# NVIDIA/vid2vid

Hardware: NVIDIA H100
Metric: frames/sec at 2048x1024 inference (higher is better)
Workload: dtype bf16x3 (split-bf16 hi/lo operands, 3 wgmma per K block, fp32 accumulate: fp32-class)

## Files before the change

### include/v2v_b200.h

```cpp
#ifndef V2V_B200_H
#define V2V_B200_H
#include <stdint.h>

#ifdef __cplusplus
extern "C" {
#endif

typedef struct CUstream_st* v2v_stream_t;
typedef struct v2v_plan v2v_plan;

#define V2V_ERR_INVALID 10001
#define V2V_ERR_STATE 10002
#define V2V_ERR_UNSUPPORTED 10003

enum { V2V_PAD_NONE = 0, V2V_PAD_ZERO = 1, V2V_PAD_REFLECT = 2 };
enum { V2V_ACT_NONE = 0, V2V_ACT_RELU = 1, V2V_ACT_LRELU = 2, V2V_ACT_TANH = 3, V2V_ACT_SIGMOID = 4 };
enum { V2V_NORM_NONE = 0, V2V_NORM_BATCH = 1, V2V_NORM_INSTANCE = 2 };
enum { V2V_IMPL_UMMA = 0, V2V_IMPL_SIMT = 1 };
enum { V2V_PREC_BF16 = 0, V2V_PREC_BF16X3 = 1 };

int v2v_version(void);
const char* v2v_last_error(void);


int v2v_correlation_out_shape(int H, int W, int pad_size, int kernel_size, int max_displacement, int stride1,
                              int stride2, int* outC, int* outH, int* outW);
int v2v_correlation_forward(const float* in1, const float* in2, float* out, int N, int C, int H, int W, int pad_size,
                            int kernel_size, int max_displacement, int stride1, int stride2, int corr_type_multiply,
                            v2v_stream_t stream);

int v2v_resample2d_forward(const float* in1, const float* flow, float* out, int N, int C, int H, int W, int inH,
                           int inW, int kernel_size, v2v_stream_t stream);

int v2v_channelnorm_forward(const float* in, float* out, int N, int C, int H, int W, int norm_deg,
                            v2v_stream_t stream);

int v2v_resample_forward(const float* image, const float* flow, float* out, int N, int C, int H, int W,
                         int align_corners, v2v_stream_t stream);

int v2v_onehot_edges(const float* labels, const float* inst, float* out, int F, int label_nc, int use_instance, int H,
                     int W, v2v_stream_t stream);

int v2v_avgpool3s2(const float* in, float* out, int P, int H, int W, v2v_stream_t stream);

int v2v_fg_mask(const float* real_A, float* mask, int B, int T, int C, int H, int W, int t, const int* fg_labels,
                int n_labels, v2v_stream_t stream);

int v2v_ids_window_push(float* window, const void* frame, int dtype, int B, int T, int H, int W, v2v_stream_t stream);
#define V2V_MAX_SLOTS 64
enum { V2V_SLOT_KEEP = 0, V2V_SLOT_PUSH = 1, V2V_SLOT_RESTART = 2, V2V_SLOT_CLEAR = 3 };
int v2v_slots_window_push(float* window, const void* frames, int dtype, int B, int T, int C, int H, int W, const int* ops,
                          v2v_stream_t stream);
int v2v_tensor2im_u8(const float* image, uint8_t* out, int B, int C, int H, int W, v2v_stream_t stream);

int v2v_l1_loss_forward(const float* a, const float* b, const float* mask, int N, int C, int H, int W, double* sum_ws, float* out,
                        v2v_stream_t stream);
int v2v_l1_loss_backward(const float* a, const float* b, const float* mask, int N, int C, int H, int W, const float* grad_out,
                         float* grad_a, float* grad_b, v2v_stream_t stream);
int v2v_mse_const_forward(const float* x, int64_t numel, float target, double* sum_ws, float* out, v2v_stream_t stream);
int v2v_mse_const_backward(const float* x, int64_t numel, float target, const float* grad_out, float* grad_x, v2v_stream_t stream);
int v2v_avgpool3s2_backward(const float* grad_out, float* grad_in, int P, int H, int W, v2v_stream_t stream);
int v2v_resample_backward(const float* image, const float* flow, const float* grad_out, float* grad_image, float* grad_flow, int N,
                          int C, int H, int W, int align_corners, v2v_stream_t stream);
int v2v_avgpool2(const float* in, float* out, int P, int H, int W, v2v_stream_t stream);
int v2v_avgpool2_backward(const float* grad_out, float* grad_in, int P, int H, int W, v2v_stream_t stream);
int v2v_face_region(const float* real_A, int N, int C, int H, int W, int openpose_only, int* box, v2v_stream_t stream);

#define V2V_MAX_INSTANCE_IDS 256
#define V2V_FACE_MAX_LABELS 32
#define V2V_FACE_MAX_FEAT 64
int v2v_instance_mean(const float* x, const float* inst, float* out, int N, int C, int H, int W, int n_ids, v2v_stream_t stream);
int v2v_face_features(const float* pooled, const float* inst, const float* table, const int* rows, int n_labels, int max_rows,
                      int num_images, int feat_num, int table_stride, float* out, int* chosen, int N, int H, int W,
                      v2v_stream_t stream);

int v2v_flownet_prep(const float* frame0, const float* frame1, int64_t batch_stride, int64_t channel_stride, float* x, float* x1,
                     float* mean_ws, int B, int H, int W, float rgb_max, v2v_stream_t stream);
int v2v_resize(const float* in, float* out, float* out_div, int planes, int h, int w, int H, int W, int mode, int use_scale_factor,
               float mul, float pre_div, float div, v2v_stream_t stream);
int v2v_sub_channels(const float* a, const float* b, float* out, int N, int Ca, int c_off, int C, int H, int W, v2v_stream_t stream);
int v2v_flow_conf(const float* im1, const float* warped, float* conf, int N, int C, int H, int W, float threshold,
                  v2v_stream_t stream);


typedef struct v2v_conv_desc {
  int Cin, Cout, kh, kw;
  int stride;
  int pad;
  int pad_mode;
  int transposed;
  int output_padding;
  const float* weight;
  const float* bias;
  int Cout2;
  const float* weight2;
  const float* bias2;
} v2v_conv_desc;

typedef struct v2v_norm_desc {
  int kind;
  const float* gamma;
  const float* beta;
  float* running_mean;
  float* running_var;
  int64_t* num_batches_tracked;
  float momentum, eps;
} v2v_norm_desc;

typedef struct v2v_head_channel {
  int slot;
  int channel;
  int dst_C;
  int act;
  float scale;
} v2v_head_channel;

int v2v_plan_create(int device, int conv_impl , v2v_plan** out);
int v2v_plan_destroy(v2v_plan* plan);
int v2v_plan_set_precision(v2v_plan* plan, int precision);

int v2v_g_input(v2v_plan* plan, int slot, int N, int C_src, int c_off, int C, int H, int W, int* value_out);
#define V2V_INPUT_EXACT_BF16 1
int v2v_g_input_ex(v2v_plan* plan, int slot, int N, int C_src, int c_off, int C, int H, int W, int flags, int* value_out);
int v2v_g_conv(v2v_plan* plan, int value_in, const v2v_conv_desc* conv, int* raw_out);
int v2v_g_norm_act(v2v_plan* plan, int raw_in, const v2v_norm_desc* norm, int act, float slope, int add0, int add1,
                   int* value_out);
int v2v_g_norm_act_slice(v2v_plan* plan, int raw_in, int c_off, int C, const v2v_norm_desc* norm, int act, float slope,
                         int add0, int add1, int* value_out);
int v2v_g_conv_act(v2v_plan* plan, int value_in, const v2v_conv_desc* conv, int act, float slope, int* value_out);
int v2v_g_head(v2v_plan* plan, int value_in, const v2v_conv_desc* conv, const v2v_head_channel* channels);
int v2v_g_concat(v2v_plan* plan, const int* values, int n, int* value_out);
int v2v_g_correlation(v2v_plan* plan, int value_a, int value_b, int pad_size, int kernel_size, int max_displacement, int stride1,
                      int stride2, int act, float slope, int* value_out);
int v2v_g_maxpool2(v2v_plan* plan, int value_in, int* value_out);
int v2v_g_feature_l1(v2v_plan* plan, int value_x, int value_y, int slot, int index);
int v2v_g_export(v2v_plan* plan, int value, int slot);
int v2v_g_composite(v2v_plan* plan, int s_raw, int s_flow, int s_weight, int s_prev, int prev_C, int s_fg, int s_mask,
                    int s_final, int N, int H, int W, int use_warp, int align_corners);

int v2v_g_composite_ex(v2v_plan* plan, int s_raw, int s_flow, int s_weight, int s_prev, int prev_C, int s_fg, int s_mask,
                       int s_final, int s_raw_out, int N, int H, int W, int use_warp, int align_corners);

int v2v_plan_set_training(v2v_plan* plan, int on);
int v2v_plan_set_sample_stats(v2v_plan* plan, int on);
#define V2V_IMAGE_ACTIVE 1
#define V2V_IMAGE_RAW_ONLY 2
int v2v_plan_set_image_flags(v2v_plan* plan, int slot);
int v2v_plan_backward(v2v_plan* plan, void* const* io_ptrs, void* const* grad_io_ptrs, int n_io, const void* const* params,
                      void* const* param_grads, int n_params, v2v_stream_t stream);

int v2v_plan_finalize(v2v_plan* plan, v2v_stream_t stream);
int v2v_plan_finalize_ws(v2v_plan* plan, void* workspace, int64_t workspace_bytes, v2v_stream_t stream);
int v2v_plan_repack(v2v_plan* plan, v2v_stream_t stream);
int v2v_plan_run(v2v_plan* plan, void* const* io_ptrs, int n_io, int use_graph, v2v_stream_t stream);

int v2v_plan_profile(v2v_plan* plan, void* const* io_ptrs, int n_io, v2v_stream_t stream, int max_ops, int* kinds,
                     float* ms, double* macs, int* n_ops);

int v2v_plan_num_kernels(const v2v_plan* plan);
double v2v_plan_conv_macs(const v2v_plan* plan);
int64_t v2v_plan_workspace_bytes(const v2v_plan* plan);
int64_t v2v_plan_describe(const v2v_plan* plan, char* buf, int64_t cap);

int v2v_conv_tap_table(const v2v_conv_desc* conv, int H, int W, int allow_reuse, int* n_groups, int* R, int* plane,
                       int* dy, int* dx, int* tap0, int* n_phases, int* phase_begin, int* oy_add, int* ox_add,
                       int* pads, int* parity, int* grid_hw, int* out_hw, int* mul);

#ifdef __cplusplus
}
#endif
#endif
```

### vid2vid_b200/_lib.py

```python
import ctypes as C
import os

_HERE = os.path.dirname(os.path.abspath(__file__))
LIB_PATH = os.environ.get('V2V_LIB') or os.path.join(_HERE, 'libv2v_b200.so')

PAD_NONE, PAD_ZERO, PAD_REFLECT = 0, 1, 2
ACT_NONE, ACT_RELU, ACT_LRELU, ACT_TANH, ACT_SIGMOID = 0, 1, 2, 3, 4
NORM_NONE, NORM_BATCH, NORM_INSTANCE = 0, 1, 2
IMPL_UMMA, IMPL_SIMT = 0, 1
PREC_BF16, PREC_BF16X3 = 0, 1
IMAGE_ACTIVE, IMAGE_RAW_ONLY = 1, 2
SLOT_KEEP, SLOT_PUSH, SLOT_RESTART, SLOT_CLEAR = 0, 1, 2, 3
MAX_SLOTS = 64


class ConvDesc(C.Structure):
    _fields_ = [('Cin', C.c_int), ('Cout', C.c_int), ('kh', C.c_int), ('kw', C.c_int), ('stride', C.c_int),
                ('pad', C.c_int), ('pad_mode', C.c_int), ('transposed', C.c_int), ('output_padding', C.c_int),
                ('weight', C.c_void_p), ('bias', C.c_void_p), ('Cout2', C.c_int), ('weight2', C.c_void_p),
                ('bias2', C.c_void_p)]


class NormDesc(C.Structure):
    _fields_ = [('kind', C.c_int), ('gamma', C.c_void_p), ('beta', C.c_void_p), ('running_mean', C.c_void_p),
                ('running_var', C.c_void_p), ('num_batches_tracked', C.c_void_p), ('momentum', C.c_float),
                ('eps', C.c_float)]


class HeadChannel(C.Structure):
    _fields_ = [('slot', C.c_int), ('channel', C.c_int), ('dst_C', C.c_int), ('act', C.c_int), ('scale', C.c_float)]


_lib = None
LAUNCHES = [0]

SYMBOLS = [
    'v2v_version', 'v2v_last_error',
    'v2v_correlation_out_shape', 'v2v_correlation_forward', 'v2v_resample2d_forward', 'v2v_channelnorm_forward',
    'v2v_resample_forward', 'v2v_onehot_edges', 'v2v_avgpool3s2', 'v2v_fg_mask',
    'v2v_l1_loss_forward', 'v2v_l1_loss_backward', 'v2v_mse_const_forward', 'v2v_mse_const_backward', 'v2v_avgpool3s2_backward',
    'v2v_resample_backward', 'v2v_avgpool2', 'v2v_avgpool2_backward', 'v2v_face_region', 'v2v_instance_mean', 'v2v_face_features', 'v2v_ids_window_push', 'v2v_slots_window_push', 'v2v_tensor2im_u8', 'v2v_flownet_prep', 'v2v_resize', 'v2v_sub_channels', 'v2v_flow_conf',
    'v2v_plan_create', 'v2v_plan_destroy', 'v2v_plan_set_precision', 'v2v_g_input', 'v2v_g_input_ex', 'v2v_g_conv', 'v2v_g_norm_act', 'v2v_g_norm_act_slice', 'v2v_g_conv_act',
    'v2v_g_head', 'v2v_g_concat', 'v2v_g_correlation', 'v2v_g_maxpool2', 'v2v_g_feature_l1', 'v2v_g_export', 'v2v_g_composite', 'v2v_g_composite_ex', 'v2v_plan_set_training', 'v2v_plan_set_sample_stats', 'v2v_plan_set_image_flags', 'v2v_plan_backward', 'v2v_plan_finalize', 'v2v_plan_finalize_ws', 'v2v_plan_repack', 'v2v_plan_run',
    'v2v_plan_profile', 'v2v_plan_num_kernels', 'v2v_plan_conv_macs', 'v2v_plan_workspace_bytes', 'v2v_plan_describe',
    'v2v_conv_tap_table',
]


def lib():
    global _lib
    if _lib is not None:
        return _lib
    if not os.path.exists(LIB_PATH):
        raise RuntimeError('libv2v_b200.so is not built (%s). Run `python -c "import __graft_entry__ as g; g.build()"` '
                           'or `python vid2vid_b200/build.py`. There is no fallback path.' % LIB_PATH)
    l = C.CDLL(LIB_PATH)
    l.v2v_last_error.restype = C.c_char_p
    l.v2v_plan_conv_macs.restype = C.c_double
    l.v2v_plan_workspace_bytes.restype = C.c_int64
    l.v2v_plan_describe.restype = C.c_int64
    l.v2v_plan_describe.argtypes = [C.c_void_p, C.c_char_p, C.c_int64]
    l.v2v_plan_create.argtypes = [C.c_int, C.c_int, C.POINTER(C.c_void_p)]
    l.v2v_plan_destroy.argtypes = [C.c_void_p]
    l.v2v_plan_set_precision.argtypes = [C.c_void_p, C.c_int]
    l.v2v_g_input.argtypes = [C.c_void_p] + [C.c_int] * 7 + [C.POINTER(C.c_int)]
    l.v2v_g_input_ex.argtypes = [C.c_void_p] + [C.c_int] * 8 + [C.POINTER(C.c_int)]
    l.v2v_g_conv.argtypes = [C.c_void_p, C.c_int, C.POINTER(ConvDesc), C.POINTER(C.c_int)]
    l.v2v_g_norm_act.argtypes = [C.c_void_p, C.c_int, C.POINTER(NormDesc), C.c_int, C.c_float, C.c_int, C.c_int,
                                 C.POINTER(C.c_int)]
    l.v2v_g_norm_act_slice.argtypes = [C.c_void_p, C.c_int, C.c_int, C.c_int, C.POINTER(NormDesc), C.c_int, C.c_float, C.c_int,
                                       C.c_int, C.POINTER(C.c_int)]
    l.v2v_g_conv_act.argtypes = [C.c_void_p, C.c_int, C.POINTER(ConvDesc), C.c_int, C.c_float, C.POINTER(C.c_int)]
    l.v2v_g_head.argtypes = [C.c_void_p, C.c_int, C.POINTER(ConvDesc), C.POINTER(HeadChannel)]
    l.v2v_g_export.argtypes = [C.c_void_p, C.c_int, C.c_int]
    l.v2v_g_maxpool2.argtypes = [C.c_void_p, C.c_int, C.POINTER(C.c_int)]
    l.v2v_g_feature_l1.argtypes = [C.c_void_p] + [C.c_int] * 4
    l.v2v_g_concat.argtypes = [C.c_void_p, C.POINTER(C.c_int), C.c_int, C.POINTER(C.c_int)]
    l.v2v_g_correlation.argtypes = [C.c_void_p] + [C.c_int] * 8 + [C.c_float, C.POINTER(C.c_int)]
    l.v2v_g_composite.argtypes = [C.c_void_p] + [C.c_int] * 13
    l.v2v_plan_finalize.argtypes = [C.c_void_p, C.c_void_p]
    l.v2v_plan_finalize_ws.argtypes = [C.c_void_p, C.c_void_p, C.c_int64, C.c_void_p]
    l.v2v_g_composite_ex.argtypes = [C.c_void_p] + [C.c_int] * 14
    l.v2v_plan_set_training.argtypes = [C.c_void_p, C.c_int]
    l.v2v_plan_set_sample_stats.argtypes = [C.c_void_p, C.c_int]
    l.v2v_plan_set_image_flags.argtypes = [C.c_void_p, C.c_int]
    l.v2v_plan_backward.argtypes = [C.c_void_p, C.POINTER(C.c_void_p), C.POINTER(C.c_void_p), C.c_int, C.POINTER(C.c_void_p),
                                    C.POINTER(C.c_void_p), C.c_int, C.c_void_p]
    l.v2v_plan_repack.argtypes = [C.c_void_p, C.c_void_p]
    l.v2v_plan_run.argtypes = [C.c_void_p, C.POINTER(C.c_void_p), C.c_int, C.c_int, C.c_void_p]
    l.v2v_plan_profile.argtypes = [C.c_void_p, C.POINTER(C.c_void_p), C.c_int, C.c_void_p, C.c_int, C.POINTER(C.c_int),
                                   C.POINTER(C.c_float), C.POINTER(C.c_double), C.POINTER(C.c_int)]
    l.v2v_plan_num_kernels.argtypes = [C.c_void_p]
    l.v2v_plan_conv_macs.argtypes = [C.c_void_p]
    l.v2v_plan_workspace_bytes.argtypes = [C.c_void_p]
    fp, ip, vp = C.c_void_p, C.POINTER(C.c_int), C.c_void_p
    l.v2v_correlation_out_shape.argtypes = [C.c_int] * 7 + [ip, ip, ip]
    l.v2v_correlation_forward.argtypes = [fp, fp, fp] + [C.c_int] * 10 + [vp]
    l.v2v_resample2d_forward.argtypes = [fp, fp, fp] + [C.c_int] * 7 + [vp]
    l.v2v_channelnorm_forward.argtypes = [fp, fp] + [C.c_int] * 5 + [vp]
    l.v2v_resample_forward.argtypes = [fp, fp, fp] + [C.c_int] * 5 + [vp]
    l.v2v_onehot_edges.argtypes = [fp, fp, fp] + [C.c_int] * 5 + [vp]
    l.v2v_avgpool3s2.argtypes = [fp, fp] + [C.c_int] * 3 + [vp]
    l.v2v_fg_mask.argtypes = [fp, fp] + [C.c_int] * 6 + [ip, C.c_int, vp]
    l.v2v_l1_loss_forward.argtypes = [fp, fp, fp] + [C.c_int] * 4 + [vp, fp, vp]
    l.v2v_l1_loss_backward.argtypes = [fp, fp, fp] + [C.c_int] * 4 + [fp, fp, fp, vp]
    l.v2v_mse_const_forward.argtypes = [fp, C.c_int64, C.c_float, vp, fp, vp]
    l.v2v_mse_const_backward.argtypes = [fp, C.c_int64, C.c_float, fp, fp, vp]
    l.v2v_avgpool3s2_backward.argtypes = [fp, fp, C.c_int, C.c_int, C.c_int, vp]
    l.v2v_avgpool2.argtypes = [fp, fp] + [C.c_int] * 3 + [vp]
    l.v2v_avgpool2_backward.argtypes = [fp, fp] + [C.c_int] * 3 + [vp]
    l.v2v_face_region.argtypes = [fp] + [C.c_int] * 5 + [vp, vp]
    l.v2v_instance_mean.argtypes = [fp, fp, fp] + [C.c_int] * 5 + [vp]
    l.v2v_face_features.argtypes = [fp, fp, fp, ip] + [C.c_int] * 5 + [fp, vp] + [C.c_int] * 3 + [vp]
    l.v2v_resample_backward.argtypes = [fp, fp, fp, fp, fp] + [C.c_int] * 5 + [vp]
    l.v2v_ids_window_push.argtypes = [fp, vp] + [C.c_int] * 5 + [vp]
    l.v2v_slots_window_push.argtypes = [fp, vp] + [C.c_int] * 6 + [ip, vp]
    l.v2v_tensor2im_u8.argtypes = [fp, vp] + [C.c_int] * 4 + [vp]
    l.v2v_flownet_prep.argtypes = [fp, fp, C.c_int64, C.c_int64, fp, fp, fp, C.c_int, C.c_int, C.c_int, C.c_float, vp]
    l.v2v_resize.argtypes = [fp, fp, fp] + [C.c_int] * 7 + [C.c_float, C.c_float, C.c_float, vp]
    l.v2v_sub_channels.argtypes = [fp, fp, fp] + [C.c_int] * 6 + [vp]
    l.v2v_flow_conf.argtypes = [fp, fp, fp] + [C.c_int] * 4 + [C.c_float, vp]
    l.v2v_conv_tap_table.argtypes = [C.POINTER(ConvDesc), C.c_int, C.c_int, C.c_int] + [ip] * 15
    _lib = l
    return l


def check(rc):
    if rc != 0:
        msg = lib().v2v_last_error()
        raise RuntimeError('libv2v_b200: error %d: %s' % (rc, msg.decode() if msg else '?'))


def current_stream_ptr():
    import torch
    return C.c_void_p(torch.cuda.current_stream().cuda_stream)
```

### vid2vid_b200/csrc/plan.cu

```cuda
#include <algorithm>
#include <cmath>
#include <cstdarg>
#include <cstdio>
#include <cstring>
#include <string>
#include <vector>

#include "plan_internal.h"

namespace v2v {

thread_local std::string g_last_error;
void set_error(const char* fmt, ...) {
  char buf[1024];
  va_list ap;
  va_start(ap, fmt);
  vsnprintf(buf, sizeof(buf), fmt, ap);
  va_end(ap);
  g_last_error = buf;
}

struct DeviceGuard {
  int prev = -1; bool changed = false;
  explicit DeviceGuard(int dev) {
    if (cudaGetDevice(&prev) == cudaSuccess && prev != dev) changed = (cudaSetDevice(dev) == cudaSuccess);
  }
  ~DeviceGuard() { if (changed) cudaSetDevice(prev); }
};

static ActDesc make_act(const Value& v, const Req& r, int split) {
  ActDesc a{};
  a.split = split;
  a.base = nullptr;
  a.N = v.N; a.H = v.H; a.W = v.W; a.Cvalid = v.C; a.C = v.Cp;
  a.pad_t = r.pads[0]; a.pad_l = r.pads[1]; a.pad_b = r.pads[2]; a.pad_r = r.pads[3];
  a.parity = r.parity;
  const int Hpad = v.H + a.pad_t + a.pad_b, Wpad = v.W + a.pad_l + a.pad_r;
  if (a.parity) { a.P = 4; a.Hp = (Hpad + 1) / 2; a.Wp = (Wpad + 1) / 2; }
  else { a.P = 1; a.Hp = Hpad; a.Wp = Wpad; }
  return a;
}

static bool same_req(const Req& a, const Req& b) {
  return a.mode == b.mode && a.parity == b.parity && !memcmp(a.pads, b.pads, sizeof(a.pads));
}

static int add_req(Value& v, const Req& r) {
  for (size_t i = 0; i < v.reqs.size(); ++i)
    if (same_req(v.reqs[i], r)) return (int)i;
  v.reqs.push_back(r);
  return (int)v.reqs.size() - 1;
}

static Req conv_req(const v2v_conv_desc& c, const ConvGeom& g) {
  Req r{};
  r.mode = c.transposed ? PAD_ZERO : (c.pad == 0 ? PAD_ZERO : c.pad_mode);
  memcpy(r.pads, g.pads, sizeof(r.pads));
  r.parity = g.parity;
  return r;
}

static void mark_backward_liveness(v2v_plan* P) {
  const size_t nv = P->values.size(), nr = P->raws.size();
  std::vector<int> uses(nv, 0), raw_uses(nr, 0);
  std::vector<char> live(nv, 0), raw_live(nr, 0);
  auto dead = [&](int v) { return uses[v] > 0 && !live[v]; };
  auto use = [&](int v, bool l) { if (v < 0) return; ++uses[v]; if (l) live[v] = 1; };
  P->op_live.assign(P->gops.size(), 1);
  for (int i = (int)P->gops.size() - 1; i >= 0; --i) {
    const GOp& op = P->gops[i];
    bool ol = true;
    switch (op.kind) {
      case G_INPUT: case G_RAWIN: case G_NORM_ACT: case G_CONV_ACT: case G_CONCAT: case G_CORR: case G_MAXPOOL:
        ol = !dead(op.value_out); break;
      case G_CONV: ol = !(raw_uses[op.raw] > 0 && !raw_live[op.raw]); break;
      default: break;
    }
    P->op_live[i] = ol;
    switch (op.kind) {
      case G_CONV: case G_CONV_ACT: case G_HEAD: case G_EXPORT: case G_MAXPOOL: use(op.value_in, ol); break;
      case G_NORM_ACT: ++raw_uses[op.raw]; if (ol) raw_live[op.raw] = 1; use(op.add[0], ol); use(op.add[1], ol); break;
      case G_CONCAT: for (int v : op.cat_in) use(v, ol); break;
      case G_CORR: use(op.value_in, ol); use(op.value_in2, ol); break;
      case G_FEATL1: use(op.value_in, true); use(op.value_in2, false); break;
      default: break;
    }
  }
  for (size_t v = 0; v < nv; ++v) P->values[v].detached = dead((int)v);
}

static int lower(v2v_plan* P) {
  if (P->lowered) return 0;
  for (auto& op : P->gops) {
    if (op.kind == G_CONV || op.kind == G_CONV_ACT || op.kind == G_HEAD) {
      Value& vin = P->values[op.value_in];
      int rc = conv_geometry(op.conv, vin.Cp, op.kind == G_HEAD ? (P->impl == V2V_IMPL_UMMA ? 2 : 1) : 0, P->tiling_n(vin.N), vin.H,
                             vin.W, true, P->sp(), &op.geom);
      if (rc) return rc;
      op.req_index = add_req(vin, conv_req(op.conv, op.geom));
      const v2v_conv_desc& c = op.conv;
      const double px = op.conv.transposed ? (double)vin.N * vin.H * vin.W : (double)vin.N * op.geom.out_h * op.geom.out_w;
      op.macs = px * c.Cin * c.Cout * c.kh * c.kw;
      P->conv_macs += op.macs;
    }
  }
  mark_backward_liveness(P);
  for (auto& v : P->values) {
    if (v.reqs.empty()) { Req r{}; r.mode = PAD_NONE; v.reqs.push_back(r); }
    v.bufs.clear();
    for (auto& r : v.reqs) {
      P->acts.push_back(make_act(v, r, P->precise));
      P->act_pad_mode.push_back(r.mode);
      v.bufs.push_back((int)P->acts.size() - 1);
    }
  }
  P->lowered = true;
  return 0;
}

int new_value(v2v_plan* p, int N, int H, int W, int C) {
  Value v; v.N = N; v.H = H; v.W = W; v.C = C; v.Cp = std::max(pad_channels(C), p->pad_min);
  p->values.push_back(v);
  return (int)p->values.size() - 1;
}

int size_arena(v2v_plan* P) {
  if (P->sized) return 0;
  int rc = lower(P); if (rc) return rc;
  size_t off = 0;
  auto take = [&](size_t bytes) { size_t o = off; off = round_up_sz(off + bytes, 1024); return o; };
  P->act_off.assign(P->acts.size(), 0);
  for (size_t i = 0; i < P->acts.size(); ++i) P->act_off[i] = take(P->acts[i].elems() * sizeof(bf16));
  P->raw_off.assign(P->raws.size(), v2v_plan::RawOff{});
  P->w_off.assign(P->gops.size(), 0);
  for (size_t i = 0; i < P->gops.size(); ++i) {
    GOp& op = P->gops[i];
    if (op.kind == G_CONV || op.kind == G_CONV_ACT || op.kind == G_HEAD) {
      fill_conv_params(P, op);
      P->w_off[i] = take((size_t)P->sp() * (op.geom.headkx ? op.geom.headkx * op.conv.Cout : op.conv.Cout) * op.Ktotal * sizeof(bf16));
      if (op.kind == G_CONV) {
        Raw& r = P->raws[op.raw];
        r.desc.N = r.N; r.desc.H = r.H; r.desc.W = r.W; r.desc.Cvalid = r.C; r.desc.C = round_up(r.C, 8);
        r.desc.f32 = P->precise;
        P->raw_off[op.raw].raw = take(r.desc.elems() * r.desc.elem_bytes());
        P->raw_off[op.raw].scale = take((size_t)r.N * r.C * sizeof(float));
        P->raw_off[op.raw].shift = take((size_t)r.N * r.C * sizeof(float));
      }
    }
  }
  P->corr_off.assign(P->gops.size(), 0);
  for (size_t i = 0; i < P->gops.size(); ++i)
    if (P->gops[i].kind == G_CORR) {
      const Value& a = P->values[P->gops[i].value_in], &o = P->values[P->gops[i].value_out];
      P->corr_off[i] = take((2 * (size_t)a.N * a.C * a.H * a.W + (size_t)o.N * o.C * o.H * o.W) * sizeof(float));
    }
  P->l1_off.assign(P->gops.size(), 0);
  for (size_t i = 0; i < P->gops.size(); ++i)
    if (P->gops[i].kind == G_FEATL1) {
      const Value& x = P->values[P->gops[i].value_in];
      P->l1_off[i] = take((size_t)feature_l1_blocks(make_act(x, x.reqs[0], P->precise)) * sizeof(double));
    }
  P->stats_begin = off;
  for (size_t i = 0; i < P->raws.size(); ++i)
    if (P->raws[i].conv_op >= 0 && !P->raws[i].no_stats) P->raw_off[i].stats = take((size_t)P->raws[i].N * 2 * P->raws[i].C * sizeof(stat_t) + 64);
  P->stats_end = off;
  P->arena_bytes = off;
  P->sized = true;
  return 0;
}

int run_xop(v2v_plan* P, const XOp& x, cudaStream_t s) {
  switch (x.kind) {
    case X_IMPORT: V2V_CUDA(launch_import_nchw(x.imp, s)); break;
    case X_EXPORT: V2V_CUDA(launch_export_nchw(x.exp, s)); break;
    case X_FINALIZE: V2V_CUDA(launch_stats_finalize(x.fin, s)); break;
    case X_APPLY: V2V_CUDA(launch_norm_apply(x.app, s)); break;
    case X_COMPOSITE: V2V_CUDA(launch_composite(x.comp, s)); break;
    case X_RAWSTATS: V2V_CUDA(launch_raw_stats(x.rawd, x.stats, x.stats_C, s)); break;
    case X_MEMSET: V2V_CUDA(cudaMemsetAsync(x.ms_ptr, 0, x.ms_bytes, s)); break;
    case X_COPY: V2V_CUDA(launch_act_copy(x.copy, s)); break;
    case X_CORR:
      V2V_CUDA(launch_correlation(x.corr.in1, x.corr.in2, x.corr.out, x.corr.N, x.corr.C, x.corr.H, x.corr.W, x.corr.pad, x.corr.k,
                                  x.corr.max_disp, x.corr.s1, x.corr.s2, s));
      break;
    case X_MAXPOOL: V2V_CUDA(launch_maxpool2(x.pool, s)); break;
    case X_FEATL1: V2V_CUDA(launch_feature_l1(x.fl1, s)); break;
    case X_CONV: {
      const GOp& op = P->gops[x.gop];
      if (P->impl == V2V_IMPL_UMMA) V2V_CUDA(launch_conv_umma(op.tmA, op.tmB, op.kp, s));
      else V2V_CUDA(launch_conv_simt(P->acts[P->values[op.value_in].bufs[op.req_index]], op.wpacked, op.Ktotal, op.kp, s));
      break;
    }
  }
  return 0;
}

FeatL1Params featl1_params(const v2v_plan* P, const GOp& op) {
  FeatL1Params f{};
  f.x = P->acts[P->values[op.value_in].bufs[0]]; f.y = P->acts[P->values[op.value_in2].bufs[0]];
  f.Cvalid = P->values[op.value_in].C;
  f.io = P->io_dev; f.slot = op.slot; f.index = op.l1_index;
  f.blocks = feature_l1_blocks(f.x);
  return f;
}

}

extern "C" {

int v2v_version(void) { return 100; }
const char* v2v_last_error(void) { return g_last_error.c_str(); }

int v2v_plan_create(int device, int conv_impl, v2v_plan** out) {
  V2V_REQUIRE(out, V2V_ERR_INVALID, "null out");
  v2v_plan* p = new v2v_plan();
  p->device = device;
  p->impl = conv_impl;
  *out = p;
  return 0;
}

int v2v_plan_set_precision(v2v_plan* p, int precision) {
  V2V_REQUIRE(p && !p->lowered && p->gops.empty(), V2V_ERR_STATE, "set the precision before describing the plan");
  V2V_REQUIRE(precision == V2V_PREC_BF16 || precision == V2V_PREC_BF16X3, V2V_ERR_INVALID, "unknown precision %d", precision);
  p->precise = (precision == V2V_PREC_BF16X3);
  return 0;
}

int v2v_plan_set_training(v2v_plan* p, int on) {
  V2V_REQUIRE(p && !p->finalized, V2V_ERR_STATE, "set the training flag before finalize");
  V2V_REQUIRE(!(on && p->sample_stats), V2V_ERR_STATE,
              "a per-sample-statistics plan cannot train: training normalises with the statistics of the whole batch");
  p->train = on != 0;
  return 0;
}

int v2v_plan_set_sample_stats(v2v_plan* p, int on) {
  V2V_REQUIRE(p && !p->lowered, V2V_ERR_STATE, "set per-sample statistics before the plan is lowered");
  V2V_REQUIRE(on || p->flags_slot < 0, V2V_ERR_STATE, "a plan with per-image flags keeps per-sample statistics");
  V2V_REQUIRE(!(on && p->train), V2V_ERR_STATE,
              "per-sample statistics are for inference plans: a training plan normalises with the statistics of the whole batch");
  p->sample_stats = on != 0;
  return 0;
}

int v2v_plan_set_image_flags(v2v_plan* p, int slot) {
  V2V_REQUIRE(p && !p->finalized, V2V_ERR_STATE, "set the image flags before finalize");
  V2V_REQUIRE(!p->train, V2V_ERR_STATE, "per-image flags are for inference plans: a training plan cannot skip images");
  V2V_REQUIRE(p->sample_stats, V2V_ERR_STATE,
              "per-image flags need a per-sample-statistics plan: batch statistics mix the images, so none can be skipped");
  V2V_REQUIRE(slot >= 0, V2V_ERR_INVALID, "bad flags slot %d", slot);
  p->flags_slot = slot;
  p->n_slots = std::max(p->n_slots, slot + 1);
  return 0;
}

int v2v_plan_backward(v2v_plan* P, void* const* io_ptrs, void* const* grad_io_ptrs, int n_io, const void* const* params,
                      void* const* param_grads, int n_params, v2v_stream_t stream_) {
  V2V_REQUIRE(P && P->finalized && P->train, V2V_ERR_STATE, "plan not finalized in training mode");
  V2V_REQUIRE(n_io >= P->n_slots && io_ptrs && grad_io_ptrs, V2V_ERR_INVALID, "need %d io / gradient pointers", P->n_slots);
  DeviceGuard guard(P->device);
  std::unordered_map<const void*, void*> pg;
  for (int i = 0; i < n_params; ++i) if (params[i] && param_grads[i]) pg[params[i]] = param_grads[i];
  return run_backward(P, io_ptrs, grad_io_ptrs, pg, reinterpret_cast<cudaStream_t>(stream_));
}

int v2v_plan_destroy(v2v_plan* p) {
  if (!p) return 0;
  if (p->graph_exec) cudaGraphExecDestroy(p->graph_exec);
  if (p->graph_stream) cudaStreamDestroy(p->graph_stream);
  if (p->arena && p->arena_owned) cudaFree(p->arena);
  if (p->garena) cudaFree(p->garena);
  if (p->train_stats) cudaFree(p->train_stats);
  if (p->io_dev) cudaFree(p->io_dev);
  if (p->wg_stage) cudaFree(p->wg_stage);
  for (auto& u : p->bwd) if (u.child) v2v_plan_destroy(u.child);
  delete p;
  return 0;
}

int v2v_g_input_ex(v2v_plan* p, int slot, int N, int C_src, int c_off, int C, int H, int W, int flags, int* value_out) {
  int rc = v2v_g_input(p, slot, N, C_src, c_off, C, H, W, value_out);
  if (rc) return rc;
  p->values[*value_out].exact_bf16 = (flags & V2V_INPUT_EXACT_BF16) != 0;
  return 0;
}

int v2v_g_input(v2v_plan* p, int slot, int N, int C_src, int c_off, int C, int H, int W, int* value_out) {
  V2V_REQUIRE(p && !p->lowered && value_out, V2V_ERR_STATE, "plan already lowered or null");
  V2V_REQUIRE(slot >= 0 && N > 0 && C > 0 && c_off >= 0 && c_off + C <= C_src && H > 0 && W > 0, V2V_ERR_INVALID,
              "bad input description");
  GOp op; op.kind = G_INPUT; op.slot = slot; op.C_src = C_src; op.c_off = c_off;
  op.value_out = new_value(p, N, H, W, C);
  p->values[op.value_out].input_slot = slot;
  p->n_slots = std::max(p->n_slots, slot + 1);
  p->gops.push_back(op);
  *value_out = op.value_out;
  return 0;
}

static int check_conv(v2v_plan* p, int value_in, const v2v_conv_desc* c) {
  V2V_REQUIRE(p && !p->lowered && c, V2V_ERR_STATE, "plan already lowered or null");
  V2V_REQUIRE(value_in >= 0 && value_in < (int)p->values.size(), V2V_ERR_INVALID, "bad value id %d", value_in);
  V2V_REQUIRE(c->Cin == p->values[value_in].C, V2V_ERR_INVALID, "conv Cin %d != value channels %d", c->Cin,
              p->values[value_in].C);
  V2V_REQUIRE(c->Cout > 0, V2V_ERR_INVALID, "bad Cout");
  return 0;
}

int v2v_g_conv(v2v_plan* p, int value_in, const v2v_conv_desc* c, int* raw_out) {
  int rc = check_conv(p, value_in, c); if (rc) return rc;
  V2V_REQUIRE(raw_out, V2V_ERR_INVALID, "null raw_out");
  ConvGeom g; rc = conv_geometry(*c, p->values[value_in].Cp, 0, p->values[value_in].N, p->values[value_in].H, p->values[value_in].W, true, p->sp(), &g); if (rc) return rc;
  GOp op; op.kind = G_CONV; op.value_in = value_in; op.conv = *c;
  Raw r{}; r.N = p->values[value_in].N; r.H = g.out_h; r.W = g.out_w; r.C = c->Cout; r.conv_op = (int)p->gops.size();
  p->raws.push_back(r);
  op.raw = (int)p->raws.size() - 1;
  p->gops.push_back(op);
  *raw_out = op.raw;
  return 0;
}

int v2v_g_norm_act_slice(v2v_plan* p, int raw_in, int c_off, int C, const v2v_norm_desc* norm, int act, float slope,
                         int add0, int add1, int* value_out) {
  V2V_REQUIRE(p && !p->lowered && norm && value_out, V2V_ERR_STATE, "plan already lowered or null");
  V2V_REQUIRE(raw_in >= 0 && raw_in < (int)p->raws.size(), V2V_ERR_INVALID, "bad raw id");
  const Raw& r = p->raws[raw_in];
  V2V_REQUIRE(c_off >= 0 && C > 0 && c_off + C <= r.C && (c_off % 8) == 0, V2V_ERR_INVALID,
              "bad channel slice [%d, %d) of %d", c_off, c_off + C, r.C);
  GOp op; op.kind = G_NORM_ACT; op.raw = raw_in; op.norm = *norm; op.act = act; op.slope = slope;
  op.add[0] = add0; op.add[1] = add1; op.n_off = c_off; op.cC = C;
  for (int k = 0; k < 2; ++k)
    if (op.add[k] >= 0) {
      V2V_REQUIRE(op.add[k] < (int)p->values.size(), V2V_ERR_INVALID, "bad addend id");
      const Value& a = p->values[op.add[k]];
      V2V_REQUIRE(a.N == r.N && a.H == r.H && a.W == r.W && a.C == C, V2V_ERR_INVALID,
                  "addend shape (%d,%d,%d,%d) != raw shape (%d,%d,%d,%d)", a.N, a.C, a.H, a.W, r.N, C, r.H, r.W);
    }
  op.value_out = new_value(p, r.N, r.H, r.W, C);
  p->gops.push_back(op);
  *value_out = op.value_out;
  return 0;
}

int v2v_g_norm_act(v2v_plan* p, int raw_in, const v2v_norm_desc* norm, int act, float slope, int add0, int add1,
                   int* value_out) {
  V2V_REQUIRE(p && raw_in >= 0 && raw_in < (int)p->raws.size(), V2V_ERR_INVALID, "bad raw id");
  return v2v_g_norm_act_slice(p, raw_in, 0, p->raws[raw_in].C, norm, act, slope, add0, add1, value_out);
}

int v2v_g_conv_act(v2v_plan* p, int value_in, const v2v_conv_desc* c, int act, float slope, int* value_out) {
  int rc = check_conv(p, value_in, c); if (rc) return rc;
  V2V_REQUIRE(value_out, V2V_ERR_INVALID, "null value_out");
  ConvGeom g; rc = conv_geometry(*c, p->values[value_in].Cp, 0, p->values[value_in].N, p->values[value_in].H, p->values[value_in].W, true, p->sp(), &g); if (rc) return rc;
  GOp op; op.kind = G_CONV_ACT; op.value_in = value_in; op.conv = *c; op.act = act; op.slope = slope;
  op.value_out = new_value(p, p->values[value_in].N, g.out_h, g.out_w, c->Cout);
  p->gops.push_back(op);
  *value_out = op.value_out;
  return 0;
}

int v2v_g_head(v2v_plan* p, int value_in, const v2v_conv_desc* c, const v2v_head_channel* ch) {
  int rc = check_conv(p, value_in, c); if (rc) return rc;
  V2V_REQUIRE(ch && c->Cout <= V2V_MAX_HEAD && !c->transposed && c->stride == 1, V2V_ERR_UNSUPPORTED,
              "head conv must be stride-1 with Cout <= %d", V2V_MAX_HEAD);
  GOp op; op.kind = G_HEAD; op.value_in = value_in; op.conv = *c;
  for (int j = 0; j < c->Cout; ++j) { op.head[j] = ch[j]; p->n_slots = std::max(p->n_slots, ch[j].slot + 1); }
  p->gops.push_back(op);
  return 0;
}

int v2v_g_concat(v2v_plan* p, const int* values, int n, int* value_out) {
  V2V_REQUIRE(p && !p->lowered && values && n >= 1 && value_out, V2V_ERR_STATE, "plan already lowered or null");
  GOp op; op.kind = G_CONCAT;
  int C = 0;
  for (int i = 0; i < n; ++i) {
    V2V_REQUIRE(values[i] >= 0 && values[i] < (int)p->values.size(), V2V_ERR_INVALID, "bad value id %d", values[i]);
    const Value& a = p->values[values[i]], &a0 = p->values[values[0]];
    V2V_REQUIRE(a.N == a0.N && a.H == a0.H && a.W == a0.W, V2V_ERR_INVALID, "concat operands differ in extent");
    C += a.C;
    op.cat_in.push_back(values[i]);
  }
  const int N0 = p->values[values[0]].N, H0 = p->values[values[0]].H, W0 = p->values[values[0]].W;
  op.value_out = new_value(p, N0, H0, W0, C);
  p->gops.push_back(op);
  *value_out = op.value_out;
  return 0;
}

int v2v_g_correlation(v2v_plan* p, int value_a, int value_b, int pad_size, int kernel_size, int max_displacement, int stride1,
                      int stride2, int act, float slope, int* value_out) {
  V2V_REQUIRE(p && !p->lowered && value_out, V2V_ERR_STATE, "plan already lowered or null");
  V2V_REQUIRE(value_a >= 0 && value_a < (int)p->values.size() && value_b >= 0 && value_b < (int)p->values.size(), V2V_ERR_INVALID,
              "bad value id");
  const Value a = p->values[value_a], b = p->values[value_b];
  V2V_REQUIRE(a.N == b.N && a.C == b.C && a.H == b.H && a.W == b.W, V2V_ERR_INVALID, "correlation operands differ in shape");
  V2V_REQUIRE(kernel_size == 1 && stride1 == 1 && pad_size == max_displacement, V2V_ERR_UNSUPPORTED,
              "correlation: only kernel 1, stride1 1, pad == max displacement (FlowNetC.py:31)");
  V2V_REQUIRE(act == V2V_ACT_NONE || act == V2V_ACT_LRELU, V2V_ERR_UNSUPPORTED, "correlation: activation must be none / LeakyReLU");
  int oc, oh, ow;
  int rc = v2v_correlation_out_shape(a.H, a.W, pad_size, kernel_size, max_displacement, stride1, stride2, &oc, &oh, &ow);
  if (rc) return rc;
  GOp op; op.kind = G_CORR; op.value_in = value_a; op.value_in2 = value_b; op.act = act; op.slope = slope;
  op.corr[0] = pad_size; op.corr[1] = kernel_size; op.corr[2] = max_displacement; op.corr[3] = stride1; op.corr[4] = stride2;
  op.value_out = new_value(p, a.N, oh, ow, oc);
  p->gops.push_back(op);
  *value_out = op.value_out;
  return 0;
}

int v2v_g_maxpool2(v2v_plan* p, int value_in, int* value_out) {
  V2V_REQUIRE(p && !p->lowered && value_out, V2V_ERR_STATE, "plan already lowered or null");
  V2V_REQUIRE(value_in >= 0 && value_in < (int)p->values.size(), V2V_ERR_INVALID, "bad value id %d", value_in);
  const Value a = p->values[value_in];
  V2V_REQUIRE(a.H >= 2 && a.W >= 2, V2V_ERR_INVALID, "max-pool input %dx%d is smaller than its window", a.H, a.W);
  GOp op; op.kind = G_MAXPOOL; op.value_in = value_in;
  op.value_out = new_value(p, a.N, a.H / 2, a.W / 2, a.C);
  p->gops.push_back(op);
  *value_out = op.value_out;
  return 0;
}

int v2v_g_feature_l1(v2v_plan* p, int value_x, int value_y, int slot, int index) {
  V2V_REQUIRE(p && !p->lowered, V2V_ERR_STATE, "plan already lowered or null");
  V2V_REQUIRE(value_x >= 0 && value_x < (int)p->values.size() && value_y >= 0 && value_y < (int)p->values.size() && value_x != value_y,
              V2V_ERR_INVALID, "bad value ids %d, %d", value_x, value_y);
  V2V_REQUIRE(slot >= 0 && index >= 0, V2V_ERR_INVALID, "bad output slot %d / index %d", slot, index);
  const Value a = p->values[value_x], b = p->values[value_y];
  V2V_REQUIRE(a.N == b.N && a.C == b.C && a.H == b.H && a.W == b.W, V2V_ERR_INVALID, "feature L1 operands differ in shape");
  GOp op; op.kind = G_FEATL1; op.value_in = value_x; op.value_in2 = value_y; op.slot = slot; op.l1_index = index;
  p->n_slots = std::max(p->n_slots, slot + 1);
  p->gops.push_back(op);
  return 0;
}

int v2v_g_export(v2v_plan* p, int value, int slot) {
  V2V_REQUIRE(p && !p->lowered, V2V_ERR_STATE, "plan already lowered or null");
  V2V_REQUIRE(value >= 0 && value < (int)p->values.size() && slot >= 0, V2V_ERR_INVALID, "bad export");
  GOp op; op.kind = G_EXPORT; op.value_in = value; op.slot = slot;
  p->n_slots = std::max(p->n_slots, slot + 1);
  p->gops.push_back(op);
  return 0;
}

int v2v_g_composite(v2v_plan* p, int s_raw, int s_flow, int s_weight, int s_prev, int prev_C, int s_fg, int s_mask,
                    int s_final, int N, int H, int W, int use_warp, int align_corners) {
  return v2v_g_composite_ex(p, s_raw, s_flow, s_weight, s_prev, prev_C, s_fg, s_mask, s_final, -1, N, H, W, use_warp, align_corners);
}

int v2v_g_composite_ex(v2v_plan* p, int s_raw, int s_flow, int s_weight, int s_prev, int prev_C, int s_fg, int s_mask,
                       int s_final, int s_raw_out, int N, int H, int W, int use_warp, int align_corners) {
  V2V_REQUIRE(p && !p->lowered, V2V_ERR_STATE, "plan already lowered or null");
  V2V_REQUIRE(s_raw >= 0 && s_final >= 0, V2V_ERR_INVALID, "composite needs raw and final slots");
  V2V_REQUIRE(!use_warp || (s_flow >= 0 && s_weight >= 0 && s_prev >= 0 && prev_C >= 3), V2V_ERR_INVALID,
              "warp needs flow, weight and prev");
  V2V_REQUIRE((s_fg >= 0) == (s_mask >= 0), V2V_ERR_INVALID, "fg and mask go together");
  GOp op; op.kind = G_COMPOSITE;
  CompositeParams& c = op.comp;
  c.s_raw = s_raw; c.s_flow = s_flow; c.s_weight = s_weight; c.s_prev = s_prev; c.s_fg = s_fg; c.s_mask = s_mask;
  c.s_raw_out = s_raw_out;
  p->n_slots = std::max(p->n_slots, s_raw_out + 1);
  c.s_final = s_final; c.prev_C = prev_C; c.N = N; c.H = H; c.W = W; c.align_corners = align_corners; c.use_warp = use_warp;
  int m = std::max({s_raw, s_flow, s_weight, s_prev, s_fg, s_mask, s_final});
  p->n_slots = std::max(p->n_slots, m + 1);
  p->gops.push_back(op);
  return 0;
}

static int finalize_impl(v2v_plan* P, void* workspace, size_t workspace_bytes, cudaStream_t stream) {
  V2V_REQUIRE(P && !P->finalized, V2V_ERR_STATE, "plan null or already finalized");
  int rc = size_arena(P); if (rc) return rc;
  DeviceGuard guard(P->device);
  const std::vector<size_t>& act_off = P->act_off;
  const std::vector<v2v_plan::RawOff>& raw_off = P->raw_off;
  const std::vector<size_t>& w_off = P->w_off;
  const std::vector<size_t>& corr_off = P->corr_off;
  const size_t stats_begin = P->stats_begin, stats_end = P->stats_end;
  if (workspace) {
    V2V_REQUIRE(workspace_bytes >= P->arena_bytes && (reinterpret_cast<uintptr_t>(workspace) & 1023) == 0, V2V_ERR_INVALID,
                "workspace of %zu bytes (1024-byte aligned) needed, got %zu at %p", P->arena_bytes, workspace_bytes, workspace);
    P->arena = workspace; P->arena_owned = false;
  } else {
    V2V_CUDA(cudaMalloc(&P->arena, P->arena_bytes));
  }
  V2V_CUDA(cudaMemsetAsync(P->arena, 0, P->arena_bytes, stream));
  V2V_CUDA(cudaMalloc(reinterpret_cast<void**>(&P->io_dev), sizeof(void*) * std::max(1, P->n_slots)));
  uint8_t* base = reinterpret_cast<uint8_t*>(P->arena);
  for (size_t i = 0; i < P->acts.size(); ++i) P->acts[i].base = reinterpret_cast<bf16*>(base + act_off[i]);
  for (size_t i = 0; i < P->raws.size(); ++i) {
    Raw& r = P->raws[i];
    r.desc.base = base + raw_off[i].raw;
    r.stats = reinterpret_cast<stat_t*>(base + raw_off[i].stats);
    r.scale = reinterpret_cast<float*>(base + raw_off[i].scale);
    r.shift = reinterpret_cast<float*>(base + raw_off[i].shift);
  }

  if (P->train) {
    size_t tot = 0;
    for (auto& r : P->raws) tot += 2 * (size_t)r.N * r.C;
    float* st = nullptr;
    V2V_CUDA(cudaMalloc(reinterpret_cast<void**>(&st), std::max<size_t>(tot, 1) * sizeof(float)));
    V2V_CUDA(cudaMemsetAsync(st, 0, std::max<size_t>(tot, 1) * sizeof(float), stream));
    P->train_stats = st;
    for (auto& r : P->raws) { r.mean = st; st += (size_t)r.N * r.C; r.rstd = st; st += (size_t)r.N * r.C; }
  }
  if (stats_end > stats_begin) {
    XOp m; m.kind = X_MEMSET; m.ms_ptr = base + stats_begin; m.ms_bytes = stats_end - stats_begin;
    P->xops.push_back(m);
  }
  for (size_t i = 0; i < P->gops.size(); ++i) {
    GOp& op = P->gops[i];
    switch (op.kind) {
      case G_INPUT: {
        const Value& v = P->values[op.value_out];
        for (size_t m = 0; m < v.bufs.size(); ++m) {
          XOp x; x.kind = X_IMPORT; x.gop = (int)i;
          x.imp.io = reinterpret_cast<const void* const*>(P->io_dev); x.imp.slot = op.slot;
          x.imp.c_off = op.c_off; x.imp.C_src = op.C_src;
          x.imp.out = P->acts[v.bufs[m]]; x.imp.pad_mode = P->act_pad_mode[v.bufs[m]];
          x.imp.skip_lo = v.exact_bf16 ? 1 : 0;
          P->xops.push_back(x);
        }
        break;
      }
      case G_CONV: case G_CONV_ACT: case G_HEAD: {
        const Value& vin = P->values[op.value_in];
        const ActDesc& ain = P->acts[vin.bufs[op.req_index]];
        op.wpacked = reinterpret_cast<bf16*>(base + w_off[i]);
        ConvKernelParams& kp = op.kp;
        V2V_REQUIRE(kp.Cp == ain.C, V2V_ERR_STATE, "internal: conv of op %zu reads %d padded channels from a %d-channel buffer", i,
                    kp.Cp, ain.C);
        kp.io = P->io_dev;
        if (op.kind == G_CONV) {
          Raw& r = P->raws[op.raw];
          kp.epi = EPI_RAW_STATS; kp.out = r.desc.base; kp.out_C = r.desc.C; kp.out_f32 = r.desc.f32;
          kp.stats = r.no_stats ? nullptr : r.stats; kp.stats_C = r.C; kp.bias = nullptr;
        } else if (op.kind == G_CONV_ACT) {
          const Value& vo = P->values[op.value_out];
          V2V_REQUIRE(vo.bufs.size() == 1 && P->act_pad_mode[vo.bufs[0]] != PAD_REFLECT, V2V_ERR_UNSUPPORTED,
                      "conv_act output needs a single zero/none-padded consumer layout");
          kp.epi = EPI_ACT_BF16; kp.out_act = P->acts[vo.bufs[0]]; kp.out_C = kp.out_act.C;
        } else {
          kp.epi = EPI_HEAD_F32;
          kp.bias2 = op.conv.Cout2 > 0 ? op.conv.bias2 : nullptr; kp.Cout1 = op.conv.Cout - op.conv.Cout2;
          for (int j = 0; j < op.conv.Cout; ++j) {
            kp.head_slot[j] = op.head[j].slot;
            kp.head_off[j] = (long long)op.head[j].channel * op.geom.out_h * op.geom.out_w;
            kp.head_bstride[j] = (long long)op.head[j].dst_C * op.geom.out_h * op.geom.out_w;
            kp.head_act[j] = op.head[j].act; kp.head_scale[j] = op.head[j].scale;
          }
        }
        if (P->impl == V2V_IMPL_UMMA) {
          rc = make_tmap_act(&op.tmA, ain, kp.PW, kp.PH, kp.kc); if (rc) return rc;
          rc = make_tmap_w(&op.tmB, op.wpacked, P->sp() * op.Ktotal, op.geom.headkx ? op.geom.headkx * op.conv.Cout : op.conv.Cout, kp.BN,
                           kp.kc); if (rc) return rc;
        }
        rc = pack_one(op, stream); if (rc) return rc;
        XOp x; x.kind = X_CONV; x.gop = (int)i;
        P->xops.push_back(x);
        if (op.kind == G_CONV && P->impl == V2V_IMPL_SIMT) {
          XOp s; s.kind = X_RAWSTATS; s.rawd = P->raws[op.raw].desc; s.stats = P->raws[op.raw].stats; s.stats_C = P->raws[op.raw].C;
          P->xops.push_back(s);
        }
        break;
      }
      case G_NORM_ACT: {
        Raw& r = P->raws[op.raw];
        const GOp& cop = P->gops[r.conv_op];
        FinalizeParams fp{};
        const bool has_norm = op.norm.kind != V2V_NORM_NONE;
        if (has_norm) {
          fp.stats = r.stats; fp.Cs = r.C; fp.C = op.cC; fp.c_off = op.n_off; fp.scale_stride = r.C;
          fp.N = r.N;
          fp.count = (double)r.H * r.W; fp.instance = (op.norm.kind == V2V_NORM_INSTANCE) || P->sample_stats;
          fp.sample_running = P->sample_stats;
          fp.io = P->io_dev; fp.flags_slot = P->flags_slot;
          const int cout1 = cop.conv.Cout - cop.conv.Cout2;
          V2V_REQUIRE(op.n_off == 0 || (cop.conv.Cout2 > 0 && op.n_off == cout1), V2V_ERR_UNSUPPORTED,
                      "a raw slice must start at channel 0 or at the second weight set");
          fp.gamma = op.norm.gamma; fp.beta = op.norm.beta; fp.conv_bias = op.n_off == 0 ? cop.conv.bias : cop.conv.bias2;
          fp.momentum = op.norm.momentum; fp.eps = op.norm.eps;
        } else if (cop.conv.bias != nullptr) {
          V2V_REQUIRE(op.n_off == 0 && cop.conv.Cout2 == 0, V2V_ERR_UNSUPPORTED, "biased norm-less conv cannot be sliced");
          v2v_plan::BiasAffine ba{r.scale, r.shift, cop.conv.bias, r.N, r.C, r.C};
          P->bias_affines.push_back(ba);
          V2V_CUDA(launch_bias_affine(ba.scale, ba.shift, ba.bias, ba.N, ba.C, ba.stride, stream));
        }
        const Value& vo = P->values[op.value_out];
        for (size_t m = 0; m < vo.bufs.size(); ++m) {
          XOp a; a.kind = X_APPLY;
          ApplyParams& ap = a.app;
          ap.raw = r.desc;
          ap.raw.base = reinterpret_cast<uint8_t*>(r.desc.base) + (size_t)op.n_off * r.desc.elem_bytes();
          ap.raw.Cvalid = op.cC;
          ap.scale = (has_norm || cop.conv.bias != nullptr) ? r.scale + op.n_off : nullptr;
          ap.shift = r.shift + op.n_off;
          ap.scale_stride = r.C;
          ap.act = op.act; ap.slope = op.slope;
          ap.n_add = 0;
          for (int k = 0; k < 2; ++k) if (op.add[k] >= 0) ap.add[ap.n_add++] = P->acts[P->values[op.add[k]].bufs[0]];
          ap.out = P->acts[vo.bufs[m]]; ap.pad_mode = P->act_pad_mode[vo.bufs[m]];
          if (has_norm) {
            const bool first = std::find(r.running_done.begin(), r.running_done.end(), op.n_off) == r.running_done.end();
            FinalizeParams side = fp;
            side.running_mean = op.norm.running_mean; side.running_var = op.norm.running_var;
            side.num_batches_tracked = reinterpret_cast<long long*>(op.norm.num_batches_tracked);
            side.scale = r.scale; side.shift = r.shift; side.mean_out = r.mean; side.rstd_out = r.rstd;
            if (first) {
              GOp& prod = P->gops[r.conv_op];
              if (P->impl == V2V_IMPL_UMMA && prod.kp.n_fin < 2) {
                prod.kp.fin[prod.kp.n_fin++] = side;
                prod.kp.fin_counter = reinterpret_cast<unsigned int*>(reinterpret_cast<uint8_t*>(r.stats) + (size_t)r.N * 2 * r.C * sizeof(stat_t));
              } else {
                XOp f; f.kind = X_FINALIZE; f.fin = side; P->xops.push_back(f);
              }
              r.running_done.push_back(op.n_off);
            }
          }
          P->xops.push_back(a);
        }
        break;
      }
      case G_RAWIN: {
        const Value& vo = P->values[op.value_out];
        for (size_t m = 0; m < vo.bufs.size(); ++m) {
          XOp a; a.kind = X_APPLY;
          ApplyParams& ap = a.app;
          ap.raw.base = const_cast<float*>(op.ext_raw); ap.raw.N = vo.N; ap.raw.H = vo.H; ap.raw.W = vo.W; ap.raw.C = op.ext_C;
          ap.raw.Cvalid = vo.C; ap.raw.f32 = 1;
          ap.scale = nullptr; ap.shift = nullptr; ap.scale_stride = 0; ap.act = ACT_NONE; ap.slope = 0.f; ap.n_add = 0;
          ap.out = P->acts[vo.bufs[m]]; ap.pad_mode = P->act_pad_mode[vo.bufs[m]];
          P->xops.push_back(a);
        }
        break;
      }
      case G_EXPORT: {
        XOp x; x.kind = X_EXPORT; x.exp.io = P->io_dev; x.exp.slot = op.slot; x.exp.in = P->acts[P->values[op.value_in].bufs[0]];
        P->xops.push_back(x);
        break;
      }
      case G_COMPOSITE: {
        XOp x; x.kind = X_COMPOSITE; x.comp = op.comp; x.comp.io = P->io_dev; x.comp.s_flags = P->flags_slot;
        P->xops.push_back(x);
        break;
      }
      case G_CONCAT: {
        const Value& vo = P->values[op.value_out];
        for (size_t m = 0; m < vo.bufs.size(); ++m) {
          int c_off = 0;
          for (int src : op.cat_in) {
            XOp x; x.kind = X_COPY;
            x.copy.in = P->acts[P->values[src].bufs[0]];
            x.copy.out = P->acts[vo.bufs[m]];
            x.copy.c_off = c_off; x.copy.pad_mode = P->act_pad_mode[vo.bufs[m]];
            c_off += P->values[src].C;
            P->xops.push_back(x);
          }
        }
        break;
      }
      case G_MAXPOOL: {
        const Value& vo = P->values[op.value_out];
        for (size_t m = 0; m < vo.bufs.size(); ++m) {
          V2V_REQUIRE(P->act_pad_mode[vo.bufs[m]] != PAD_REFLECT, V2V_ERR_UNSUPPORTED, "max-pool output needs a zero / no halo");
          XOp x; x.kind = X_MAXPOOL; x.gop = (int)i;
          x.pool.in = P->acts[P->values[op.value_in].bufs[0]]; x.pool.out = P->acts[vo.bufs[m]];
          P->xops.push_back(x);
        }
        break;
      }
      case G_FEATL1: {
        XOp x; x.kind = X_FEATL1; x.gop = (int)i;
        x.fl1 = featl1_params(P, op);
        x.fl1.partials = reinterpret_cast<double*>(base + P->l1_off[i]);
        P->xops.push_back(x);
        break;
      }
      case G_CORR: {
        const Value& va = P->values[op.value_in], &vb = P->values[op.value_in2], &vo = P->values[op.value_out];
        float* sa = reinterpret_cast<float*>(base + corr_off[i]);
        float* sb = sa + (size_t)va.N * va.C * va.H * va.W;
        float* so = sb + (size_t)va.N * va.C * va.H * va.W;
        XOp ea; ea.kind = X_EXPORT; ea.exp.io = P->io_dev; ea.exp.slot = 0; ea.exp.direct = sa; ea.exp.in = P->acts[va.bufs[0]];
        XOp eb = ea; eb.exp.direct = sb; eb.exp.in = P->acts[vb.bufs[0]];
        P->xops.push_back(ea); P->xops.push_back(eb);
        XOp c; c.kind = X_CORR;
        c.corr = CorrParams{sa, sb, so, va.N, va.C, va.H, va.W, op.corr[0], op.corr[1], op.corr[2], op.corr[3], op.corr[4]};
        P->xops.push_back(c);
        for (size_t m = 0; m < vo.bufs.size(); ++m) {
          XOp x; x.kind = X_IMPORT; x.gop = (int)i;
          x.imp.io = reinterpret_cast<const void* const*>(P->io_dev); x.imp.slot = 0; x.imp.direct = so;
          x.imp.c_off = 0; x.imp.C_src = vo.C; x.imp.act = op.act; x.imp.slope = op.slope;
          x.imp.out = P->acts[vo.bufs[m]]; x.imp.pad_mode = P->act_pad_mode[vo.bufs[m]];
          P->xops.push_back(x);
        }
        break;
      }
    }
  }
  if (P->train) {
    rc = alloc_training(P, stream); if (rc) return rc;
    rc = build_backward_units(P, stream); if (rc) return rc;
  }
  V2V_CUDA(cudaStreamSynchronize(stream));
  P->finalized = true;
  return 0;
}

int v2v_plan_finalize(v2v_plan* P, v2v_stream_t stream_) {
  return finalize_impl(P, nullptr, 0, reinterpret_cast<cudaStream_t>(stream_));
}

int v2v_plan_finalize_ws(v2v_plan* P, void* workspace, int64_t workspace_bytes, v2v_stream_t stream_) {
  V2V_REQUIRE(workspace && workspace_bytes > 0, V2V_ERR_INVALID, "null workspace");
  return finalize_impl(P, workspace, (size_t)workspace_bytes, reinterpret_cast<cudaStream_t>(stream_));
}

int v2v_plan_repack(v2v_plan* P, v2v_stream_t stream_) {
  V2V_REQUIRE(P && P->finalized, V2V_ERR_STATE, "plan not finalized");
  DeviceGuard guard(P->device);
  cudaStream_t stream = reinterpret_cast<cudaStream_t>(stream_);
  for (auto& op : P->gops)
    if (op.kind == G_CONV || op.kind == G_CONV_ACT || op.kind == G_HEAD) { int rc = pack_one(op, stream); if (rc) return rc; }
  for (const auto& ba : P->bias_affines) V2V_CUDA(launch_bias_affine(ba.scale, ba.shift, ba.bias, ba.N, ba.C, ba.stride, stream));
  for (auto& u : P->bwd) if (u.child) { int rc = v2v_plan_repack(u.child, stream_); if (rc) return rc; }
  return 0;
}

static int check_composite_alignment(const v2v_plan* P, void* const* io_ptrs) {
  for (const XOp& x : P->xops)
    if (x.kind == X_COMPOSITE && composite_vec4(x.comp))
      V2V_REQUIRE(composite_slots_aligned(x.comp, io_ptrs), V2V_ERR_INVALID,
                  "composite (W %% 4 == 0) needs 16-byte aligned raw / final / flow / weight / fg / mask tensors");
  return 0;
}

int v2v_plan_run(v2v_plan* P, void* const* io_ptrs, int n_io, int use_graph, v2v_stream_t stream_) {
  V2V_REQUIRE(P && P->finalized, V2V_ERR_STATE, "plan not finalized");
  V2V_REQUIRE(n_io >= P->n_slots && io_ptrs, V2V_ERR_INVALID, "need %d io pointers, got %d", P->n_slots, n_io);
  if (int rc = check_composite_alignment(P, io_ptrs)) return rc;
  DeviceGuard guard(P->device);
  cudaStream_t stream = reinterpret_cast<cudaStream_t>(stream_);
  V2V_CUDA(cudaMemcpyAsync(P->io_dev, io_ptrs, sizeof(void*) * P->n_slots, cudaMemcpyHostToDevice, stream));
  if (use_graph & 2) {
    for (const XOp& x : P->xops) {
      if (x.kind == X_FINALIZE) {
        XOp y = x; y.fin.running_mean = nullptr; y.fin.running_var = nullptr; y.fin.num_batches_tracked = nullptr;
        int rc = run_xop(P, y, stream); if (rc) return rc;
      } else if (x.kind == X_CONV && P->impl == V2V_IMPL_UMMA && P->gops[x.gop].kp.n_fin > 0) {
        const GOp& op = P->gops[x.gop];
        ConvKernelParams kp = op.kp;
        for (int q = 0; q < kp.n_fin; ++q) { kp.fin[q].running_mean = nullptr; kp.fin[q].running_var = nullptr; kp.fin[q].num_batches_tracked = nullptr; }
        V2V_CUDA(launch_conv_umma(op.tmA, op.tmB, kp, stream));
      } else { int rc = run_xop(P, x, stream); if (rc) return rc; }
    }
    return 0;
  }
  if (!use_graph) {
    for (const XOp& x : P->xops) { int rc = run_xop(P, x, stream); if (rc) return rc; }
    return 0;
  }
  if (!P->graph_exec) {
    cudaGraph_t graph;
    if (!P->graph_stream) V2V_CUDA(cudaStreamCreateWithFlags(&P->graph_stream, cudaStreamNonBlocking));
    V2V_CUDA(cudaStreamBeginCapture(P->graph_stream, cudaStreamCaptureModeThreadLocal));
    int rc = 0;
    for (const XOp& x : P->xops) { rc = run_xop(P, x, P->graph_stream); if (rc) break; }
    cudaError_t e = cudaStreamEndCapture(P->graph_stream, &graph);
    if (rc) return rc;
    V2V_CUDA(e);
    V2V_CUDA(cudaGraphInstantiate(&P->graph_exec, graph, 0));
    V2V_CUDA(cudaGraphDestroy(graph));
  }
  V2V_CUDA(cudaGraphLaunch(P->graph_exec, stream));
  return 0;
}

int v2v_plan_profile(v2v_plan* P, void* const* io_ptrs, int n_io, v2v_stream_t stream_, int max_ops, int* kinds,
                     float* ms, double* macs, int* n_ops) {
  V2V_REQUIRE(P && P->finalized, V2V_ERR_STATE, "plan not finalized");
  V2V_REQUIRE(n_io >= P->n_slots && io_ptrs && kinds && ms && macs && n_ops, V2V_ERR_INVALID, "bad profile arguments");
  if (int rc = check_composite_alignment(P, io_ptrs)) return rc;
  DeviceGuard guard(P->device);
  cudaStream_t stream = reinterpret_cast<cudaStream_t>(stream_);
  V2V_CUDA(cudaMemcpyAsync(P->io_dev, io_ptrs, sizeof(void*) * P->n_slots, cudaMemcpyHostToDevice, stream));
  const int n = std::min<int>(max_ops, (int)P->xops.size());
  std::vector<cudaEvent_t> ev(n + 1);
  for (auto& e : ev) V2V_CUDA(cudaEventCreate(&e));
  V2V_CUDA(cudaEventRecord(ev[0], stream));
  for (int i = 0; i < (int)P->xops.size(); ++i) {
    int rc = run_xop(P, P->xops[i], stream);
    if (rc) return rc;
    if (i < n) V2V_CUDA(cudaEventRecord(ev[i + 1], stream));
  }
  V2V_CUDA(cudaStreamSynchronize(stream));
  for (int i = 0; i < n; ++i) {
    V2V_CUDA(cudaEventElapsedTime(&ms[i], ev[i], ev[i + 1]));
    kinds[i] = (int)P->xops[i].kind;
    macs[i] = (P->xops[i].kind == X_CONV) ? P->gops[P->xops[i].gop].macs : 0.0;
  }
  for (auto& e : ev) cudaEventDestroy(e);
  *n_ops = n;
  return 0;
}

int v2v_plan_num_kernels(const v2v_plan* P) { return P ? (int)P->xops.size() : 0; }
double v2v_plan_conv_macs(const v2v_plan* P) {
  if (!P) return 0.0;
  if (!P->lowered) lower(const_cast<v2v_plan*>(P));
  return P->conv_macs;
}
int64_t v2v_plan_workspace_bytes(const v2v_plan* P_) {
  v2v_plan* P = const_cast<v2v_plan*>(P_);
  if (!P) return 0;
  if (!P->sized && size_arena(P)) return -1;
  return (int64_t)P->arena_bytes;
}

}

extern "C" {

int64_t v2v_plan_describe(const v2v_plan* P_, char* buf, int64_t cap) {
// ... 78 lines not shown
```

### vid2vid_b200/csrc/plan_internal.h

```cpp
#pragma once
#include <string>
#include <unordered_map>
#include <vector>

#include "../../include/v2v_b200.h"
#include "v2v_internal.h"
#include "backward.h"

namespace v2v {

void set_error(const char* fmt, ...);

#define V2V_CUDA(expr)                                                                          \
  do {                                                                                          \
    cudaError_t e__ = (expr);                                                                   \
    if (e__ != cudaSuccess) {                                                                   \
      set_error("%s failed: %s (%s:%d)", #expr, cudaGetErrorString(e__), __FILE__, __LINE__);   \
      return (int)e__;                                                                          \
    }                                                                                           \
  } while (0)
#define V2V_REQUIRE(cond, code, ...) \
  do {                               \
    if (!(cond)) {                   \
      set_error(__VA_ARGS__);        \
      return code;                   \
    }                                \
  } while (0)

static inline int round_up(int a, int b) { return (a + b - 1) / b * b; }
static inline size_t round_up_sz(size_t a, size_t b) { return (a + b - 1) / b * b; }
static inline int pad_channels(int c) { return c <= 16 ? 16 : (c <= 32 ? 32 : round_up(c, 64)); }

struct ConvGeom {
  int pads[4];
  int parity;
  int grid_h, grid_w;
  int out_h, out_w;
  int mul;
  int TH, TW, R;
  int RW;
  int patch2d_kc;
  int patch2d_bn;
  int headkx;
  int n_groups, n_phases;
  ConvGroup groups[V2V_MAX_TAPS];
  ConvPhase phases[V2V_MAX_PHASES];
};

struct Req { int mode, pads[4], parity; };

struct Value {
  int N, H, W, C;
  int Cp;
  std::vector<Req> reqs;
  std::vector<int> bufs;
  float* gval = nullptr;
  int input_slot = -1;
  bool exact_bf16 = false;
  bool detached = false;
};
struct Raw {
  int N, H, W, C;
  int conv_op = -1;
  RawDesc desc{};
  stat_t* stats = nullptr;
  float* scale = nullptr; float* shift = nullptr;
  std::vector<int> running_done;
  float* mean = nullptr; float* rstd = nullptr;
  float* graw = nullptr;
  bool no_stats = false;
};

enum GKind { G_INPUT, G_CONV, G_NORM_ACT, G_CONV_ACT, G_HEAD, G_EXPORT, G_COMPOSITE, G_CONCAT, G_CORR, G_RAWIN, G_MAXPOOL, G_FEATL1 };
struct GOp {
  GKind kind;
  int slot = -1, C_src = 0, c_off = 0;
  int value_in = -1, value_out = -1, raw = -1;
  v2v_conv_desc conv{};
  ConvGeom geom{};
  int req_index = -1;
  v2v_norm_desc norm{};
  int act = 0; float slope = 0.f;
  int add[2] = {-1, -1};
  int n_off = 0, cC = 0;
  v2v_head_channel head[V2V_MAX_HEAD];
  CompositeParams comp{};
  std::vector<int> cat_in;
  int value_in2 = -1;
  int l1_index = 0;
  int corr[5] = {0, 0, 0, 0, 0};
  const float* ext_raw = nullptr; int ext_C = 0;
  int pack_dgrad = 0; const float* dg_w2 = nullptr; int dg_Cout1 = 0;
  bf16* wpacked = nullptr; int Ktotal = 0, Cp = 0;
  float* gdz = nullptr;
  double macs = 0.0;
  CUtensorMap tmA{}, tmB{};
  ConvKernelParams kp{};
};

enum XKind { X_IMPORT, X_CONV, X_RAWSTATS, X_FINALIZE, X_APPLY, X_EXPORT, X_COMPOSITE, X_MEMSET, X_COPY, X_CORR, X_MAXPOOL, X_FEATL1 };
struct XOp {
  XKind kind;
  int gop = -1;
  ImportParams imp{};
  ExportParams exp{};
  FinalizeParams fin{};
  ApplyParams app{};
  CompositeParams comp{};
  CopyParams copy{};
  CorrParams corr{};
  PoolParams pool{};
  FeatL1Params fl1{};
  RawDesc rawd{}; stat_t* stats = nullptr; int stats_C = 0;
  void* ms_ptr = nullptr; size_t ms_bytes = 0;
};

}

using namespace v2v;

struct BwdUnit {
  int gop = -1, mode = 0;
  v2v_plan* child = nullptr;
  int child_raw = -1;
  bool wgrad = false;
  std::string simt, wg_simt;
  CUtensorMap tmOut{}, tmIn{};
  WgradParams wg{};
  int M = 0, M1 = 0, Nv = 0;
};

struct v2v_plan {
  std::vector<BwdUnit> bwd;
  std::vector<int> bwd_of;
  float* wg_stage = nullptr;
  int pad_min = 0;

  int device = 0;
  int impl = V2V_IMPL_UMMA;
  int precise = 0;
  int sp() const { return precise ? 2 : 1; }
  bool lowered = false, finalized = false;
  bool train = false;
  bool sample_stats = false;
  int tiling_n(int N) const { return sample_stats ? 1 : N; }
  int flags_slot = -1;
  void* garena = nullptr; size_t garena_bytes = 0;
  std::vector<float*> gslot;
  float* gsums = nullptr;
  float* train_stats = nullptr;
  std::vector<Value> values;
  std::vector<Raw> raws;
  std::vector<GOp> gops;
  std::vector<ActDesc> acts;
  std::vector<int> act_pad_mode;
  std::vector<char> op_live;
  std::vector<XOp> xops;
  int n_slots = 0;
  double conv_macs = 0.0;
  struct BiasAffine { float* scale; float* shift; const float* bias; int N, C, stride; };
  std::vector<BiasAffine> bias_affines;
  struct RawOff { size_t raw = 0, stats = 0, scale = 0, shift = 0; };
  bool sized = false, arena_owned = true;
  std::vector<size_t> act_off, w_off, corr_off, l1_off;
  std::vector<RawOff> raw_off;
  size_t stats_begin = 0, stats_end = 0;
  void* arena = nullptr; size_t arena_bytes = 0;
  void** io_dev = nullptr;
  cudaGraphExec_t graph_exec = nullptr;
  cudaStream_t graph_stream = nullptr;
};

namespace v2v {

extern const int kSmemBudget;
int conv_geometry(const v2v_conv_desc& c, int Cp, int head, int N, int H, int W, bool allow_reuse, int sp, ConvGeom* g);
void fill_conv_params(v2v_plan* P, GOp& op);
int make_tmap_act(CUtensorMap* tm, const ActDesc& a, int box_w, int box_h, int kc);
int make_tmap_w(CUtensorMap* tm, bf16* w, int Ktotal, int Cout, int BN, int kc);
int pack_one(const GOp& op, cudaStream_t stream);
void describe_conv(v2v_plan* P, const GOp& op, std::string& s);

int new_value(v2v_plan* p, int N, int H, int W, int C);
int size_arena(v2v_plan* P);
int run_xop(v2v_plan* P, const XOp& x, cudaStream_t s);
FeatL1Params featl1_params(const v2v_plan* P, const GOp& op);

int alloc_training(v2v_plan* P, cudaStream_t stream);
int choose_backward_unit(v2v_plan* P, int i, BwdUnit& u);
int build_backward_units(v2v_plan* P, cudaStream_t stream);
int run_backward(v2v_plan* P, void* const* io, void* const* gio, const std::unordered_map<const void*, void*>& pg,
                 cudaStream_t s);
void describe_backward_unit(const BwdUnit& u, std::string& s);
void describe_epilogue_backward(const v2v_plan* P, std::string& s);

}
```

### vid2vid_b200/csrc/pyramid.cu

```cuda
#include "../../include/v2v_b200.h"
#include "ptx.cuh"
#include "v2v_internal.h"

namespace v2v {

__global__ void onehot_edges_kernel(const float* __restrict__ labels, const float* __restrict__ inst,
                                    float* __restrict__ out, int F, int label_nc, int use_inst, int H, int W) {
  const size_t HW = (size_t)H * W;
  const int Cout = label_nc + (use_inst ? 1 : 0);
  const int x = blockIdx.x * blockDim.x + threadIdx.x, y = blockIdx.y, f = blockIdx.z;
  if (x < W) {
    const size_t pix = (size_t)y * W + x;
    const size_t idx = (size_t)f * HW + pix;
    const int lab = (int)labels[idx];
    float* o = out + (size_t)f * Cout * HW + pix;
    for (int c = 0; c < label_nc; ++c) o[(size_t)c * HW] = (c == lab) ? 1.f : 0.f;
    if (use_inst) {
      const float* ip = inst + (size_t)f * HW;
      const float v = ip[pix];
      bool e = false;
      if (x > 0) e |= (ip[pix - 1] != v);
      if (x < W - 1) e |= (ip[pix + 1] != v);
      if (y > 0) e |= (ip[pix - W] != v);
      if (y < H - 1) e |= (ip[pix + W] != v);
      o[(size_t)label_nc * HW] = e ? 1.f : 0.f;
    }
  }
}

__global__ void __launch_bounds__(256) avgpool3s2_kernel(const float* __restrict__ in, float* __restrict__ out, int P, int H, int W,
                                                         int Ho, int Wo) {
  const int xo = blockIdx.x * blockDim.x + threadIdx.x;
  if (xo >= Wo) return;
  const int yo = blockIdx.y;
  for (int pl = blockIdx.z; pl < P; pl += gridDim.z) {
    const float* ip = in + (size_t)pl * H * W;
    float s = 0.f;
    int cnt = 0;
#pragma unroll
    for (int dy = -1; dy <= 1; ++dy) {
      const int y = 2 * yo + dy;
      if (y < 0 || y >= H) continue;
#pragma unroll
      for (int dx = -1; dx <= 1; ++dx) {
        const int x = 2 * xo + dx;
        if (x < 0 || x >= W) continue;
        s += __ldg(ip + (size_t)y * W + x);
        ++cnt;
      }
    }
    out[((size_t)pl * Ho + yo) * Wo + xo] = s / (float)cnt;
  }
}

__global__ void __launch_bounds__(128) avgpool3s2_vec_kernel(const float* __restrict__ in, float* __restrict__ out, int P, int H, int W,
                                                             int Ho, int Wo) {
  const int k = blockIdx.x * blockDim.x + threadIdx.x;
  if (4 * k >= W) return;
  const int yo = blockIdx.y;
  for (int pl = blockIdx.z; pl < P; pl += gridDim.z) {
    const float* ip = in + (size_t)pl * H * W;
    float s0 = 0.f, s1 = 0.f;
    int rows = 0;
#pragma unroll
    for (int dy = -1; dy <= 1; ++dy) {
      const int y = 2 * yo + dy;
      if (y < 0 || y >= H) continue;
      ++rows;
      const float* rp = ip + (size_t)y * W + 4 * k;
      const float4 v = *reinterpret_cast<const float4*>(rp);
      if (k > 0) s0 += __ldg(rp - 1);
      s0 += v.x; s0 += v.y;
      s1 += v.y; s1 += v.z; s1 += v.w;
    }
    const int c0 = (k > 0 ? 3 : 2), c1 = 3;
    *reinterpret_cast<float2*>(out + ((size_t)pl * Ho + yo) * Wo + 2 * k) = make_float2(s0 / (float)(rows * c0), s1 / (float)(rows * c1));
  }
}

struct FgLabels { int v[16]; };
__global__ void fg_mask_kernel(const float* __restrict__ real_A, float* __restrict__ mask, int B, int T, int C, int H,
                               int W, int t, FgLabels labels, int n_labels) {
  const size_t HW = (size_t)H * W, total = (size_t)B * HW;
  for (size_t idx = blockIdx.x * (size_t)blockDim.x + threadIdx.x; idx < total;
       idx += (size_t)gridDim.x * blockDim.x) {
    const int b = (int)(idx / HW);
    const size_t pix = idx - (size_t)b * HW;
    float s = 0.f;
    for (int i = 0; i < n_labels; ++i) s += real_A[(((size_t)b * T + t) * C + labels.v[i]) * HW + pix];
    mask[idx] = fminf(fmaxf(s, 0.f), 1.f);
  }
}

__global__ void ids_window_push_kernel(float* __restrict__ window, const void* __restrict__ frame, int dtype, int T, size_t HW,
                                       size_t total) {
  for (size_t idx = blockIdx.x * (size_t)blockDim.x + threadIdx.x; idx < total; idx += (size_t)gridDim.x * blockDim.x) {
    const size_t b = idx / HW, pix = idx - b * HW;
    float* win = window + b * T * HW;
    for (int t = 0; t + 1 < T; ++t) win[(size_t)t * HW + pix] = win[(size_t)(t + 1) * HW + pix];
    float v;
    if (dtype == 0) v = (float)reinterpret_cast<const uint8_t*>(frame)[idx];
    else if (dtype == 1) v = (float)reinterpret_cast<const int*>(frame)[idx];
    else v = reinterpret_cast<const float*>(frame)[idx];
    win[(size_t)(T - 1) * HW + pix] = v;
  }
}

struct SlotOps { int v[V2V_MAX_SLOTS]; };
__global__ void slots_window_push_kernel(float* __restrict__ window, const void* __restrict__ frames, int dtype, int T, size_t E,
                                         size_t total, SlotOps ops) {
  for (size_t idx = blockIdx.x * (size_t)blockDim.x + threadIdx.x; idx < total; idx += (size_t)gridDim.x * blockDim.x) {
    const size_t b = idx / E, e = idx - b * E;
    const int op = ops.v[b];
    if (op == V2V_SLOT_KEEP) continue;
    float* win = window + b * T * E;
    if (op == V2V_SLOT_PUSH)
      for (int t = 0; t + 1 < T; ++t) win[(size_t)t * E + e] = win[(size_t)(t + 1) * E + e];
    else
      for (int t = 0; t + 1 < T; ++t) win[(size_t)t * E + e] = 0.f;
    float v = 0.f;
    if (op != V2V_SLOT_CLEAR) {
      if (dtype == 0) v = (float)reinterpret_cast<const uint8_t*>(frames)[idx];
      else if (dtype == 1) v = (float)reinterpret_cast<const int*>(frames)[idx];
      else v = reinterpret_cast<const float*>(frames)[idx];
    }
    win[(size_t)(T - 1) * E + e] = v;
  }
}

__global__ void tensor2im_u8_kernel(const float* __restrict__ img, uint8_t* __restrict__ out, int C, size_t HW, size_t total) {
  for (size_t pix = blockIdx.x * (size_t)blockDim.x + threadIdx.x; pix < total; pix += (size_t)gridDim.x * blockDim.x) {
    const size_t b = pix / HW, p = pix - b * HW;
    for (int c = 0; c < C; ++c) {
      float v = __fmul_rn(__fdiv_rn(__fadd_rn(img[(b * C + c) * HW + p], 1.f), 2.0f), 255.0f);
      v = fminf(fmaxf(v, 0.f), 255.f);
      out[pix * C + c] = (uint8_t)v;
    }
  }
}

static inline int grid1d(size_t total) {
  size_t b = (total + 255) / 256;
  const size_t cap = 132 * 16;
  return (int)(b < cap ? (b ? b : 1) : cap);
}

cudaError_t launch_onehot_edges(const float* labels, const float* inst, float* out, int F, int label_nc, int use_inst,
                                int H, int W, cudaStream_t s) {
  dim3 grid((W + 255) / 256, H, F);
  onehot_edges_kernel<<<grid, 256, 0, s>>>(labels, inst, out, F, label_nc, use_inst, H, W);
  return cudaGetLastError();
}
cudaError_t launch_avgpool3s2(const float* in, float* out, int P, int H, int W, cudaStream_t s) {
  const int Ho = (H - 1) / 2 + 1, Wo = (W - 1) / 2 + 1;
  const bool aligned = (reinterpret_cast<uintptr_t>(in) & 15) == 0 && (reinterpret_cast<uintptr_t>(out) & 7) == 0;
  if (W % 4 == 0 && W >= 4 && aligned) {
    dim3 grid((W / 4 + 127) / 128, Ho, P < 64 ? P : 64);
    avgpool3s2_vec_kernel<<<grid, 128, 0, s>>>(in, out, P, H, W, Ho, Wo);
    return cudaGetLastError();
  }
  dim3 grid((Wo + 255) / 256, Ho, P < 64 ? P : 64);
  avgpool3s2_kernel<<<grid, 256, 0, s>>>(in, out, P, H, W, Ho, Wo);
  return cudaGetLastError();
}
cudaError_t launch_ids_window_push(float* window, const void* frame, int dtype, int B, int T, int H, int W, cudaStream_t s) {
  ids_window_push_kernel<<<grid1d((size_t)B * H * W), 256, 0, s>>>(window, frame, dtype, T, (size_t)H * W, (size_t)B * H * W);
  return cudaGetLastError();
}
cudaError_t launch_slots_window_push(float* window, const void* frames, int dtype, int B, int T, int C, int H, int W, const int* ops,
                                    cudaStream_t s) {
  SlotOps o{};
  for (int b = 0; b < B; ++b) o.v[b] = ops[b];
  const size_t E = (size_t)C * H * W;
  slots_window_push_kernel<<<grid1d((size_t)B * E), 256, 0, s>>>(window, frames, dtype, T, E, (size_t)B * E, o);
  return cudaGetLastError();
}
cudaError_t launch_tensor2im_u8(const float* img, uint8_t* out, int B, int C, int H, int W, cudaStream_t s) {
  tensor2im_u8_kernel<<<grid1d((size_t)B * H * W), 256, 0, s>>>(img, out, C, (size_t)H * W, (size_t)B * H * W);
  return cudaGetLastError();
}
cudaError_t launch_fg_mask(const float* real_A, float* mask, int B, int T, int C, int H, int W, int t,
                           FgLabels labels, int n_labels, cudaStream_t s) {
  fg_mask_kernel<<<grid1d((size_t)B * H * W), 256, 0, s>>>(real_A, mask, B, T, C, H, W, t, labels, n_labels);
  return cudaGetLastError();
}

}
```

### vid2vid_b200/csrc/v2v_internal.h

```cpp
#pragma once
#include <cuda.h>
#include <cuda_runtime.h>
#include <cuda_bf16.h>
#include <stdint.h>

namespace v2v {

typedef __nv_bfloat16 bf16;

struct ActDesc {
  bf16* base;
  int N, H, W;
  int C;
  int Cvalid;
  int pad_t, pad_l, pad_b, pad_r;
  int parity;
  int P, Hp, Wp;
  int split;
  __host__ __device__ int Cs() const { return C << split; }
  __host__ __device__ size_t elems() const { return (size_t)N * P * Hp * Wp * Cs(); }
  __host__ __device__ size_t offset(int n, int y, int x) const {
    int yp = y + pad_t, xp = x + pad_l;
    if (parity) {
      int pl = ((yp & 1) << 1) | (xp & 1);
      return ((((size_t)n * 4 + pl) * Hp + (yp >> 1)) * Wp + (xp >> 1)) * Cs();
    }
    return (((size_t)n * Hp + yp) * Wp + xp) * Cs();
  }
};

struct RawDesc {
  void* base;
  int N, H, W, C, Cvalid;
  int f32;
  __host__ __device__ size_t elems() const { return (size_t)N * H * W * C; }
  __host__ __device__ size_t elem_bytes() const { return f32 ? 4 : 2; }
};

enum PadMode { PAD_NONE = 0, PAD_ZERO = 1, PAD_REFLECT = 2 };
enum ActKind { ACT_NONE = 0, ACT_RELU = 1, ACT_LRELU = 2, ACT_TANH = 3, ACT_SIGMOID = 4 };
enum EpiMode { EPI_RAW_STATS = 0, EPI_HEAD_F32 = 1, EPI_ACT_BF16 = 2 };

#define V2V_MAX_TAPS 64
#define V2V_MAX_PHASES 4
#define V2V_MAX_HEAD 16
#define V2V_MAX_ACC_COLS 128

struct ConvGroup {
  int8_t plane, dy, dx, pad_;
  int16_t tap0, pad2_;
};

struct ConvPhase {
  int group_begin, group_end;
  int oy_add, ox_add;
};

typedef unsigned long long stat_t;
#define V2V_STAT_SUM_SCALE 1048576.0f
#define V2V_STAT_SQ_SCALE 65536.0f

struct FinalizeParams {
  const stat_t* stats;
  int Cs, C;
  int N;
  double count;
  int instance;
  int sample_running;
  const float* gamma;
  const float* beta;
  const float* conv_bias;
  float* running_mean;
  float* running_var;
  long long* num_batches_tracked;
  float momentum, eps;
  float* scale;
  float* shift;
  float* mean_out;
  float* rstd_out;
  int c_off, scale_stride;
  void* const* io;
  int flags_slot = -1;
};

struct ConvKernelParams {
  int N, tiles_x, tiles_y, TH, TW;
  int grid_h, grid_w;
  int Cout, BN;
  int Cp, cblocks;
  int kc, row_bytes, kmma;
  int kmma_last;
  int BNt;
  int layout_type, sbo_bytes;
  int R, RW;
  int PW, PH;
  int sbo_a_bytes;
  int a_slot_bytes, b_slot_bytes, SB;
  int b_resident;
  int n_tiles, m_total;
  int CG, SG;
  int MG, total_units;
  int num_phases;
  int split;
  int a_half_bytes, b_half_bytes;
  int Khalf;
  int out_f32;
  int ring2, TB, SBr;
  int tile_dx;
  int headkx;
  int n_fin;
  FinalizeParams fin[2];
  unsigned int* fin_counter;
  int a_exact;

  ConvPhase phases[V2V_MAX_PHASES];
  ConvGroup groups[V2V_MAX_TAPS];
  int epi;
  int oy_mul, ox_mul;
  int out_H, out_W, out_C;
  void* out;
  ActDesc out_act;
  stat_t* stats;
  int stats_C;
  const float* bias;
  const float* bias2; int Cout1;
  int grid;
  void* const* io;
  int head_slot[V2V_MAX_HEAD];
  long long head_off[V2V_MAX_HEAD];
  long long head_bstride[V2V_MAX_HEAD];
  int head_act[V2V_MAX_HEAD];
  float head_scale[V2V_MAX_HEAD];
  float lrelu_slope;
  int act;
};

cudaError_t launch_conv_umma(const CUtensorMap& tmA, const CUtensorMap& tmB, const ConvKernelParams& p,
                             cudaStream_t stream);
cudaError_t launch_conv_simt(const ActDesc& in, const bf16* wpacked, int Ktotal, const ConvKernelParams& p,
                             cudaStream_t stream);
size_t conv_umma_smem_bytes(const ConvKernelParams& p);
int conv_umma_tail_width(const ConvKernelParams& p);
int conv_umma_async_epilogue(const ConvKernelParams& p);



struct ApplyParams {
  RawDesc raw;
  const float* scale;
  const float* shift;
  int scale_stride;
  int act; float slope;
  int n_add;
  ActDesc add[2];
  ActDesc out;
  int pad_mode;
};

struct ImportParams {
  const void* const* io;
  int slot;
  const float* direct;
  int act; float slope;
  int c_off, C_src;
  ActDesc out;
  int pad_mode;
  int skip_lo;
};
struct ExportParams {
  void* const* io;
  int slot;
  float* direct;
  ActDesc in;
};

struct CopyParams {
  ActDesc in, out;
  int c_off;
  int pad_mode;
};

struct CorrParams {
  const float* in1; const float* in2; float* out;
  int N, C, H, W, pad, k, max_disp, s1, s2;
};

struct PackParams {
  const float* w;
  const float* w2; int Cout1;
  int transposed;
  int Cout, Cin, kh, kw;
  int Cp, ntaps;
  int8_t tap_ky[V2V_MAX_TAPS], tap_kx[V2V_MAX_TAPS];
  int split;
  int headkx;
  int dgrad;
  bf16* out;
};

struct CompositeParams {
  void* const* io;
  int s_raw, s_flow, s_weight, s_prev, s_fg, s_mask, s_final;
  int s_raw_out;
  int prev_C;
  int N, H, W;
  int align_corners;
  int use_warp;
  int s_flags = -1;
};

struct PoolParams {
  ActDesc in, out;
};
struct FeatL1Params {
  ActDesc x, y;
  int Cvalid;
  void* const* io;
  int slot, index;
  double* partials;
  int blocks;
};

cudaError_t launch_raw_stats(const RawDesc& raw, stat_t* stats, int stats_C, cudaStream_t stream);

__device__ __forceinline__ void split_bf16(float x, bf16& hi, bf16& lo) {
  hi = __float2bfloat16_rn(x);
  lo = __float2bfloat16_rn(x - __bfloat162float(hi));
}
cudaError_t launch_stats_finalize(const FinalizeParams& p, cudaStream_t stream);
cudaError_t launch_norm_apply(const ApplyParams& p, cudaStream_t stream);
bool norm_apply_uses_rows(const ApplyParams& p);
cudaError_t launch_import_nchw(const ImportParams& p, cudaStream_t stream);
cudaError_t launch_export_nchw(const ExportParams& p, cudaStream_t stream);
cudaError_t launch_pack_weights(const PackParams& p, cudaStream_t stream);
cudaError_t launch_act_copy(const CopyParams& p, cudaStream_t stream);
cudaError_t launch_bias_affine(float* scale, float* shift, const float* bias, int N, int C, int stride, cudaStream_t stream);
cudaError_t launch_correlation(const float*, const float*, float*, int, int, int, int, int, int, int, int, int, cudaStream_t);
cudaError_t launch_composite(const CompositeParams& p, cudaStream_t stream);
bool composite_vec4(const CompositeParams& p);
bool composite_slots_aligned(const CompositeParams& p, void* const* io);
cudaError_t launch_maxpool2(const PoolParams& p, cudaStream_t stream);
cudaError_t launch_maxpool2_bwd(const PoolParams& p, const float* gout, float* gin, cudaStream_t stream);
cudaError_t launch_feature_l1(const FeatL1Params& p, cudaStream_t stream);
cudaError_t launch_feature_l1_bwd(const FeatL1Params& p, const float* g, float* gx, cudaStream_t stream);
int feature_l1_blocks(const ActDesc& x);
int device_sm_count();

}
```

### vid2vid_b200/model_g.py

```python
import collections
import contextlib
import os

import torch
import torch.nn as nn

from .base_model import HostScheduleMixin
from . import networks, ops


def _adam(params, **kw):
    params = list(params)
    if params and all(p.is_cuda for p in params):
        try:
            return torch.optim.Adam(params, fused=True, **kw)
        except (TypeError, RuntimeError):
            pass
    return torch.optim.Adam(params, **kw)


class Vid2VidModelG(HostScheduleMixin, nn.Module):
    def name(self):
        return 'Vid2VidModelG'

    def initialize(self, opt):
        self.opt = opt
        self.gpu_ids = opt.gpu_ids
        self.isTrain = opt.isTrain
        self.n_scales = opt.n_scales_spatial
        self.use_single_G = opt.use_single_G
        if getattr(opt, 'openpose_only', False):
            opt.no_flow = True
        dev = torch.device('cuda', self.gpu_ids[0] if len(self.gpu_ids) else torch.cuda.current_device())
        self.device_ = dev
        for s in range(self.n_scales):
            setattr(self, 'netG' + str(s), networks.build_netG(opt, s).to(dev))
        getattr(self, 'netG' + str(self.n_scales - 1)).input_exact_bf16 = bool(opt.label_nc != 0)
        if (not self.isTrain or getattr(opt, 'continue_train', False) or getattr(opt, 'load_pretrain', '')) and \
                not getattr(opt, 'synthetic_weights', False):
            for s in range(self.n_scales):
                self.load_network(getattr(self, 'netG' + str(s)), 'G' + str(s), opt.which_epoch, getattr(opt, 'load_pretrain', ''))
        self.netG_i = self.load_single_G() if self.use_single_G else None
        self.fake_B_prev = None
        if self.isTrain:
            self.init_train()
        return self

    def load_network(self, network, network_label, epoch_label, save_dir=''):
        save_filename = '%s_net_%s.pth' % (epoch_label, network_label)
        save_dir = save_dir or os.path.join(self.opt.checkpoints_dir, self.opt.name)
        save_path = os.path.join(save_dir, save_filename)
        if not os.path.isfile(save_path):
            print('%s not exists yet!' % save_path)
            if 'G0' in network_label:
                raise FileNotFoundError('Generator must exist! (%s)' % save_path)
            return
        sd = torch.load(save_path, map_location=self.device_)
        try:
            network.load_state_dict(sd)
        except Exception:
            own = network.state_dict()
            kept = {k: v for k, v in sd.items() if k in own and v.size() == own[k].size()}
            missing = sorted({k.split('.')[0] for k in own if k not in kept})
            print('Pretrained network %s: loaded %d of %d tensors; not initialised from the file: %s' % (
                network_label, len(kept), len(own), missing))
            own.update(kept)
            network.load_state_dict(own)

    def load_single_G(self):
        opt = self.opt
        if 'City' in opt.dataroot:
            single_path = 'checkpoints/label2city_single/'
            if opt.loadSize == 512:
                load_path, netG = single_path + 'latest_net_G_512.pth', networks.define_G(35, 3, 0, 64, 'global', 3, 'instance', 0, [], opt)
            elif opt.loadSize == 1024:
                load_path, netG = single_path + 'latest_net_G_1024.pth', networks.define_G(35, 3, 0, 64, 'global', 4, 'instance', 0, [], opt)
            elif opt.loadSize == 2048:
                load_path, netG = single_path + 'latest_net_G_2048.pth', networks.define_G(35, 3, 0, 32, 'local', 4, 'instance', 0, [], opt)
            else:
                raise ValueError('Single image generator does not exist')
        elif 'face' in opt.dataroot:
            single_path = 'checkpoints/edge2face_single/'
            load_path = single_path + 'latest_net_G.pth'
            opt.feat_num = 16
            netG = networks.define_G(15, 3, 0, 64, 'global_with_features', 3, 'instance', 0, [], opt)
            self.netE = self._load(networks.define_G(3, 16, 0, 16, 'encoder', 4, 'instance', 0, []), single_path + 'latest_net_E.pth')
            self.load_face_features(single_path + 'features.npy')
        else:
            raise ValueError('Single image generator does not exist')
        return self._load(netG, load_path)

    def _load(self, net, path):
        if not (getattr(self.opt, 'synthetic_weights', False) and not os.path.exists(path)):
            if not os.path.exists(path):
                raise FileNotFoundError('first-frame generator weights not found: %s' % path)
            net.load_state_dict(torch.load(path, map_location=self.device_))
        return net.to(self.device_)

    def load_face_features(self, path='checkpoints/edge2face_single/features.npy', features=None):
        if features is None:
            if os.path.exists(path):
                import numpy as np
                features = np.load(path, encoding='latin1', allow_pickle=True).item()
            elif getattr(self.opt, 'synthetic_weights', False):
                features = networks.synthetic_face_features(16, self.opt.feat_num, seed=0)
            else:
                raise FileNotFoundError('face features table not found: %s' % path)
        table, self.face_rows, self.face_num_images = networks.pack_face_features(features, self.opt.feat_num)
        self.face_table = table.to(self.device_)
        return features

    def encode_input(self, input_map, real_image, inst_map=None):
        size = input_map.size()
        self.bs, tG, self.height, self.width = size[0], size[1], size[3], size[4]
        input_map = input_map.to(self.device_, torch.float32)
        if self.opt.label_nc != 0:
            inst = inst_map.to(self.device_, torch.float32) if self.opt.use_instance else None
            input_map = ops.onehot_edges(input_map, inst, self.opt.label_nc, self.opt.use_instance)
        elif self.opt.use_instance:
            raise NotImplementedError('use_instance without label_nc')
        pool_map = None
        if self.opt.dataset_mode == 'face':
            pool_map = inst_map.to(self.device_, torch.float32)
        if real_image is not None:
            real_image = real_image.to(self.device_, torch.float32)
        return input_map, real_image, pool_map

    def build_pyr(self, tensor):
        if tensor is None:
            return [None] * self.n_scales
        pyr = [tensor]
        for _ in range(1, self.n_scales):
            pyr.append(ops.avgpool3s2(pyr[-1]))
        return pyr

    def compute_mask(self, real_As, ts, te=None):
        assert te is None or te == ts + 1
        return ops.fg_mask(real_As, ts, list(self.opt.fg_labels))

    def inference(self, input_A, input_B, inst_A):
        with torch.no_grad():
            real_A, real_B, pool_map = self.encode_input(input_A, input_B, inst_A)
            with self._per_clip_statistics(self.bs > 1):
                return self._inference(real_A, real_B, pool_map)

    @contextlib.contextmanager
    def _per_clip_statistics(self, on):
        nets = [getattr(self, 'netG' + str(s)) for s in range(self.n_scales)] + ([self.netG_i] if self.netG_i is not None else [])
        prev = [getattr(net, 'sample_stats', False) for net in nets]
        for net in nets:
            net.sample_stats = on
        try:
            yield
        finally:
            for net, p in zip(nets, prev):
                net.sample_stats = p

    def _inference(self, real_A, real_B, pool_map):
        self.is_first_frame = self.fake_B_prev is None
        if self.is_first_frame:
            self.fake_B_prev = self.generate_first_frame(real_A, real_B, pool_map)
        elif self.bs != self._clips():
            raise ValueError('this sequence was started with %d clip(s) and is fed %d: clips of one sequence start and advance '
                             'together (reset_stream() starts a new one)' % (self._clips(), self.bs))
        real_A = self.build_pyr(real_A)
        self.fake_B_feat = self.flow_feat = self.fake_B_fg_feat = None
        for s in range(self.n_scales):
            fake_B = self.generate_frame_infer(real_A[self.n_scales - 1 - s], s)
        return fake_B, (real_A[0][0, -1] if self.bs == 1 else real_A[0][:, -1])

    def _clips(self):
        return self.fake_B_prev[0].shape[0] if self.fake_B_prev[0].dim() == 5 else 1

    def reset_stream(self, clips=None):
        n = self._clips() if self.fake_B_prev is not None else 0
        if clips is not None and n > 1 and sorted(set(clips)) != list(range(n)):
            raise NotImplementedError('restarting clip(s) %s of a running batch of %d clips is not supported: the clips of a batch '
                                      'start and advance together; call reset_stream() to restart the whole batch, or use '
                                      'stream_slots(B), whose slots start and stop independently' % (list(clips), n))
        self.fake_B_prev = None
        self._win_A = self._win_I = None

    _DT = {torch.uint8: 0, torch.int32: 1, torch.float32: 2}

    def inference_stream(self, label_frame, inst_frame=None, out_u8=None):
        import ctypes as C
        from . import _lib as L
        if self.opt.dataset_mode == 'face' and self.use_single_G:
            raise ValueError('inference_stream does not take the real frames that the face first-frame generator needs '
                             '(use_single_G with dataset_mode face): use inference()')
        tG = self.opt.n_frames_G
        H, W = label_frame.shape[-2:]
        B = label_frame.shape[0] if label_frame.dim() == 3 else 1
        if inst_frame is not None and tuple(inst_frame.shape) != tuple(label_frame.shape):
            raise ValueError('inst_frame %s does not match label_frame %s' % (tuple(inst_frame.shape), tuple(label_frame.shape)))
        dev = self.device_
        if getattr(self, '_win_A', None) is not None and self._win_A.shape[0] != B:
            raise ValueError('this stream was started with %d clip(s) and is fed %d: clips of one stream start and advance '
                             'together (reset_stream() starts a new one)' % (self._win_A.shape[0], B))
        if getattr(self, '_win_A', None) is None or self._win_A.shape[-2:] != (H, W):
            self._win_A = torch.zeros(B, tG, 1, H, W, device=dev)
            self._win_I = torch.zeros(B, tG, 1, H, W, device=dev) if self.opt.use_instance else None
            self._win_n = 0
        for win, fr in ((self._win_A, label_frame), (self._win_I, inst_frame if inst_frame is not None else label_frame)):
            if win is None:
                continue
            fr = fr.to(dev, non_blocking=True).contiguous()
            if fr.dtype not in self._DT:
                raise TypeError('id maps must be uint8, int32 or float32')
            L.check(L.lib().v2v_ids_window_push(C.c_void_p(win.data_ptr()), C.c_void_p(fr.data_ptr()), self._DT[fr.dtype], B, tG, H,
                                                W, L.current_stream_ptr()))
            L.LAUNCHES[0] += 1
        self._win_n += 1
        if self._win_n < tG:
            return None
        fake_B, _ = self.inference(self._win_A, None, self._win_I)
        if out_u8 is None:
            return fake_B
        shape = (H, W, fake_B.shape[1]) if label_frame.dim() == 2 else (B, H, W, fake_B.shape[1])
        if getattr(self, '_u8_dev', None) is None or tuple(self._u8_dev.shape) != shape:
            self._u8_dev = torch.empty(shape, dtype=torch.uint8, device=dev)
        L.check(L.lib().v2v_tensor2im_u8(C.c_void_p(fake_B.data_ptr()), C.c_void_p(self._u8_dev.data_ptr()), B, fake_B.shape[1], H,
                                         W, L.current_stream_ptr()))
        L.LAUNCHES[0] += 1
        if out_u8.is_cuda:
            out_u8.copy_(self._u8_dev)
        else:
            out_u8.copy_(self._u8_dev, non_blocking=True)
        return out_u8

    def stream_slots(self, B):
        return SlotStream(self, B)

    def generate_frame_infer(self, real_A, s):
        tG = self.opt.n_frames_G
        b, _, _, h, w = real_A.size()
        si = self.n_scales - 1 - s
        netG_s = getattr(self, 'netG' + str(s))
        real_As_reshaped = real_A[:, :tG].reshape(b, -1, h, w)
        fake_B_prevs_reshaped = self.fake_B_prev[si].reshape(b, -1, h, w)
        mask_F = None
        if self.opt.fg:
            mask_F = self.compute_mask(real_A, tG - 1)
            mask_F = mask_F[0] if b == 1 else mask_F
        use_raw_only = self.opt.no_first_img and self.is_first_frame
        fake_B, flow, weight, fake_B_raw, self.fake_B_feat, self.flow_feat, self.fake_B_fg_feat = netG_s.forward(
            real_As_reshaped, fake_B_prevs_reshaped, mask_F, self.fake_B_feat, self.flow_feat, self.fake_B_fg_feat,
            use_raw_only)
        if b == 1:
            self.fake_B_prev[si] = torch.cat([self.fake_B_prev[si][1:, ...], fake_B])
        else:
            self.fake_B_prev[si] = torch.cat([self.fake_B_prev[si][:, 1:], fake_B.unsqueeze(1)], dim=1)
        return fake_B

    def generate_first_frame(self, real_A, real_B, pool_map=None):
        tG = self.opt.n_frames_G
        if self.opt.no_first_img:
            fake_B_prev = torch.zeros(self.bs, tG - 1, self.opt.output_nc, self.height, self.width, device=self.device_)
        elif self.opt.isTrain or self.opt.use_real_img:
            fake_B_prev = real_B[:, :(tG - 1), ...]
        elif self.opt.use_single_G:
            if self.opt.use_instance:
                real_A = real_A[:, :, :self.opt.label_nc, :, :]
            frames = []
            if self.opt.dataset_mode == 'face':
                self.netG_i.sample_stats = False
                for i in range(tG - 1):
                    frames.append(torch.cat([self.netG_i.forward(real_A[c:c + 1, i].contiguous(), self.get_face_features(
                        real_B[c:c + 1, i], pool_map[c:c + 1, i])) for c in range(self.bs)]).unsqueeze(1))
            else:
                for i in range(tG - 1):
                    frames.append(self.netG_i.forward(real_A[:, i].contiguous(), None).unsqueeze(1))
            fake_B_prev = torch.cat(frames, dim=1)
        else:
            raise ValueError('Please specify the method for generating the first frame')
        fake_B_prev = self.build_pyr(fake_B_prev)
        if not self.opt.isTrain and self.bs == 1:
            fake_B_prev = [B[0] for B in fake_B_prev]
        return fake_B_prev

    def get_face_features(self, real_image, inst):
        feat = self.netE.forward(real_image.contiguous(), inst.contiguous())
        feat_map, self.face_chosen = ops.face_features(feat, inst.contiguous(), self.face_table, self.face_rows, self.face_num_images)
        return feat_map

    def init_train(self):
        opt = self.opt
        self.n_gpus = 1
        self.n_frames_per_gpu = min(getattr(opt, 'max_frames_per_gpu', 1), opt.n_frames_total - opt.n_frames_G + 1)
        self.n_frames_load = self.n_gpus * self.n_frames_per_gpu
        self.n_frames_bp = 1
        self.finetune_all = getattr(opt, 'niter_fix_global', 0) == 0
        scales = range(self.n_scales) if self.finetune_all else [self.n_scales - 1]
        params = [p for s in scales for p in getattr(self, 'netG' + str(s)).parameters()]
        beta1, beta2, lr = (0.0, 0.9, opt.lr / 2) if opt.TTUR else (opt.beta1, 0.999, opt.lr)
        self.old_lr = opt.lr
        self.optimizer_G = _adam(params, lr=lr, betas=(beta1, beta2))
        return self

    def forward(self, input_A, input_B, inst_A, fake_B_prev, dummy_bs=0):
        tG = self.opt.n_frames_G
        real_A_all, real_B_all, _ = self.encode_input(input_A, input_B, inst_A)
        is_first_frame = fake_B_prev is None
        if is_first_frame:
            fake_B_prev = self.generate_first_frame(real_A_all, real_B_all)
        fake_B, fake_B_raw, flow, weight = self.generate_frame_train(real_A_all, fake_B_prev, is_first_frame)
        fake_B_prev = [B[:, -tG + 1:].detach() for B in fake_B]
        fake_B = [B[:, tG - 1:] for B in fake_B]
        return fake_B[0], fake_B_raw, flow, weight, real_A_all[:, tG - 1:], real_B_all[:, tG - 2:], fake_B_prev

    def generate_frame_train(self, real_A_all, fake_B_pyr, is_first_frame):
        tG, n_scales = self.opt.n_frames_G, self.n_scales
        if not hasattr(self, 'n_frames_load'):
            self.init_train()
        bs = real_A_all.shape[0]
        real_A_pyr = self.build_pyr(real_A_all)
        fake_B_pyr = list(fake_B_pyr)
        fake_Bs_raw, flows, weights = None, None, None
        cat = lambda a, b: b if a is None else torch.cat([a, b], dim=1)
        for t in range(self.n_frames_load):
            fake_B_feat = flow_feat = fake_B_fg_feat = None
            for s in range(n_scales):
                si = n_scales - 1 - s
                real_As = real_A_pyr[si]
                h, w = real_As.shape[-2:]
                real_As_reshaped = real_As[:, t:t + tG].reshape(bs, -1, h, w)
                fake_B_prevs = fake_B_pyr[si][:, t:t + tG - 1]
                if (t % self.n_frames_bp) == 0:
                    fake_B_prevs = fake_B_prevs.detach()
                fake_B_prevs_reshaped = fake_B_prevs.reshape(bs, -1, h, w)
                mask_F = self.compute_mask(real_As, t + tG - 1) if self.opt.fg else None
                use_raw_only = self.opt.no_first_img and is_first_frame
                frozen = s != n_scales - 1 and not self.finetune_all
                with torch.no_grad() if frozen else contextlib.nullcontext():
                    fake_B, flow, weight, fake_B_raw, fake_B_feat, flow_feat, fake_B_fg_feat = getattr(self, 'netG' + str(s)).forward(
                        real_As_reshaped, fake_B_prevs_reshaped, mask_F, fake_B_feat, flow_feat, fake_B_fg_feat, use_raw_only)
                fake_B_pyr[si] = cat(fake_B_pyr[si], fake_B.unsqueeze(1))
                if s == n_scales - 1:
                    fake_Bs_raw = cat(fake_Bs_raw, fake_B_raw.unsqueeze(1))
                    if flow is not None:
                        flows, weights = cat(flows, flow.unsqueeze(1)), cat(weights, weight.unsqueeze(1))
        return fake_B_pyr, fake_Bs_raw, flows, weights

    def save(self, label):
        for s in range(self.n_scales):
            self.save_network(getattr(self, 'netG' + str(s)), 'G' + str(s), label, self.gpu_ids)

    def compute_fake_B_prev(self, real_B_prev, fake_B_last, fake_B):
        fake_B_prev = real_B_prev[:, 0:1] if fake_B_last is None else fake_B_last[0][:, -1:]
        if fake_B.size()[1] > 1:
            fake_B_prev = torch.cat([fake_B_prev, fake_B[:, :-1].detach()], dim=1)
        return fake_B_prev


class SlotStep(collections.namedtuple('SlotStep', 'ops ready join raw_only')):

    def flags(self):
        from . import _lib as L
        return [(L.IMAGE_ACTIVE if r else 0) | (L.IMAGE_RAW_ONLY if o else 0) for r, o in zip(self.ready, self.raw_only)]


class SlotSchedule:

    def __init__(self, B, tG, no_first_img=False):
        from . import _lib as L
        if not 1 <= B <= L.MAX_SLOTS:
            raise ValueError('a slot stream has 1 to %d slots, not %d' % (L.MAX_SLOTS, B))
        self.B, self.tG, self.no_first_img = B, tG, bool(no_first_img)
        self.frames = [0] * B
        self._next = [None] * B

    def _slot(self, k):
        if isinstance(k, bool) or not isinstance(k, int) or not 0 <= k < self.B:
            raise IndexError('slot %r is out of range for a stream of %d slots' % (k, self.B))
        return k

    def start(self, k):
        self._next[self._slot(k)] = 'start'

    def stop(self, k):
        self._next[self._slot(k)] = 'stop'

    def step(self):
        from . import _lib as L
        ops = []
        for k in range(self.B):
            nxt, self._next[k] = self._next[k], None
            if nxt == 'start':
                self.frames[k] = 1
                ops.append(L.SLOT_RESTART)
            elif nxt == 'stop':
                self.frames[k] = 0
                ops.append(L.SLOT_CLEAR)
            elif self.frames[k]:
                self.frames[k] += 1
                ops.append(L.SLOT_PUSH)
            else:
                ops.append(L.SLOT_KEEP)
        ready = [n >= self.tG for n in self.frames]
        join = [n == self.tG for n in self.frames]
        return SlotStep(ops, ready, join, [j and self.no_first_img for j in join])


class SlotStream:

    def __init__(self, model, B):
        opt = model.opt
        if opt.dataset_mode == 'face' and model.use_single_G:
            raise ValueError('a slot stream does not take the real frames that the face first-frame generator needs '
                             '(use_single_G with dataset_mode face): use inference()')
        if not (opt.no_first_img or (model.use_single_G and not opt.use_real_img)):
            raise ValueError('a slot stream seeds the first frames of a joining clip with --no_first_img or --use_single_G '
                             '(it takes no real frames)')
        self.model, self.B, self.tG = model, B, opt.n_frames_G
        self.schedule = SlotSchedule(B, self.tG, opt.no_first_img)
        self.C = 1 if opt.label_nc != 0 else opt.input_nc
        self._win_A = self._win_I = self.fake_B_prev = self._flags = self._u8_dev = None

    def start(self, k):
        self.schedule.start(k)

    def stop(self, k):
        self.schedule.stop(k)

    def _check(self, frames, inst):
        B, opt = self.B, self.model.opt
        if opt.label_nc != 0:
            if frames.dim() != 3 or frames.shape[0] != B:
                raise ValueError('frames must be (%d, H, W) id maps, got %s' % (B, tuple(frames.shape)))
            if frames.dtype not in Vid2VidModelG._DT:
                raise TypeError('id maps must be uint8, int32 or float32')
        elif frames.dim() != 4 or tuple(frames.shape[:2]) != (B, self.C) or frames.dtype != torch.float32:
            raise ValueError('frames must be (%d, %d, H, W) float32, got %s %s' % (B, self.C, tuple(frames.shape), frames.dtype))
        if inst is not None and (tuple(inst.shape) != tuple(frames.shape) or inst.dtype not in Vid2VidModelG._DT):
            raise ValueError('inst %s does not match frames %s' % (tuple(inst.shape), tuple(frames.shape)))
        H, W = frames.shape[-2:]
        if self._win_A is not None and tuple(self._win_A.shape[-2:]) != (H, W):
            raise ValueError('this slot stream runs %dx%d frames, got %dx%d' % (self._win_A.shape[-2], self._win_A.shape[-1], H, W))
        return H, W

    def step(self, frames, inst=None, out_u8=None):
        import ctypes as C
        from . import _lib as L
        m, opt, B, tG = self.model, self.model.opt, self.B, self.tG
        H, W = self._check(frames, inst)
        dev = m.device_
        if self._win_A is None:
            self._win_A = torch.zeros(B, tG, self.C, H, W, device=dev)
            self._win_I = torch.zeros(B, tG, 1, H, W, device=dev) if opt.use_instance else None
            self.fake_B_prev, h, w = [], H, W
            for _ in range(m.n_scales):
                self.fake_B_prev.append(torch.zeros(B, tG - 1, opt.output_nc, h, w, device=dev))
                h, w = (h - 1) // 2 + 1, (w - 1) // 2 + 1
            self._flags = torch.zeros(B, dtype=torch.int32, device=dev)
        st = self.schedule.step()
        ops = (C.c_int * B)(*st.ops)
        for win, fr in ((self._win_A, frames), (self._win_I, inst if inst is not None else frames)):
            if win is None:
                continue
            fr = fr.to(dev, non_blocking=True).contiguous()
            L.check(L.lib().v2v_slots_window_push(C.c_void_p(win.data_ptr()), C.c_void_p(fr.data_ptr()), Vid2VidModelG._DT[fr.dtype],
                                                  B, tG, win.shape[2], H, W, ops, L.current_stream_ptr()))
            L.LAUNCHES[0] += 1
        self._flags.copy_(torch.tensor(st.flags(), dtype=torch.int32).pin_memory(), non_blocking=True)
        with torch.no_grad():
            real_A, _, _ = m.encode_input(self._win_A, None, self._win_I)
            for k in range(B):
                if st.join[k]:
                    self._seed_first_frames(real_A, k)
            real_A = m.build_pyr(real_A)
            feats = (None, None, None)
            with m._per_clip_statistics(True):
                for s in range(m.n_scales):
                    si = m.n_scales - 1 - s
                    ra = real_A[si]
                    h, w = ra.shape[-2:]
                    mask = m.compute_mask(ra, tG - 1) if opt.fg else None
                    fake_B, _, _, _, *feats = getattr(m, 'netG' + str(s)).forward(
                        ra[:, :tG].reshape(B, -1, h, w), self.fake_B_prev[si].reshape(B, -1, h, w), mask, *feats, False,
                        image_flags=self._flags)
                    self.fake_B_prev[si] = torch.cat([self.fake_B_prev[si][:, 1:], fake_B.unsqueeze(1)], dim=1)
        if out_u8 is None:
            return fake_B, st.ready
        if self._u8_dev is None or tuple(self._u8_dev.shape) != (B, H, W, fake_B.shape[1]):
            self._u8_dev = torch.empty(B, H, W, fake_B.shape[1], dtype=torch.uint8, device=dev)
        L.check(L.lib().v2v_tensor2im_u8(C.c_void_p(fake_B.data_ptr()), C.c_void_p(self._u8_dev.data_ptr()), B, fake_B.shape[1], H,
                                         W, L.current_stream_ptr()))
        L.LAUNCHES[0] += 1
        out_u8.copy_(self._u8_dev, non_blocking=not out_u8.is_cuda)
        return out_u8, st.ready

    def _seed_first_frames(self, real_A, k):
        m, opt = self.model, self.model.opt
        if opt.no_first_img:
            for prev in self.fake_B_prev:
                prev[k].zero_()
            return
        a = real_A[k:k + 1, :, :opt.label_nc] if opt.use_instance else real_A[k:k + 1]
        first = torch.cat([m.netG_i.forward(a[:, i].contiguous(), None).unsqueeze(1) for i in range(self.tG - 1)], dim=1)
        for prev, p in zip(self.fake_B_prev, m.build_pyr(first)):
            prev[k] = p[0]
```

### vid2vid_b200/networks.py

```python
import copy
import functools
import os
import sys

import torch
import torch.nn as nn

from . import _lib as L
from .plan import Plan, conv_desc, norm_desc


def weights_init(m):
    name = m.__class__.__name__
    if name.find('Conv') != -1 and hasattr(m, 'weight'):
        m.weight.data.normal_(0.0, 0.02)
    elif name.find('BatchNorm2d') != -1:
        m.weight.data.normal_(1.0, 0.02)
        m.bias.data.fill_(0)


def get_norm_layer(norm_type='instance'):
    if norm_type == 'batch':
        return functools.partial(nn.BatchNorm2d, affine=True)
    if norm_type == 'instance':
# ... 10 lines not shown
        netG = LocalEnhancer(input_nc, output_nc, ngf, n_downsampling, opt.n_blocks, opt.n_local_enhancers,
                             opt.n_blocks_local, norm_layer)
    elif which_model_netG == 'global_with_features':
        netG = Global_with_z(input_nc, output_nc, opt.feat_num, ngf, n_downsampling, opt.n_blocks, norm_layer)
    elif which_model_netG == 'encoder':
        netG = Encoder(input_nc, output_nc, ngf, n_downsampling, norm_layer)
    elif which_model_netG == 'local_with_features':
        raise NotImplementedError('Generator model name [local_with_features] (Local_with_z) is not implemented')
    elif which_model_netG == 'composite':
        netG = CompositeGenerator(opt, input_nc, output_nc, prev_output_nc, ngf, n_downsampling, opt.n_blocks,
                                  opt.fg, opt.no_flow, norm_layer)
    elif which_model_netG == 'compositeLocal':
        netG = CompositeLocalGenerator(opt, input_nc, output_nc, prev_output_nc, ngf, n_downsampling,
                                       opt.n_blocks_local, opt.fg, opt.no_flow, norm_layer, scale=scale)
    else:
        raise NotImplementedError('Generator model name [%s] is not recognized' % which_model_netG)
    if len(gpu_ids) > 0:
        netG.cuda(gpu_ids[0])
    netG.apply(weights_init)
    return netG


def define_D(input_nc, ndf, n_layers_D, norm='instance', num_D=1, getIntermFeat=False, gpu_ids=[]):
    netD = MultiscaleDiscriminator(input_nc, ndf, n_layers_D, get_norm_layer(norm), num_D, getIntermFeat)
    if len(gpu_ids) > 0:
        netD.cuda(gpu_ids[0])
    netD.apply(weights_init)
    return netD


def _stem(cin, cout, norm_layer):
    return [nn.ReflectionPad2d(3), nn.Conv2d(cin, cout, kernel_size=7, padding=0), norm_layer(cout), nn.ReLU(True)]


def _down(cin, cout, norm_layer):
    return [nn.Conv2d(cin, cout, kernel_size=3, stride=2, padding=1), norm_layer(cout), nn.ReLU(True)]


def _up(cin, cout, norm_layer):
    return [nn.ConvTranspose2d(cin, cout, kernel_size=3, stride=2, padding=1, output_padding=1), norm_layer(cout),
            nn.ReLU(True)]


def _head(cin, cout, act=None):
    return [nn.ReflectionPad2d(3), nn.Conv2d(cin, cout, kernel_size=7, padding=0)] + ([act] if act else [])


class ResnetBlock(nn.Module):

    def __init__(self, dim, padding_type, norm_layer, activation=nn.ReLU(True), use_dropout=False):
        super().__init__()
        if padding_type != 'reflect' or use_dropout:
            raise NotImplementedError('only reflect padding without dropout is used by vid2vid')
        self.conv_block = nn.Sequential(nn.ReflectionPad2d(1), nn.Conv2d(dim, dim, kernel_size=3, padding=0),
                                        norm_layer(dim), activation,
                                        nn.ReflectionPad2d(1), nn.Conv2d(dim, dim, kernel_size=3, padding=0),
                                        norm_layer(dim))


_ACTS = {nn.ReLU: (L.ACT_RELU, 0.0), nn.Tanh: (L.ACT_TANH, 0.0), nn.Sigmoid: (L.ACT_SIGMOID, 0.0)}


def _act_of(m):
    if isinstance(m, nn.LeakyReLU):
        return L.ACT_LRELU, m.negative_slope
    for k, v in _ACTS.items():
        if isinstance(m, k):
            return v
    return None


def _units(mods):
    units, i, pend = [], 0, None
    mods = list(mods)
    while i < len(mods):
        m = mods[i]
        if isinstance(m, nn.ReflectionPad2d):
            pend = m.padding[0]
            i += 1
        elif isinstance(m, (nn.Conv2d, nn.ConvTranspose2d)):
            norm, act, slope = None, L.ACT_NONE, 0.0
            j = i + 1
            if j < len(mods) and isinstance(mods[j], (nn.BatchNorm2d, nn.InstanceNorm2d)):
                norm = mods[j]
                j += 1
            if j < len(mods) and _act_of(mods[j]) is not None:
                act, slope = _act_of(mods[j])
                j += 1
            if pend is not None:
                units.append(('conv', m, L.PAD_REFLECT, pend, norm, act, slope))
            else:
                units.append(('conv', m, L.PAD_ZERO, None, norm, act, slope))
            pend, i = None, j
        elif isinstance(m, ResnetBlock):
            units.append(('res', m))
            i += 1
        else:
            raise NotImplementedError('cannot lower layer %r' % (m,))
    return units


def emit_seq(plan, mods, v, final_adds=(), defer_last=False):
    units = _units(mods)
    finish = None
    for k, u in enumerate(units):
        last = k == len(units) - 1
        adds = tuple(final_adds) if last else ()
        if u[0] == 'conv':
            _, conv, pmode, pad, norm, act, slope = u
            desc = conv_desc(conv, pmode, pad)
            if norm is None:
                if adds or (last and defer_last):
                    raise NotImplementedError('addends need a normalised unit')
                v = plan.conv_act(v, desc, act, slope)
            else:
                raw = plan.conv(v, desc)
                nd = norm_desc(norm)
                if last and defer_last:
                    finish = (lambda raw=raw, nd=nd, act=act, slope=slope: (lambda a: plan.norm_act(raw, nd, act, slope, a)))()
                else:
                    v = plan.norm_act(raw, nd, act, slope, adds)
        else:
            cb = u[1].conv_block
            raw1 = plan.conv(v, conv_desc(cb[1], L.PAD_REFLECT, 1))
            h = plan.norm_act(raw1, norm_desc(cb[2]), L.ACT_RELU, 0.0)
            raw2 = plan.conv(h, conv_desc(cb[5], L.PAD_REFLECT, 1))
            nd = norm_desc(cb[6])
            if last and defer_last:
                finish = (lambda raw2=raw2, nd=nd, v0=v: (lambda a: plan.norm_act(raw2, nd, L.ACT_NONE, 0.0, (v0,) + tuple(a))))()
            else:
                v = plan.norm_act(raw2, nd, L.ACT_NONE, 0.0, (v,) + adds)
    if defer_last:
        if finish is None:
            raise NotImplementedError('defer_last on an empty sequence')
        return finish
    return v


def emit_head(plan, mods, v, dst):
    (u,) = _units(mods)
    _, conv, pmode, pad, norm, act, slope = u
    assert norm is None
    slot, dst_c, scale = dst
    plan.head(v, conv_desc(conv, pmode, pad), [(slot, j, dst_c, act, scale) for j in range(conv.out_channels)])


def emit_head_pair(plan, mods_a, dst_a, mods_b, dst_b, v):
    (ua,), (ub,) = _units(mods_a), _units(mods_b)
    _, ca, pmode, pad, na, act_a, _ = ua
    _, cb, pmode_b, pad_b, nb, act_b, _ = ub
    assert na is None and nb is None and (pmode, pad) == (pmode_b, pad_b)
    chans = [(dst_a[0], j, dst_a[1], act_a, dst_a[2]) for j in range(ca.out_channels)]
    chans += [(dst_b[0], j, dst_b[1], act_b, dst_b[2]) for j in range(cb.out_channels)]
    plan.head(v, conv_desc(ca, pmode, pad, m2=cb), chans)


def emit_unit_pair(plan, mods_a, mods_b, v):
    (ua,), (ub,) = _units(mods_a), _units(mods_b)
    _, ca, pmode, pad, na, act_a, slope_a = ua
    _, cb, pmode_b, pad_b, nb, act_b, slope_b = ub
    assert na is not None and nb is not None and (pmode, pad) == (pmode_b, pad_b)
    raw = plan.conv(v, conv_desc(ca, pmode, pad, m2=cb))
    va = plan.norm_act(raw, norm_desc(na), act_a, slope_a, c_off=0, Cn=ca.out_channels)
    vb = plan.norm_act(raw, norm_desc(nb), act_b, slope_b, c_off=ca.out_channels, Cn=cb.out_channels)
    return va, vb


def _can_pair(mods_a, mods_b):
    ca, cb = mods_a[1], mods_b[1]
    return (isinstance(ca, nn.Conv2d) and isinstance(cb, nn.Conv2d) and ca.in_channels == cb.in_channels and
            ca.kernel_size == cb.kernel_size and ca.stride == cb.stride and ca.out_channels % 8 == 0)


class _PlanFunction(torch.autograd.Function):

    @staticmethod
    def forward(ctx, owner, plan, io, in_slots, out_slots, fixed_slots, *args):
        n_in = len(in_slots)
        ctx.plan, ctx.in_slots, ctx.out_slots, ctx.n_in, ctx.fixed = plan, in_slots, out_slots, n_in, set(fixed_slots)
        ctx.params = args[n_in:]
        plan.run(io, owner.use_cuda_graph)
        ctx.run_id = plan.run_id
        ctx.n_slots = len(io)
        ctx.io_slots = [i for i, t_ in enumerate(io) if t_ is not None]
        ctx.save_for_backward(*[io[i] for i in ctx.io_slots])
        return tuple(io[s] for s in out_slots)

    @staticmethod
    def backward(ctx, *gouts):
        plan = ctx.plan
        io = [None] * ctx.n_slots
        for i, t_ in zip(ctx.io_slots, ctx.saved_tensors):
            io[i] = t_
        if plan.run_id != ctx.run_id:
            scratch = list(io)
            for s_ in range(len(scratch)):
                if s_ not in ctx.fixed and scratch[s_] is not None:
                    scratch[s_] = torch.empty_like(scratch[s_])
            plan.run(scratch, False, recompute=True)
            io = scratch
        gio = [None] * len(io)
        for s_, g in zip(ctx.out_slots, gouts):
            if g is not None:
                gio[s_] = g.contiguous().float()
        gin = []
        for k, s_ in enumerate(ctx.in_slots):
            if ctx.needs_input_grad[6 + k] and io[s_] is not None:
                gio[s_] = torch.zeros_like(io[s_])
                gin.append(gio[s_])
            else:
                gin.append(None)
        if os.environ.get('V2V_DEBUG_AUTOGRAD'):
            print('plan backward: in_slots', ctx.in_slots, 'needs', ctx.needs_input_grad[6:6 + ctx.n_in], 'gin', [g is not None for g in gin])
        need = [bool(ctx.needs_input_grad[6 + ctx.n_in + j]) for j in range(len(ctx.params))]
        direct = [need[j] and p.grad is not None and p.grad.is_contiguous() and p.grad.dtype == torch.float32 and
                  p.grad.device == p.device for j, p in enumerate(ctx.params)]
        fresh = [j for j, p in enumerate(ctx.params) if need[j] and not direct[j]]
        pgrads, ret = [None] * len(ctx.params), [None] * len(ctx.params)
        if fresh:
            flat = torch.zeros(sum(ctx.params[j].numel() for j in fresh), device=ctx.params[fresh[0]].device, dtype=torch.float32)
            off = 0
            for j in fresh:
                n = ctx.params[j].numel()
                pgrads[j] = ret[j] = flat[off:off + n].view_as(ctx.params[j])
                off += n
        for j, p in enumerate(ctx.params):
            if direct[j]:
                pgrads[j] = p.grad
        plan.backward(io, gio, ctx.params, pgrads)
        return (None,) * 6 + tuple(gin) + tuple(ret)


DEFAULT_PRECISION = os.environ.get('V2V_PRECISION', 'precise')


def set_default_precision(mode):
    global DEFAULT_PRECISION
    assert mode in ('fast', 'precise')
    DEFAULT_PRECISION = mode


class _Planned(nn.Module):

    align_corners = False
    use_cuda_graph = True
    precision = None
    sample_stats = False

    def _precision(self):
        return self.precision or DEFAULT_PRECISION

    def _plans(self):
        if '_plan_cache' not in self.__dict__:
            self.__dict__['_plan_cache'] = {}
        return self.__dict__['_plan_cache']

    def _signature(self):
        ts = self.__dict__.get('_sig_tensors')
        if ts is None:
            ts = self.__dict__['_sig_tensors'] = list(self.parameters()) + list(self.buffers())
        ptrs, ver = 0, 0
        for t in ts:
            ptrs = (ptrs * 1000003 + t.data_ptr()) & 0xFFFFFFFFFFFF
            ver += t._version
        return ptrs, ver

    def _wants_grad(self, *tensors):
        if not torch.is_grad_enabled():
            return False
        return any(p.requires_grad for p in self.parameters()) or any(t is not None and t.requires_grad for t in tensors)

    def _get_plan(self, key, device, build, train=False):
        ptrs, ver = self._signature()
        key = key + (('train',) if train else ()) + (('sample_stats',) if self.sample_stats else ()) + (self._precision(),)
        ent = self._plans().get(key)
        if ent is not None and ent['ptrs'] != ptrs:
            ent = None
        if ent is None:
            if os.environ.get('V2V_LOG_PLANS'):
                print('v2v: building plan %s for %s (cached: %d)' % (key, type(self).__name__, len(self._plans())), file=sys.stderr, flush=True)
            plan = Plan(device.index if device.index is not None else torch.cuda.current_device(),
                        precision=self._precision(), train=train, sample_stats=self.sample_stats)
            build(plan)
            plan.finalize()
            ent = {'plan': plan, 'ptrs': ptrs, 'ver': ver}
            self._plans()[key] = ent
        elif ent['ver'] != ver:
            ent['plan'].repack()
            ent['ver'] = ver
        return ent['plan']

    @staticmethod
    def _require_cuda(*ts):
        for t in ts:
            if t is not None and (not t.is_cuda or t.dtype != torch.float32):
                raise RuntimeError('vid2vid_b200 modules run on CUDA fp32 tensors only (no CPU fallback)')

    def conv_macs(self, *shape_key):
        plan = Plan(0)
        self._describe(plan, *shape_key)
        return plan.conv_macs


S_IN, S_PREV, S_MASK, S_FINAL, S_FLOW, S_W, S_RAW, S_IMGF, S_FLOWF, S_FGF, S_FG, S_CI, S_CF, S_CG, S_RAWC, S_FLAGS = range(16)


class CompositeGenerator(_Planned):

    def __init__(self, opt, input_nc, output_nc, prev_output_nc, ngf, n_downsampling, n_blocks, use_fg_model=False,
                 no_flow=False, norm_layer=nn.BatchNorm2d, padding_type='reflect'):
        assert n_blocks >= 0
        super().__init__()
        self.opt = opt
        self.n_downsampling = n_downsampling
        self.use_fg_model = use_fg_model
        self.no_flow = no_flow
        self.input_nc, self.output_nc, self.prev_output_nc = input_nc, output_nc, prev_output_nc
        nd, mult = n_downsampling, 2 ** n_downsampling
        rb = lambda c: ResnetBlock(c, padding_type=padding_type, activation=nn.ReLU(True), norm_layer=norm_layer)

        if use_fg_model:
            c = ngf // 2 if nd > 2 else ngf
            indv_down = _stem(input_nc, c, norm_layer)
            for i in range(nd):
                indv_down += _down(c * 2 ** i, c * 2 ** (i + 1), norm_layer)
            indv_up = []
            for i in range(nd):
                indv_up += _up(c * 2 ** (nd - i), c * 2 ** (nd - i) // 2, norm_layer)
            self.indv_down = nn.Sequential(*indv_down)
            self.indv_res = nn.Sequential(*[rb(c * mult) for _ in range(n_blocks)])
            self.indv_up = nn.Sequential(*indv_up)
            self.indv_final = nn.Sequential(*_head(c, output_nc, nn.Tanh()))

        down_seg = _stem(input_nc, ngf, norm_layer)
        for i in range(nd):
            down_seg += _down(ngf * 2 ** i, ngf * 2 ** (i + 1), norm_layer)
        down_seg += [rb(ngf * mult) for _ in range(n_blocks - n_blocks // 2)]
        down_img = _stem(prev_output_nc, ngf, norm_layer) + copy.deepcopy(down_seg[4:])
        res_img = [rb(ngf * mult) for _ in range(n_blocks // 2)]
        up_img = []
        for i in range(nd):
            up_img += _up(ngf * 2 ** (nd - i), ngf * 2 ** (nd - i) // 2, norm_layer)

        self.model_down_seg = nn.Sequential(*down_seg)
        self.model_down_img = nn.Sequential(*down_img)
        self.model_res_img = nn.Sequential(*res_img)
        self.model_up_img = nn.Sequential(*up_img)
        self.model_final_img = nn.Sequential(*_head(ngf, output_nc, nn.Tanh()))
        if not no_flow:
            self.model_res_flow = copy.deepcopy(self.model_res_img)
            self.model_up_flow = copy.deepcopy(self.model_up_img)
            self.model_final_flow = nn.Sequential(*_head(ngf, 2))
            self.model_final_w = nn.Sequential(*_head(ngf, 1, nn.Sigmoid()))

    flow_multiplier = 20.0
    fuse_stems = True
    input_exact_bf16 = False

    def _describe(self, plan, N, H, W, use_raw_only=False):
        v_in = plan.input(S_IN, N, self.input_nc, 0, self.input_nc, H, W, exact_bf16=self.input_exact_bf16)
        v_prev = plan.input(S_PREV, N, self.prev_output_nc, 0, self.prev_output_nc, H, W)
        fg0 = None
        if self.use_fg_model and self.fuse_stems and _can_pair(self.model_down_seg, self.indv_down):
            seg0, fg0 = emit_unit_pair(plan, list(self.model_down_seg)[:4], list(self.indv_down)[:4], v_in)
            seg = emit_seq(plan, list(self.model_down_seg)[4:], seg0)
        else:
            seg = emit_seq(plan, self.model_down_seg, v_in)
        down = emit_seq(plan, self.model_down_img, v_prev, final_adds=(seg,))
        img_feat = emit_seq(plan, self.model_up_img, emit_seq(plan, self.model_res_img, down))
        plan.export(img_feat, S_IMGF)
        emit_head(plan, self.model_final_img, img_feat, (S_RAW, self.output_nc, 1.0))
        if not self.no_flow:
            flow_feat = emit_seq(plan, self.model_up_flow, emit_seq(plan, self.model_res_flow, down))
            plan.export(flow_feat, S_FLOWF)
            emit_head_pair(plan, self.model_final_flow, (S_FLOW, 2, self.flow_multiplier),
                           self.model_final_w, (S_W, 1, 1.0), flow_feat)
        if self.use_fg_model:
            fgd = emit_seq(plan, list(self.indv_down)[4:], fg0) if fg0 is not None else emit_seq(plan, self.indv_down, v_in)
            fg_feat = emit_seq(plan, self.indv_up, emit_seq(plan, self.indv_res, fgd))
            plan.export(fg_feat, S_FGF)
            emit_head(plan, self.indv_final, fg_feat, (S_FG, self.output_nc, 1.0))
        self._emit_composite(plan, N, H, W, use_raw_only)

    def _emit_composite(self, plan, N, H, W, use_raw_only):
        warp = not (use_raw_only or self.no_flow)
        plan.composite(S_RAW, S_FLOW if warp else -1, S_W if warp else -1, S_PREV if warp else -1, self.prev_output_nc,
                       S_FG if self.use_fg_model else -1, S_MASK if self.use_fg_model else -1, S_FINAL, N, H, W, warp,
                       self.align_corners, s_raw_out=S_RAWC if (plan.train and self.use_fg_model) else -1)

    def _run(self, key, coarse, input, img_prev, mask, use_raw_only, image_flags=None):
        self._require_cuda(input, img_prev, mask, *coarse)
        input, img_prev = input.contiguous(), img_prev.contiguous()
        N, _, H, W = input.shape
        if input.shape[1] != self.input_nc or img_prev.shape[1] != self.prev_output_nc or tuple(img_prev.shape[2:]) != (H, W):
            raise ValueError('netG input / img_prev shapes %s / %s do not match the module (%d / %d channels)' % (
                tuple(input.shape), tuple(img_prev.shape), self.input_nc, self.prev_output_nc))
        if self.use_fg_model and (mask is None or mask.numel() != N * H * W):
            raise ValueError('fg model needs a (N,1,H,W) mask')
        if self.output_nc != 3:
            raise NotImplementedError('the fused composite kernel handles 3 output channels')
        train = self._wants_grad(input, img_prev, *coarse)
        build = lambda p: self._describe(p, N, H, W, use_raw_only)
        if image_flags is not None:
            if train:
                raise RuntimeError('per-image flags are for inference plans: a slot plan has no gradient')
            if not self.sample_stats:
                raise ValueError('per-image flags need per-sample statistics (sample_stats = True)')
            if not image_flags.is_cuda or image_flags.dtype != torch.int32 or image_flags.numel() != N:
                raise ValueError('image_flags must be an int32 CUDA tensor of %d elements' % N)
            key = key + ('image_flags',)
            build = lambda p: (p.set_image_flags(S_FLAGS), self._describe(p, N, H, W, use_raw_only))
        plan = self._get_plan(key + (N, H, W, bool(use_raw_only), bool(self.align_corners), bool(self.input_exact_bf16)), input.device,
                              build, train=train)
        new = lambda c: torch.empty((N, c, H, W), device=input.device, dtype=torch.float32)
        io = [None] * 16
        io[S_FLAGS] = image_flags
        io[S_IN], io[S_PREV] = input, img_prev
        io[S_FINAL], io[S_RAW], io[S_IMGF] = new(self.output_nc), new(self.output_nc), new(self._feat_c())
        if not self.no_flow:
            io[S_FLOW], io[S_W], io[S_FLOWF] = new(2), new(1), new(self._feat_c())
        if self.use_fg_model:
            io[S_MASK] = mask.contiguous()
            io[S_FGF], io[S_FG] = new(self._fg_feat_c()), new(self.output_nc)
        for s, t in zip((S_CI, S_CF, S_CG), coarse):
            io[s] = t.contiguous() if t is not None else None
        if not train:
            plan.run(io, self.use_cuda_graph)
            return io[S_FINAL], io[S_FLOW], io[S_W], io[S_RAW], io[S_IMGF], io[S_FLOWF], io[S_FGF]
        raw_slot = S_RAW
        if self.use_fg_model:
            io[S_RAWC] = new(self.output_nc)
            raw_slot = S_RAWC
        in_slots = [s for s in (S_IN, S_PREV, S_CI, S_CF, S_CG) if io[s] is not None]
        out_slots = [s for s in (S_FINAL, S_FLOW, S_W, raw_slot, S_IMGF, S_FLOWF, S_FGF) if io[s] is not None]
        fixed = [s for s in (S_IN, S_PREV, S_MASK, S_CI, S_CF, S_CG) if io[s] is not None]
        params = [p for p in self.parameters()]
        outs = _PlanFunction.apply(self, plan, io, tuple(in_slots), tuple(out_slots), tuple(fixed),
                                   *([io[s] for s in in_slots] + params))
        res = dict(zip(out_slots, outs))
        return (res.get(S_FINAL), res.get(S_FLOW), res.get(S_W), res.get(raw_slot), res.get(S_IMGF), res.get(S_FLOWF),
                res.get(S_FGF))

    def _feat_c(self):
        return self.model_final_img[1].in_channels

    def _fg_feat_c(self):
        return self.indv_final[1].in_channels

    def forward(self, input, img_prev, mask, img_feat_coarse, flow_feat_coarse, img_fg_feat_coarse, use_raw_only, image_flags=None):
        return self._run(('G',), (), input, img_prev, mask, use_raw_only, image_flags)


class CompositeLocalGenerator(CompositeGenerator):

    def __init__(self, opt, input_nc, output_nc, prev_output_nc, ngf, n_downsampling, n_blocks_local,
                 use_fg_model=False, no_flow=False, norm_layer=nn.BatchNorm2d, padding_type='reflect', scale=1):
        _Planned.__init__(self)
        self.opt = opt
        self.use_fg_model = use_fg_model
        self.no_flow = no_flow
        self.scale = scale
        self.input_nc, self.output_nc, self.prev_output_nc = input_nc, output_nc, prev_output_nc
        rb = lambda c: ResnetBlock(c, padding_type=padding_type, activation=nn.ReLU(True), norm_layer=norm_layer)
        if use_fg_model:
            c = ngf // 2 if n_downsampling > 2 else ngf
            self.indv_down = nn.Sequential(*(_stem(input_nc, c, norm_layer) + _down(c, c * 2, norm_layer)))
            self.indv_up = nn.Sequential(*([rb(c * 2) for _ in range(n_blocks_local)] + _up(c * 2, c, norm_layer)))
            self.indv_final = nn.Sequential(*_head(c, output_nc, nn.Tanh()))
        self.model_down_seg = nn.Sequential(*(_stem(input_nc, ngf, norm_layer) + _down(ngf, ngf * 2, norm_layer)))
        self.model_down_img = nn.Sequential(*(_stem(prev_output_nc, ngf, norm_layer) + _down(ngf, ngf * 2, norm_layer)))
        self.model_up_img = nn.Sequential(*([rb(ngf * 2) for _ in range(n_blocks_local)] + _up(ngf * 2, ngf, norm_layer)))
        self.model_final_img = nn.Sequential(*_head(ngf, output_nc, nn.Tanh()))
        if not no_flow:
            self.model_up_flow = copy.deepcopy(self.model_up_img)
            self.model_final_flow = nn.Sequential(*_head(ngf, 2))
            self.model_final_w = nn.Sequential(*_head(ngf, 1, nn.Sigmoid()))

    def _describe(self, plan, N, H, W, use_raw_only=False):
        h2, w2 = H // 2, W // 2
        c2 = self.model_down_seg[4].out_channels
        v_in = plan.input(S_IN, N, self.input_nc, 0, self.input_nc, H, W, exact_bf16=self.input_exact_bf16)
        v_prev = plan.input(S_PREV, N, self.prev_output_nc, 0, self.prev_output_nc, H, W)
        ci = plan.input(S_CI, N, c2, 0, c2, h2, w2)
        fg0 = None
        if self.use_fg_model and self.fuse_stems and _can_pair(self.model_down_seg, self.indv_down):
            seg0, fg0 = emit_unit_pair(plan, list(self.model_down_seg)[:4], list(self.indv_down)[:4], v_in)
            seg = emit_seq(plan, list(self.model_down_seg)[4:], seg0)
        else:
            seg = emit_seq(plan, self.model_down_seg, v_in)
        fin = emit_seq(plan, self.model_down_img, v_prev, defer_last=True)
        img_feat = emit_seq(plan, self.model_up_img, fin((seg, ci)))
        plan.export(img_feat, S_IMGF)
        emit_head(plan, self.model_final_img, img_feat, (S_RAW, self.output_nc, 1.0))
        if not self.no_flow:
            cf = plan.input(S_CF, N, c2, 0, c2, h2, w2)
            flow_feat = emit_seq(plan, self.model_up_flow, fin((seg, cf)))
            plan.export(flow_feat, S_FLOWF)
            emit_head_pair(plan, self.model_final_flow, (S_FLOW, 2, 20.0 * (2 ** self.scale)),
                           self.model_final_w, (S_W, 1, 1.0), flow_feat)
        if self.use_fg_model:
            cg_c = self.indv_down[4].out_channels
            cg = plan.input(S_CG, N, cg_c, 0, cg_c, h2, w2)
            if fg0 is not None:
                fgd = emit_seq(plan, list(self.indv_down)[4:], fg0, final_adds=(cg,))
            else:
                fgd = emit_seq(plan, self.indv_down, v_in, final_adds=(cg,))
            fg_feat = emit_seq(plan, self.indv_up, fgd)
            plan.export(fg_feat, S_FGF)
            emit_head(plan, self.indv_final, fg_feat, (S_FG, self.output_nc, 1.0))
        self._emit_composite(plan, N, H, W, use_raw_only)

    def forward(self, input, img_prev, mask, img_feat_coarse, flow_feat_coarse, img_fg_feat_coarse, use_raw_only, image_flags=None):
        return self._run(('GL',), (img_feat_coarse, flow_feat_coarse, img_fg_feat_coarse), input, img_prev, mask,
                         use_raw_only, image_flags)


class GlobalGenerator(_Planned):

    def __init__(self, input_nc, output_nc, ngf=64, n_downsampling=3, n_blocks=9, norm_layer=nn.BatchNorm2d,
                 padding_type='reflect'):
        assert n_blocks >= 0
        super().__init__()
        cm = lambda c: min(1024, c)
        self.input_nc, self.output_nc = input_nc, output_nc
        model = _stem(input_nc, ngf, norm_layer)
        for i in range(n_downsampling):
            model += _down(cm(ngf * 2 ** i), cm(ngf * 2 ** (i + 1)), norm_layer)
        model += [ResnetBlock(cm(ngf * 2 ** n_downsampling), padding_type=padding_type, activation=nn.ReLU(True),
                              norm_layer=norm_layer) for _ in range(n_blocks)]
        for i in range(n_downsampling):
            m = 2 ** (n_downsampling - i)
            model += _up(cm(ngf * m), cm(int(ngf * m / 2)), norm_layer)
        model += _head(ngf, output_nc, nn.Tanh())
        self.model = nn.Sequential(*model)

    def _describe(self, plan, N, H, W):
        v = plan.input(0, N, self.input_nc, 0, self.input_nc, H, W)
        mods = list(self.model)
        v = emit_seq(plan, mods[:-3], v)
        emit_head(plan, mods[-3:], v, (1, self.output_nc, 1.0))

    def forward(self, input, feat=None):
        if feat is not None:
            input = torch.cat([input, feat], dim=1)
        self._require_cuda(input)
        input = input.contiguous()
        N, _, H, W = input.shape
        plan = self._get_plan(('GG', N, H, W), input.device, lambda p: self._describe(p, N, H, W))
        out = torch.empty((N, self.output_nc, H, W), device=input.device, dtype=torch.float32)
        plan.run([input, out], self.use_cuda_graph)
        return out


class Global_with_z(_Planned):

    def __init__(self, input_nc, output_nc, nz, ngf=64, n_downsample_G=3, n_blocks=9, norm_layer=nn.BatchNorm2d,
                 padding_type='reflect'):
        super().__init__()
        self.n_downsample_G = n_downsample_G
        self.input_nc, self.output_nc, self.nz = input_nc, output_nc, nz
        cm = lambda c: min(1024, c)
        model_downsample = _stem(input_nc + nz, ngf, norm_layer)
        for i in range(n_downsample_G):
            model_downsample += _down(cm(ngf * 2 ** i), cm(ngf * 2 ** (i + 1)), norm_layer)
        mult = 2 ** n_downsample_G
        model_resnet = [ResnetBlock(cm(ngf * mult) + nz, padding_type=padding_type, norm_layer=norm_layer) for _ in range(n_blocks)]
        model_upsample = []
        for i in range(n_downsample_G):
            mult = 2 ** (n_downsample_G - i)
            model_upsample += _up(cm(ngf * mult) + (nz * 2 if i == 0 else 0), cm(ngf * mult // 2), norm_layer)
        self.model_downsample = nn.Sequential(*model_downsample)
        self.model_resnet = nn.Sequential(*model_resnet)
        self.model_upsample = nn.Sequential(*model_upsample)
        self.model_upsample_conv = nn.Sequential(*_head(ngf + nz, output_nc, nn.Tanh()))
        self.downsample = nn.AvgPool2d(3, stride=2, padding=[1, 1], count_include_pad=False)

    def _z_dims(self, H, W):
        for _ in range(self.n_downsample_G):
            H, W = (H - 1) // 2 + 1, (W - 1) // 2 + 1
        return H, W

    def _describe(self, plan, N, H, W):
        cin = self.input_nc + self.nz
        v_xz = plan.input(0, N, cin, 0, cin, H, W)
        v_z = plan.input(0, N, cin, self.input_nc, self.nz, H, W)
        v_zd = plan.input(1, N, self.nz, 0, self.nz, *self._z_dims(H, W))
        down = emit_seq(plan, self.model_downsample, v_xz)
        res = emit_seq(plan, self.model_resnet, plan.concat([down, v_zd]))
        up = emit_seq(plan, self.model_upsample, plan.concat([res, v_zd]))
        emit_head(plan, self.model_upsample_conv, plan.concat([up, v_z]), (2, self.output_nc, 1.0))

    def forward(self, x, z):
        from . import ops
        self._require_cuda(x, z)
        if self._wants_grad(x, z):
            raise NotImplementedError('Global_with_z has no backward (the first-frame generator runs under no_grad)')
        N, _, H, W = x.shape
        if x.shape[1] != self.input_nc or tuple(z.shape) != (N, self.nz, H, W) or H % 2 ** self.n_downsample_G or W % 2 ** self.n_downsample_G:
            raise ValueError('Global_with_z: x %s / z %s do not fit (%d + %d channels, sides divisible by %d)' % (
                tuple(x.shape), tuple(z.shape), self.input_nc, self.nz, 2 ** self.n_downsample_G))
        z = z.contiguous()
        z_down = z
        for _ in range(self.n_downsample_G):
            z_down = ops.avgpool3s2(z_down)
        xz = torch.cat([x, z], dim=1)
        plan = self._get_plan(('GZ', N, H, W), x.device, lambda p: self._describe(p, N, H, W))
        out = torch.empty((N, self.output_nc, H, W), device=x.device, dtype=torch.float32)
        plan.run([xz, z_down, out], self.use_cuda_graph)
        return out


class Encoder(_Planned):

    n_ids = 7

    def __init__(self, input_nc, output_nc, ngf=32, n_downsampling=4, norm_layer=nn.BatchNorm2d):
        super().__init__()
        self.input_nc, self.output_nc = input_nc, output_nc
        model = _stem(input_nc, ngf, norm_layer)
        for i in range(n_downsampling):
            model += _down(ngf * 2 ** i, ngf * 2 ** (i + 1), norm_layer)
        for i in range(n_downsampling):
            mult = 2 ** (n_downsampling - i)
            model += _up(ngf * mult, int(ngf * mult / 2), norm_layer)
        model += _head(ngf, output_nc, nn.Tanh())
        self.model = nn.Sequential(*model)

    def _describe(self, plan, N, H, W):
        mods = list(self.model)
        v = emit_seq(plan, mods[:-3], plan.input(0, N, self.input_nc, 0, self.input_nc, H, W))
        emit_head(plan, mods[-3:], v, (1, self.output_nc, 1.0))

    def forward(self, input, inst):
        from . import ops
        self._require_cuda(input, inst)
        if self._wants_grad(input):
            raise NotImplementedError('Encoder has no backward (the face first frame runs under no_grad)')
        input = input.contiguous()
        N, _, H, W = input.shape
        plan = self._get_plan(('E', N, H, W), input.device, lambda p: self._describe(p, N, H, W))
        out = torch.empty((N, self.output_nc, H, W), device=input.device, dtype=torch.float32)
        plan.run([input, out], self.use_cuda_graph)
        return ops.instance_mean(out, inst.contiguous(), self.n_ids, out=out)


FACE_LABELS = 7


def synthetic_face_features(num_images, feat_num=16, seed=0, n_labels=FACE_LABELS):
    g = torch.Generator().manual_seed(seed)
    out = {}
    for label in range(n_labels):
        f = torch.rand((num_images, feat_num), generator=g, dtype=torch.float64) * 2 - 1
        out[label] = torch.cat([f, torch.arange(num_images, dtype=torch.float64)[:, None]], 1).float().double().numpy()
    return out


def pack_face_features(features, feat_num):
    labels = sorted(int(k) for k in features)
    if labels != list(range(len(labels))):
        raise ValueError('features table labels must be 0 .. n-1, got %s' % labels)
    arrs = [torch.as_tensor(features[k], dtype=torch.float32) for k in labels]
    if any(a.dim() != 2 or a.shape[1] < feat_num + 1 for a in arrs):
        raise ValueError('features table rows need feat_num + 1 = %d columns' % (feat_num + 1))
    rows = [a.shape[0] for a in arrs]
    table = torch.zeros(len(arrs), max(rows), feat_num + 1)
    for k, a in enumerate(arrs):
        table[k, :a.shape[0]] = a[:, :feat_num + 1]
    if len(rows) < FACE_LABELS:
        raise ValueError('features table has %d labels; the face parts are %d' % (len(rows), FACE_LABELS))
    return table, rows, rows[6]


class LocalEnhancer(_Planned):

    def __init__(self, input_nc, output_nc, ngf=32, n_downsample_global=3, n_blocks_global=9, n_local_enhancers=1,
                 n_blocks_local=3, norm_layer=nn.BatchNorm2d, padding_type='reflect'):
        super().__init__()
        self.n_local_enhancers = n_local_enhancers
        self.input_nc, self.output_nc = input_nc, output_nc
        g = GlobalGenerator(input_nc, output_nc, ngf * (2 ** n_local_enhancers), n_downsample_global, n_blocks_global,
                            norm_layer).model
        self.model = nn.Sequential(*[g[i] for i in range(len(g) - 3)])
        for n in range(1, n_local_enhancers + 1):
            c = ngf * (2 ** (n_local_enhancers - n))
            down = _stem(input_nc, c, norm_layer) + _down(c, c * 2, norm_layer)
            up = [ResnetBlock(c * 2, padding_type=padding_type, norm_layer=norm_layer) for _ in range(n_blocks_local)]
            up += _up(c * 2, c, norm_layer)
            if n == n_local_enhancers:
                up += _head(ngf, output_nc, nn.Tanh())
            setattr(self, 'model%d_1' % n, nn.Sequential(*down))
            setattr(self, 'model%d_2' % n, nn.Sequential(*up))
        self.downsample = nn.AvgPool2d(3, stride=2, padding=[1, 1], count_include_pad=False)

    def _describe(self, plan, N, H, W):
        L_ = self.n_local_enhancers
        dims = [(H, W)]
        for _ in range(L_):
            dims.append(((dims[-1][0] - 1) // 2 + 1, (dims[-1][1] - 1) // 2 + 1))
        out = emit_seq(plan, self.model, plan.input(L_, N, self.input_nc, 0, self.input_nc, *dims[L_]))
        for n in range(1, L_ + 1):
            lvl = L_ - n
            x = emit_seq(plan, getattr(self, 'model%d_1' % n),
                         plan.input(lvl, N, self.input_nc, 0, self.input_nc, *dims[lvl]), final_adds=(out,))
            mods = list(getattr(self, 'model%d_2' % n))
            if n == L_:
                out = emit_seq(plan, mods[:-3], x)
                emit_head(plan, mods[-3:], out, (L_ + 1, self.output_nc, 1.0))
            else:
                out = emit_seq(plan, mods, x)

    def forward(self, input, feat_map=None):
        from . import ops
        if feat_map is not None:
            input = torch.cat([input, feat_map], dim=1)
        self._require_cuda(input)
        pyr = [input.contiguous()]
        for _ in range(self.n_local_enhancers):
            pyr.append(ops.avgpool3s2(pyr[-1]))
        N, _, H, W = input.shape
        plan = self._get_plan(('LE', N, H, W), input.device, lambda p: self._describe(p, N, H, W))
        out = torch.empty((N, self.output_nc, H, W), device=input.device, dtype=torch.float32)
        plan.run(pyr + [out], self.use_cuda_graph)
        return out


class NLayerDiscriminator(nn.Module):

    def __init__(self, input_nc, ndf=64, n_layers=3, norm_layer=nn.BatchNorm2d, getIntermFeat=False):
        super().__init__()
        self.getIntermFeat, self.n_layers = getIntermFeat, n_layers
        kw, padw = 4, 2
        seq = [[nn.Conv2d(input_nc, ndf, kernel_size=kw, stride=2, padding=padw), nn.LeakyReLU(0.2, True)]]
        nf = ndf
        for n in range(1, n_layers):
            nf_prev, nf = nf, min(nf * 2, 512)
            seq += [[nn.Conv2d(nf_prev, nf, kernel_size=kw, stride=2, padding=padw), norm_layer(nf),
                     nn.LeakyReLU(0.2, True)]]
        nf_prev, nf = nf, min(nf * 2, 512)
        seq += [[nn.Conv2d(nf_prev, nf, kernel_size=kw, stride=1, padding=padw), norm_layer(nf), nn.LeakyReLU(0.2, True)]]
        seq += [[nn.Conv2d(nf, 1, kernel_size=kw, stride=1, padding=padw)]]
        if getIntermFeat:
            for n in range(len(seq)):
                setattr(self, 'model' + str(n), nn.Sequential(*seq[n]))
        else:
            self.model = nn.Sequential(*[m for s in seq for m in s])


class MultiscaleDiscriminator(_Planned):

    def __init__(self, input_nc, ndf=64, n_layers=3, norm_layer=nn.BatchNorm2d, num_D=3, getIntermFeat=False):
        super().__init__()
        self.num_D, self.n_layers, self.getIntermFeat = num_D, n_layers, getIntermFeat
        self.input_nc = input_nc
        for i in range(num_D):
            netD = NLayerDiscriminator(input_nc, min(64, ndf * (2 ** (num_D - 1 - i))), n_layers, norm_layer,
                                       getIntermFeat)
            if getIntermFeat:
                for j in range(n_layers + 2):
                    setattr(self, 'scale%d_layer%d' % (i, j), getattr(netD, 'model' + str(j)))
            else:
                setattr(self, 'layer' + str(i), netD.model)
        self.downsample = nn.AvgPool2d(3, stride=2, padding=[1, 1], count_include_pad=False)

    def _tower_layers(self, d):
        if self.getIntermFeat:
            return [list(getattr(self, 'scale%d_layer%d' % (d, j))) for j in range(self.n_layers + 2)]
        mods, layers, cur = list(getattr(self, 'layer' + str(d))), [], []
        for m in mods:
            if isinstance(m, nn.Conv2d) and cur:
                layers.append(cur)
                cur = []
            cur.append(m)
        layers.append(cur)
        return layers

    def _tower_params(self, d):
        return [p for mods in self._tower_layers(d) for m in mods for p in m.parameters()]

    def _describe(self, plan, d, N, H, W):
        layers = self._tower_layers(d)
        v = plan.input(0, N, self.input_nc, 0, self.input_nc, H, W)
        shapes = []
        for j, mods in enumerate(layers):
            last = j == len(layers) - 1
            conv = mods[0]
            oh = (H + 2 * conv.padding[0] - conv.kernel_size[0]) // conv.stride[0] + 1
            ow = (W + 2 * conv.padding[1] - conv.kernel_size[1]) // conv.stride[1] + 1
            if last:
                plan.head(v, conv_desc(conv), [(1 + j, 0, 1, L.ACT_NONE, 1.0)])
            else:
                v = emit_seq(plan, mods, v)
                if self.getIntermFeat:
                    plan.export(v, 1 + j)
            shapes.append((conv.out_channels, oh, ow))
            H, W = oh, ow
        return shapes

    def _tower_forward(self, d, x):
        N, _, H, W = x.shape
        key = ('D', d, N, H, W)
        shapes_box = {}

        def build(p):
            shapes_box['s'] = self._describe(p, d, N, H, W)
        train = self._wants_grad(x)
        plan = self._get_plan(key, x.device, build, train=train)
        shapes = self._plans()[key + (('train',) if train else ()) + (self._precision(),)].setdefault('shapes', shapes_box.get('s'))
        outs = [torch.empty((N, c, h, w), device=x.device, dtype=torch.float32) for (c, h, w) in shapes]
        io = [x] + [o if (self.getIntermFeat or j == len(outs) - 1) else None for j, o in enumerate(outs)]
        if not train:
            plan.run(io, self.use_cuda_graph)
            return outs if self.getIntermFeat else [outs[-1]]
        out_slots = tuple(s for s in range(1, len(io)) if io[s] is not None)
        params = [p for p in self._tower_params(d)]
        res = _PlanFunction.apply(self, plan, io, (0,), out_slots, (0,), *([x] + params))
        return list(res)
# ... 213 lines not shown
```

### vid2vid_b200/plan.py

```python
import ctypes as C
import json
import os

import torch
import torch.nn as nn

from . import _lib as L


def _ptr(t):
    return C.c_void_p(t.data_ptr()) if t is not None else C.c_void_p(None)


def conv_desc(m, pad_mode=L.PAD_ZERO, pad=None, m2=None):
    d = L.ConvDesc()
    tr = isinstance(m, nn.ConvTranspose2d)
    d.Cin, d.Cout = m.in_channels, m.out_channels
    d.kh, d.kw = m.kernel_size
    assert m.stride[0] == m.stride[1] and m.padding[0] == m.padding[1]
    d.stride = m.stride[0]
    d.pad = m.padding[0] if pad is None else pad
    d.pad_mode = pad_mode
    d.transposed = int(tr)
    d.output_padding = m.output_padding[0] if tr else 0
    d.weight = m.weight.data_ptr()
    d.bias = m.bias.data_ptr() if m.bias is not None else None
    if m2 is not None:
        assert (m2.in_channels, m2.kernel_size, m2.stride, m2.padding) == (m.in_channels, m.kernel_size, m.stride, m.padding)
        assert (m2.bias is None) == (m.bias is None)
        d.Cout = m.out_channels + m2.out_channels
        d.Cout2 = m2.out_channels
        d.weight2 = m2.weight.data_ptr()
        d.bias2 = m2.bias.data_ptr() if m2.bias is not None else None
    return d


def norm_desc(m):
    d = L.NormDesc()
    if m is None:
        d.kind = L.NORM_NONE
        return d
    d.kind = L.NORM_BATCH if isinstance(m, nn.BatchNorm2d) else L.NORM_INSTANCE
    d.gamma = m.weight.data_ptr() if getattr(m, 'weight', None) is not None else None
    d.beta = m.bias.data_ptr() if getattr(m, 'bias', None) is not None else None
    if getattr(m, 'running_mean', None) is not None:
        d.running_mean = m.running_mean.data_ptr()
        d.running_var = m.running_var.data_ptr()
        d.num_batches_tracked = m.num_batches_tracked.data_ptr()
    d.momentum = m.momentum if m.momentum is not None else 0.1
    d.eps = m.eps
    return d


class Plan:
    def __init__(self, device=0, impl=None, precision='fast', train=False, sample_stats=False):
        if impl is None:
            impl = L.IMPL_SIMT if os.environ.get('V2V_CONV_IMPL') == 'simt' else L.IMPL_UMMA
        self._h = C.c_void_p()
        self.device = device
        self.precision = precision
        L.check(L.lib().v2v_plan_create(device, impl, C.byref(self._h)))
        L.check(L.lib().v2v_plan_set_precision(self._h, {'fast': L.PREC_BF16, 'precise': L.PREC_BF16X3}[precision]))
        self.train = bool(train)
        if train:
            L.check(L.lib().v2v_plan_set_training(self._h, 1))
        self.sample_stats = bool(sample_stats)
        if sample_stats:
            L.check(L.lib().v2v_plan_set_sample_stats(self._h, 1))
        self.run_id = 0
        self._keep = []
        self.finalized = False
        self.n_slots = 0
        self._graph_ok = False

    def __del__(self):
        try:
            if self._h:
                L.lib().v2v_plan_destroy(self._h)
                self._h = None
        except Exception:
            pass

    def set_image_flags(self, slot):
        L.check(L.lib().v2v_plan_set_image_flags(self._h, slot))
        self.n_slots = max(self.n_slots, slot + 1)

    def input(self, slot, N, C_src, c_off, Cn, H, W, exact_bf16=False):
        v = C.c_int()
        L.check(L.lib().v2v_g_input_ex(self._h, slot, N, C_src, c_off, Cn, H, W, 1 if exact_bf16 else 0, C.byref(v)))
        self.n_slots = max(self.n_slots, slot + 1)
        return v.value

    def conv(self, vin, desc):
        r = C.c_int()
        self._keep.append(desc)
        L.check(L.lib().v2v_g_conv(self._h, vin, C.byref(desc), C.byref(r)))
        return r.value

    def norm_act(self, raw, ndesc, act=L.ACT_NONE, slope=0.0, adds=(), c_off=0, Cn=None):
        v = C.c_int()
        if len(adds) > 2:
            raise NotImplementedError('at most two addends per normalise pass')
        adds = list(adds) + [-1, -1]
        self._keep.append(ndesc)
        if Cn is None:
            L.check(L.lib().v2v_g_norm_act(self._h, raw, C.byref(ndesc), act, slope, adds[0], adds[1], C.byref(v)))
        else:
            L.check(L.lib().v2v_g_norm_act_slice(self._h, raw, c_off, Cn, C.byref(ndesc), act, slope, adds[0], adds[1],
                                                 C.byref(v)))
        return v.value

    def conv_act(self, vin, desc, act=L.ACT_NONE, slope=0.0):
        v = C.c_int()
        self._keep.append(desc)
        L.check(L.lib().v2v_g_conv_act(self._h, vin, C.byref(desc), act, slope, C.byref(v)))
        return v.value

    def head(self, vin, desc, channels):
        arr = (L.HeadChannel * len(channels))()
        for i, (slot, ch, dst_c, act, scale) in enumerate(channels):
            arr[i].slot, arr[i].channel, arr[i].dst_C, arr[i].act, arr[i].scale = slot, ch, dst_c, act, scale
            self.n_slots = max(self.n_slots, slot + 1)
        self._keep += [desc, arr]
        L.check(L.lib().v2v_g_head(self._h, vin, C.byref(desc), arr))

    def concat(self, values):
        arr = (C.c_int * len(values))(*values)
        v = C.c_int()
        L.check(L.lib().v2v_g_concat(self._h, arr, len(values), C.byref(v)))
        return v.value

    def correlation(self, va, vb, pad_size=20, kernel_size=1, max_displacement=20, stride1=1, stride2=2, act=L.ACT_NONE,
                    slope=0.0):
        v = C.c_int()
        L.check(L.lib().v2v_g_correlation(self._h, va, vb, pad_size, kernel_size, max_displacement, stride1, stride2, act, slope,
                                          C.byref(v)))
        return v.value

    def maxpool2(self, vin):
        v = C.c_int()
        L.check(L.lib().v2v_g_maxpool2(self._h, vin, C.byref(v)))
        return v.value

    def feature_l1(self, vx, vy, slot, index):
        L.check(L.lib().v2v_g_feature_l1(self._h, vx, vy, slot, index))
        self.n_slots = max(self.n_slots, slot + 1)

    def export(self, v, slot):
        L.check(L.lib().v2v_g_export(self._h, v, slot))
        self.n_slots = max(self.n_slots, slot + 1)

    def composite(self, s_raw, s_flow, s_weight, s_prev, prev_C, s_fg, s_mask, s_final, N, H, W, use_warp,
                  align_corners, s_raw_out=-1):
        L.check(L.lib().v2v_g_composite_ex(self._h, s_raw, s_flow, s_weight, s_prev, prev_C, s_fg, s_mask, s_final, s_raw_out,
                                           N, H, W, int(use_warp), int(align_corners)))
        self.n_slots = max(self.n_slots, s_raw + 1, s_flow + 1, s_weight + 1, s_prev + 1, s_fg + 1, s_mask + 1,
                           s_final + 1, s_raw_out + 1)

    def _stream(self):
        return C.c_void_p(torch.cuda.current_stream(self.device).cuda_stream)

    def finalize(self, workspace=None):
        if workspace is None:
            L.check(L.lib().v2v_plan_finalize(self._h, self._stream()))
        else:
            need = self.workspace_bytes
            base = (workspace.data_ptr() + 1023) // 1024 * 1024
            avail = workspace.data_ptr() + workspace.numel() * workspace.element_size() - base
            if avail < need:
                raise ValueError('workspace holds %d usable bytes, the plan needs %d' % (avail, need))
            self._workspace = workspace
            L.check(L.lib().v2v_plan_finalize_ws(self._h, C.c_void_p(base), need, self._stream()))
        self.finalized = True

    def repack(self):
        L.check(L.lib().v2v_plan_repack(self._h, self._stream()))

    def _io_array(self, io):
        arr = (C.c_void_p * self.n_slots)()
        for i in range(self.n_slots):
            t = io[i] if i < len(io) else None
            arr[i] = t.data_ptr() if t is not None else None
        return arr

    def run(self, io, use_graph=True, recompute=False):
        arr = self._io_array(io)
        g = 2 if recompute else int(use_graph and self._graph_ok)
        L.check(L.lib().v2v_plan_run(self._h, arr, self.n_slots, g, self._stream()))
        L.LAUNCHES[0] += self.num_kernels
        if not recompute:
            self._graph_ok = True
        self.last_io = io
        self.run_id += 1

    def backward(self, io, gio, params, grads):
        n = len(params)
        pa, ga = (C.c_void_p * max(n, 1))(), (C.c_void_p * max(n, 1))()
        for i, (p_, g_) in enumerate(zip(params, grads)):
            pa[i], ga[i] = p_.data_ptr(), (g_.data_ptr() if g_ is not None else None)
        L.check(L.lib().v2v_plan_backward(self._h, self._io_array(io), self._io_array(gio), self.n_slots, pa, ga, n,
                                          self._stream()))
        L.LAUNCHES[0] += 3 * self.num_kernels

    def profile(self, io=None):
        io = io if io is not None else self.last_io
        arr = (C.c_void_p * self.n_slots)()
        for i in range(self.n_slots):
            t = io[i] if i < len(io) else None
            arr[i] = t.data_ptr() if t is not None else None
        n = self.num_kernels + 4
        kinds, ms, macs, cnt = (C.c_int * n)(), (C.c_float * n)(), (C.c_double * n)(), C.c_int()
        L.check(L.lib().v2v_plan_profile(self._h, arr, self.n_slots, self._stream(), n, kinds, ms, macs,
                                         C.byref(cnt)))
        return [(kinds[i], ms[i], macs[i]) for i in range(cnt.value)]

    @property
    def num_kernels(self):
        return L.lib().v2v_plan_num_kernels(self._h)

    @property
    def conv_macs(self):
        return L.lib().v2v_plan_conv_macs(self._h)

    @property
    def workspace_bytes(self):
        return L.lib().v2v_plan_workspace_bytes(self._h)

    def describe(self):
        n = L.lib().v2v_plan_describe(self._h, None, 0)
        buf = C.create_string_buffer(int(n))
        L.lib().v2v_plan_describe(self._h, buf, n)
        return json.loads(buf.value.decode())
```

Baseline: 21.32.

## Build one-hot label pyramid input directly inside the generator plan

Adds a label-input graph op whose kernel reads raw label and instance maps and writes the one-hot, edge-map and avg-pooled pyramid levels straight into the padded bf16 activation buffer. It can also emit the foreground mask. This removes the separate one-hot, edge, pooling and import passes and their fp32 intermediate tensors. The cost is a more complex kernel that stages codes in shared memory and recomputes the pooled windows per output pixel, and it only applies to inference callers that pass label ids.

```diff
diff --git a/include/v2v_b200.h b/include/v2v_b200.h
--- a/include/v2v_b200.h
+++ b/include/v2v_b200.h
@@ -122,6 +122,8 @@
 int v2v_g_input(v2v_plan* plan, int slot, int N, int C_src, int c_off, int C, int H, int W, int* value_out);
 #define V2V_INPUT_EXACT_BF16 1
 int v2v_g_input_ex(v2v_plan* plan, int slot, int N, int C_src, int c_off, int C, int H, int W, int flags, int* value_out);
+int v2v_g_label_input(v2v_plan* plan, int s_labels, int s_inst, int N, int T, int tG, int label_nc, int level, int H0, int W0,
+                      int s_mask, const int* fg_labels, int n_fg, int flags, int* value_out);
 int v2v_g_conv(v2v_plan* plan, int value_in, const v2v_conv_desc* conv, int* raw_out);
 int v2v_g_norm_act(v2v_plan* plan, int raw_in, const v2v_norm_desc* norm, int act, float slope, int add0, int add1,
                    int* value_out);
diff --git a/vid2vid_b200/_lib.py b/vid2vid_b200/_lib.py
--- a/vid2vid_b200/_lib.py
+++ b/vid2vid_b200/_lib.py
@@ -40,7 +40,7 @@
     'v2v_resample_forward', 'v2v_onehot_edges', 'v2v_avgpool3s2', 'v2v_fg_mask',
     'v2v_l1_loss_forward', 'v2v_l1_loss_backward', 'v2v_mse_const_forward', 'v2v_mse_const_backward', 'v2v_avgpool3s2_backward',
     'v2v_resample_backward', 'v2v_avgpool2', 'v2v_avgpool2_backward', 'v2v_face_region', 'v2v_instance_mean', 'v2v_face_features', 'v2v_ids_window_push', 'v2v_slots_window_push', 'v2v_tensor2im_u8', 'v2v_flownet_prep', 'v2v_resize', 'v2v_sub_channels', 'v2v_flow_conf',
-    'v2v_plan_create', 'v2v_plan_destroy', 'v2v_plan_set_precision', 'v2v_g_input', 'v2v_g_input_ex', 'v2v_g_conv', 'v2v_g_norm_act', 'v2v_g_norm_act_slice', 'v2v_g_conv_act',
+    'v2v_plan_create', 'v2v_plan_destroy', 'v2v_plan_set_precision', 'v2v_g_input', 'v2v_g_input_ex', 'v2v_g_label_input', 'v2v_g_conv', 'v2v_g_norm_act', 'v2v_g_norm_act_slice', 'v2v_g_conv_act',
     'v2v_g_head', 'v2v_g_concat', 'v2v_g_correlation', 'v2v_g_maxpool2', 'v2v_g_feature_l1', 'v2v_g_export', 'v2v_g_composite', 'v2v_g_composite_ex', 'v2v_plan_set_training', 'v2v_plan_set_sample_stats', 'v2v_plan_set_image_flags', 'v2v_plan_backward', 'v2v_plan_finalize', 'v2v_plan_finalize_ws', 'v2v_plan_repack', 'v2v_plan_run',
     'v2v_plan_profile', 'v2v_plan_num_kernels', 'v2v_plan_conv_macs', 'v2v_plan_workspace_bytes', 'v2v_plan_describe',
     'v2v_conv_tap_table',
@@ -65,6 +65,7 @@
     l.v2v_plan_set_precision.argtypes = [C.c_void_p, C.c_int]
     l.v2v_g_input.argtypes = [C.c_void_p] + [C.c_int] * 7 + [C.POINTER(C.c_int)]
     l.v2v_g_input_ex.argtypes = [C.c_void_p] + [C.c_int] * 8 + [C.POINTER(C.c_int)]
+    l.v2v_g_label_input.argtypes = [C.c_void_p] + [C.c_int] * 10 + [C.POINTER(C.c_int), C.c_int, C.c_int, C.POINTER(C.c_int)]
     l.v2v_g_conv.argtypes = [C.c_void_p, C.c_int, C.POINTER(ConvDesc), C.POINTER(C.c_int)]
     l.v2v_g_norm_act.argtypes = [C.c_void_p, C.c_int, C.POINTER(NormDesc), C.c_int, C.c_float, C.c_int, C.c_int,
                                  C.POINTER(C.c_int)]
diff --git a/vid2vid_b200/csrc/plan.cu b/vid2vid_b200/csrc/plan.cu
--- a/vid2vid_b200/csrc/plan.cu
+++ b/vid2vid_b200/csrc/plan.cu
@@ -71,7 +71,7 @@
     const GOp& op = P->gops[i];
     bool ol = true;
     switch (op.kind) {
-      case G_INPUT: case G_RAWIN: case G_NORM_ACT: case G_CONV_ACT: case G_CONCAT: case G_CORR: case G_MAXPOOL:
+      case G_INPUT: case G_LABELS: case G_RAWIN: case G_NORM_ACT: case G_CONV_ACT: case G_CONCAT: case G_CORR: case G_MAXPOOL:
         ol = !dead(op.value_out); break;
       case G_CONV: ol = !(raw_uses[op.raw] > 0 && !raw_live[op.raw]); break;
       default: break;
@@ -172,6 +172,7 @@
 int run_xop(v2v_plan* P, const XOp& x, cudaStream_t s) {
   switch (x.kind) {
     case X_IMPORT: V2V_CUDA(launch_import_nchw(x.imp, s)); break;
+    case X_LABELS: V2V_CUDA(launch_label_input(x.lab, s)); break;
     case X_EXPORT: V2V_CUDA(launch_export_nchw(x.exp, s)); break;
     case X_FINALIZE: V2V_CUDA(launch_stats_finalize(x.fin, s)); break;
     case X_APPLY: V2V_CUDA(launch_norm_apply(x.app, s)); break;
@@ -299,6 +300,39 @@
   return 0;
 }
 
+int v2v_g_label_input(v2v_plan* p, int s_labels, int s_inst, int N, int T, int tG, int label_nc, int level, int H0, int W0, int s_mask,
+                      const int* fg_labels, int n_fg, int flags, int* value_out) {
+  V2V_REQUIRE(p && !p->lowered && value_out, V2V_ERR_STATE, "plan already lowered or null");
+  V2V_REQUIRE(!p->train, V2V_ERR_UNSUPPORTED, "label inputs are for inference plans (a training plan imports the one-hot pyramid)");
+  V2V_REQUIRE(s_labels >= 0 && s_inst != s_labels && N > 0 && tG > 0 && T >= tG && label_nc > 0 && label_nc < 0x7fff && H0 > 0 && W0 > 0,
+              V2V_ERR_INVALID,
+              "bad label input description");
+  V2V_REQUIRE(level >= 0 && level <= 2, V2V_ERR_UNSUPPORTED, "label input level %d: levels 0 to 2 only", level);
+  V2V_REQUIRE(!(flags & V2V_INPUT_EXACT_BF16) || level == 0, V2V_ERR_INVALID,
+              "label input level %d: pooled one-hot values are not exact in bf16", level);
+  V2V_REQUIRE(n_fg >= 0 && n_fg <= V2V_MAX_FG_LABELS && (s_mask >= 0) == (n_fg > 0) && (n_fg == 0 || fg_labels), V2V_ERR_INVALID,
+              "label input: a mask slot needs 1 to %d fg labels", V2V_MAX_FG_LABELS);
+  const int Cf = label_nc + (s_inst >= 0 ? 1 : 0);
+  GOp op; op.kind = G_LABELS;
+  LabelParams& l = op.lab;
+  l.s_labels = s_labels; l.s_inst = s_inst < 0 ? -1 : s_inst; l.s_mask = s_mask < 0 ? -1 : s_mask;
+  l.T = T; l.tG = tG; l.label_nc = label_nc; l.level = level; l.H0 = H0; l.W0 = W0; l.n_fg = n_fg;
+  for (int i = 0; i < n_fg; ++i) {
+    V2V_REQUIRE(fg_labels[i] >= 0 && fg_labels[i] < Cf, V2V_ERR_INVALID, "fg label %d out of range for %d channels", fg_labels[i], Cf);
+    l.fg[i] = fg_labels[i];
+  }
+  int H = H0, W = W0;
+  for (int i = 0; i < level; ++i) { H = (H - 1) / 2 + 1; W = (W - 1) / 2 + 1; }
+  op.value_out = new_value(p, N, H, W, tG * Cf);
+  V2V_REQUIRE(label_input_tile(p->values[op.value_out].Cp, tG, level) > 0, V2V_ERR_UNSUPPORTED,
+              "label input: %d channels do not fit a block", tG * Cf);
+  p->values[op.value_out].exact_bf16 = (flags & V2V_INPUT_EXACT_BF16) != 0;
+  p->n_slots = std::max({p->n_slots, s_labels + 1, s_inst + 1, s_mask + 1});
+  p->gops.push_back(op);
+  *value_out = op.value_out;
+  return 0;
+}
+
 static int check_conv(v2v_plan* p, int value_in, const v2v_conv_desc* c) {
   V2V_REQUIRE(p && !p->lowered && c, V2V_ERR_STATE, "plan already lowered or null");
   V2V_REQUIRE(value_in >= 0 && value_in < (int)p->values.size(), V2V_ERR_INVALID, "bad value id %d", value_in);
@@ -519,6 +553,19 @@
           x.imp.c_off = op.c_off; x.imp.C_src = op.C_src;
           x.imp.out = P->acts[v.bufs[m]]; x.imp.pad_mode = P->act_pad_mode[v.bufs[m]];
           x.imp.skip_lo = v.exact_bf16 ? 1 : 0;
+          P->xops.push_back(x);
+        }
+        break;
+      }
+      case G_LABELS: {
+        const Value& v = P->values[op.value_out];
+        for (size_t m = 0; m < v.bufs.size(); ++m) {
+          XOp x; x.kind = X_LABELS; x.gop = (int)i;
+          x.lab = op.lab;
+          x.lab.io = P->io_dev;
+          x.lab.out = P->acts[v.bufs[m]]; x.lab.pad_mode = P->act_pad_mode[v.bufs[m]];
+          x.lab.skip_lo = v.exact_bf16 ? 1 : 0;
+          if (m > 0) x.lab.s_mask = -1;
           P->xops.push_back(x);
         }
         break;
diff --git a/vid2vid_b200/csrc/plan_internal.h b/vid2vid_b200/csrc/plan_internal.h
--- a/vid2vid_b200/csrc/plan_internal.h
+++ b/vid2vid_b200/csrc/plan_internal.h
@@ -71,7 +71,8 @@
   bool no_stats = false;
 };
 
-enum GKind { G_INPUT, G_CONV, G_NORM_ACT, G_CONV_ACT, G_HEAD, G_EXPORT, G_COMPOSITE, G_CONCAT, G_CORR, G_RAWIN, G_MAXPOOL, G_FEATL1 };
+enum GKind { G_INPUT, G_CONV, G_NORM_ACT, G_CONV_ACT, G_HEAD, G_EXPORT, G_COMPOSITE, G_CONCAT, G_CORR, G_RAWIN, G_MAXPOOL, G_FEATL1,
+             G_LABELS };
 struct GOp {
   GKind kind;
   int slot = -1, C_src = 0, c_off = 0;
@@ -91,6 +92,7 @@
   int corr[5] = {0, 0, 0, 0, 0};
   const float* ext_raw = nullptr; int ext_C = 0;
   int pack_dgrad = 0; const float* dg_w2 = nullptr; int dg_Cout1 = 0;
+  LabelParams lab{};
   bf16* wpacked = nullptr; int Ktotal = 0, Cp = 0;
   float* gdz = nullptr;
   double macs = 0.0;
@@ -98,7 +100,8 @@
   ConvKernelParams kp{};
 };
 
-enum XKind { X_IMPORT, X_CONV, X_RAWSTATS, X_FINALIZE, X_APPLY, X_EXPORT, X_COMPOSITE, X_MEMSET, X_COPY, X_CORR, X_MAXPOOL, X_FEATL1 };
+enum XKind { X_IMPORT, X_CONV, X_RAWSTATS, X_FINALIZE, X_APPLY, X_EXPORT, X_COMPOSITE, X_MEMSET, X_COPY, X_CORR, X_MAXPOOL, X_FEATL1,
+             X_LABELS };
 struct XOp {
   XKind kind;
   int gop = -1;
@@ -111,6 +114,7 @@
   CorrParams corr{};
   PoolParams pool{};
   FeatL1Params fl1{};
+  LabelParams lab{};
   RawDesc rawd{}; stat_t* stats = nullptr; int stats_C = 0;
   void* ms_ptr = nullptr; size_t ms_bytes = 0;
 };
diff --git a/vid2vid_b200/csrc/pyramid.cu b/vid2vid_b200/csrc/pyramid.cu
--- a/vid2vid_b200/csrc/pyramid.cu
+++ b/vid2vid_b200/csrc/pyramid.cu
@@ -139,6 +139,188 @@
   }
 }
 
+__device__ __forceinline__ int label_at(const float* lp, size_t pix, int label_nc) {
+  const int l = (int)__ldg(lp + pix);
+  return (l >= 0 && l < label_nc) ? l : -1;
+}
+__device__ __forceinline__ bool edge_at(const float* ip, int y, int x, int H, int W) {
+  const size_t pix = (size_t)y * W + x;
+  const float v = __ldg(ip + pix);
+  bool e = false;
+  if (x > 0) e |= (__ldg(ip + pix - 1) != v);
+  if (x < W - 1) e |= (__ldg(ip + pix + 1) != v);
+  if (y > 0) e |= (__ldg(ip + pix - W) != v);
+  if (y < H - 1) e |= (__ldg(ip + pix + W) != v);
+  return e;
+}
+__device__ __forceinline__ int code_label(uint16_t c) { return (int)(c & 0x7fff) - 1; }
+struct Window0 { int lab[9]; int n, ne; };
+__device__ __forceinline__ void window0(const uint16_t* codes, int cols, int y0_lo, int x0_lo, int y1, int x1, int H0, int W0,
+                                        Window0& w) {
+  w.n = 0; w.ne = 0;
+#pragma unroll
+  for (int dy = -1; dy <= 1; ++dy)
+#pragma unroll
+    for (int dx = -1; dx <= 1; ++dx) {
+      const int y = 2 * y1 + dy, x = 2 * x1 + dx, k = (dy + 1) * 3 + dx + 1;
+      const bool in = y >= 0 && y < H0 && x >= 0 && x < W0;
+      const uint16_t c = in ? codes[(y - y0_lo) * cols + (x - x0_lo)] : 0;
+      w.lab[k] = code_label(c);
+      if (in) { ++w.n; w.ne += c >> 15; }
+    }
+}
+__device__ __forceinline__ int reflect_px(int i, int n) {
+  if (i < 0) i = -i;
+  if (i >= n) i = 2 * (n - 1) - i;
+  return i;
+}
+__host__ __device__ __forceinline__ int label_stage_rows(int level) { return level == 1 ? 3 : (level == 2 ? 7 : 0); }
+__host__ __device__ __forceinline__ int label_stage_cols(int level, int TPX) { return level == 1 ? 2 * TPX + 1 : 4 * TPX + 3; }
+static size_t label_input_smem(int C, int tG, int level, int TPX) {
+  return (size_t)TPX * (C + 1) * sizeof(float) + (size_t)tG * label_stage_rows(level) * label_stage_cols(level, TPX) * sizeof(uint16_t);
+}
+
+template <int LEVEL>
+__global__ void __launch_bounds__(256) label_input_kernel(LabelParams p, int TPX) {
+  extern __shared__ float vals[];
+  __shared__ int xrange[2];
+  const ActDesc& o = p.out;
+  const int stride = o.C + 1;
+  const int Cf = p.label_nc + (p.s_inst >= 0 ? 1 : 0);
+  const int Wpad = o.W + o.pad_l + o.pad_r, Hpad = o.H + o.pad_t + o.pad_b;
+  const int xt = blockIdx.x * TPX;
+  const int yp = blockIdx.y % Hpad, n = blockIdx.y / Hpad;
+  const float* labels = reinterpret_cast<const float*>(p.io[p.s_labels]);
+  const float* inst = p.s_inst >= 0 ? reinterpret_cast<const float*>(p.io[p.s_inst]) : nullptr;
+  const size_t HW0 = (size_t)p.H0 * p.W0;
+  const int rows = label_stage_rows(LEVEL), cols = label_stage_cols(LEVEL, TPX);
+  uint16_t* codes = reinterpret_cast<uint16_t*>(vals + TPX * stride);
+  const bool yhalo = yp < o.pad_t || yp >= o.pad_t + o.H;
+  const int y = reflect_px(yp - o.pad_t, o.H);
+  for (int i = threadIdx.x; i < TPX * stride; i += blockDim.x) vals[i] = 0.f;
+  if (LEVEL > 0) {
+    if (threadIdx.x == 0) { xrange[0] = 0x7fffffff; xrange[1] = -1; }
+    __syncthreads();
+    if (threadIdx.x < TPX && xt + (int)threadIdx.x < Wpad && (!yhalo || p.pad_mode == PAD_REFLECT)) {
+      const int x = xt + (int)threadIdx.x - o.pad_l;
+      if ((x >= 0 && x < o.W) || p.pad_mode == PAD_REFLECT) {
+        atomicMin(&xrange[0], reflect_px(x, o.W));
+        atomicMax(&xrange[1], reflect_px(x, o.W));
+      }
+    }
+    __syncthreads();
+    const int y0_lo = LEVEL == 1 ? 2 * y - 1 : 4 * y - 3, x0_lo = LEVEL == 1 ? 2 * xrange[0] - 1 : 4 * xrange[0] - 3;
+    const int ncols = xrange[1] < xrange[0] ? 0 : (LEVEL == 1 ? 2 : 4) * (xrange[1] - xrange[0]) + (LEVEL == 1 ? 3 : 7);
+    for (int i = threadIdx.x; i < p.tG * rows * ncols; i += blockDim.x) {
+      const int c = i % ncols, r = (i / ncols) % rows, f = i / (ncols * rows);
+      const int y0 = y0_lo + r, x0 = x0_lo + c;
+      uint16_t code = 0;
+      if (y0 >= 0 && y0 < p.H0 && x0 >= 0 && x0 < p.W0) {
+        const size_t plane = ((size_t)n * p.T + f) * HW0;
+        code = (uint16_t)(label_at(labels + plane, (size_t)y0 * p.W0 + x0, p.label_nc) + 1);
+        if (inst && edge_at(inst + plane, y0, x0, p.H0, p.W0)) code |= 0x8000;
+      }
+      codes[(f * rows + r) * cols + c] = code;
+    }
+  }
+  __syncthreads();
+  const int y0_lo = LEVEL == 1 ? 2 * y - 1 : 4 * y - 3, x0_lo = LEVEL == 1 ? 2 * xrange[0] - 1 : 4 * xrange[0] - 3;
+  for (int it = threadIdx.x; it < TPX * p.tG; it += blockDim.x) {
+    const int px = it % TPX, f = it / TPX;
+    const int xp = xt + px;
+    if (xp >= Wpad) continue;
+    int x = xp - o.pad_l;
+    const bool halo = yhalo || x < 0 || x >= o.W;
+    if (halo && p.pad_mode != PAD_REFLECT) continue;
+    x = reflect_px(x, o.W);
+    float* v = vals + px * stride + f * Cf;
+    if (LEVEL == 0) {
+      const float* lp = labels + ((size_t)n * p.T + f) * HW0;
+      const int l = label_at(lp, (size_t)y * p.W0 + x, p.label_nc);
+      if (l >= 0) v[l] = 1.f;
+      if (inst) v[p.label_nc] = edge_at(inst + ((size_t)n * p.T + f) * HW0, y, x, p.H0, p.W0) ? 1.f : 0.f;
+    } else if (LEVEL == 1) {
+      Window0 w;
+      window0(codes + f * rows * cols, cols, y0_lo, x0_lo, y, x, p.H0, p.W0, w);
+#pragma unroll
+      for (int k = 0; k < 9; ++k) if (w.lab[k] >= 0) v[w.lab[k]] += 1.f;
+      if (inst) v[p.label_nc] = (float)w.ne;
+      for (int c = 0; c < Cf; ++c) v[c] = v[c] / (float)w.n;
+    } else {
+      const int H1 = (p.H0 - 1) / 2 + 1, W1 = (p.W0 - 1) / 2 + 1;
+      int n2 = 0;
+      for (int dy = -1; dy <= 1; ++dy) {
+        const int y1 = 2 * y + dy;
+        if (y1 < 0 || y1 >= H1) continue;
+        for (int dx = -1; dx <= 1; ++dx) {
+          const int x1 = 2 * x + dx;
+          if (x1 < 0 || x1 >= W1) continue;
+          ++n2;
+          Window0 w;
+          window0(codes + f * rows * cols, cols, y0_lo, x0_lo, y1, x1, p.H0, p.W0, w);
+          const float n1 = (float)w.n;
+#pragma unroll
+          for (int k = 0; k < 9; ++k) {
+            const int l = w.lab[k];
+            if (l < 0) continue;
+            bool first = true;
+            int m = 0;
+#pragma unroll
+            for (int k2 = 0; k2 < 9; ++k2)
+              if (w.lab[k2] == l) { first &= k2 >= k; ++m; }
+            if (first) v[l] += (float)m / n1;
+          }
+          if (inst && w.ne) v[p.label_nc] += (float)w.ne / n1;
+        }
+      }
+      for (int c = 0; c < Cf; ++c) v[c] = v[c] / (float)n2;
+    }
+    if (p.s_mask >= 0 && f == p.tG - 1 && !halo) {
+      float s = 0.f;
+      for (int i = 0; i < p.n_fg; ++i) s += v[p.fg[i]];
+      float* mask = reinterpret_cast<float*>(p.io[p.s_mask]);
+      mask[((size_t)n * o.H + y) * o.W + x] = fminf(fmaxf(s, 0.f), 1.f);
+    }
+  }
+  __syncthreads();
+  const int groups = o.C / 8;
+  const bool lo_half = o.split && !p.skip_lo;
+  for (int i = threadIdx.x; i < TPX * groups; i += blockDim.x) {
+    const int px = i / groups, c = 8 * (i - px * groups);
+    const int xo = xt + px;
+    if (xo >= Wpad) continue;
+    const float* f = vals + px * stride + c;
+    uint32_t hi[4], lo[4];
+#pragma unroll
+    for (int j = 0; j < 4; ++j) {
+      const float f0 = f[2 * j], f1 = f[2 * j + 1];
+      hi[j] = pack_bf16x2(f0, f1);
+      lo[j] = pack_bf16x2(f0 - __bfloat162float(__float2bfloat16_rn(f0)), f1 - __bfloat162float(__float2bfloat16_rn(f1)));
+    }
+    bf16* d = o.base + o.offset(n, yp - o.pad_t, xo - o.pad_l) + c;
+    *reinterpret_cast<uint4*>(d) = make_uint4(hi[0], hi[1], hi[2], hi[3]);
+    if (lo_half) *reinterpret_cast<uint4*>(d + o.C) = make_uint4(lo[0], lo[1], lo[2], lo[3]);
+  }
+}
+
+int label_input_tile(int C, int tG, int level) {
+  for (int t = 64; t >= 16; t >>= 1)
+    if (label_input_smem(C, tG, level, t) <= 48 * 1024) return t;
+  return 0;
+}
+
+cudaError_t launch_label_input(const LabelParams& p, cudaStream_t s) {
+  const ActDesc& o = p.out;
+  const int TPX = label_input_tile(o.C, p.tG, p.level);
+  const int Wpad = o.W + o.pad_l + o.pad_r, Hpad = o.H + o.pad_t + o.pad_b;
+  dim3 grid((Wpad + TPX - 1) / TPX, Hpad * o.N);
+  const size_t smem = label_input_smem(o.C, p.tG, p.level, TPX);
+  if (p.level == 0) label_input_kernel<0><<<grid, 256, smem, s>>>(p, TPX);
+  else if (p.level == 1) label_input_kernel<1><<<grid, 256, smem, s>>>(p, TPX);
+  else label_input_kernel<2><<<grid, 256, smem, s>>>(p, TPX);
+  return cudaGetLastError();
+}
+
 static inline int grid1d(size_t total) {
   size_t b = (total + 255) / 256;
   const size_t cap = 132 * 16;
diff --git a/vid2vid_b200/csrc/v2v_internal.h b/vid2vid_b200/csrc/v2v_internal.h
--- a/vid2vid_b200/csrc/v2v_internal.h
+++ b/vid2vid_b200/csrc/v2v_internal.h
@@ -167,6 +167,17 @@
   int pad_mode;
   int skip_lo;
 };
+#define V2V_MAX_FG_LABELS 16
+struct LabelParams {
+  void* const* io;
+  int s_labels, s_inst;
+  int s_mask;
+  int T, tG, label_nc, level, H0, W0;
+  int fg[V2V_MAX_FG_LABELS], n_fg;
+  ActDesc out;
+  int pad_mode;
+  int skip_lo;
+};
 struct ExportParams {
   void* const* io;
   int slot;
@@ -231,6 +242,8 @@
 cudaError_t launch_norm_apply(const ApplyParams& p, cudaStream_t stream);
 bool norm_apply_uses_rows(const ApplyParams& p);
 cudaError_t launch_import_nchw(const ImportParams& p, cudaStream_t stream);
+cudaError_t launch_label_input(const LabelParams& p, cudaStream_t stream);
+int label_input_tile(int C, int tG, int level);
 cudaError_t launch_export_nchw(const ExportParams& p, cudaStream_t stream);
 cudaError_t launch_pack_weights(const PackParams& p, cudaStream_t stream);
 cudaError_t launch_act_copy(const CopyParams& p, cudaStream_t stream);
diff --git a/vid2vid_b200/model_g.py b/vid2vid_b200/model_g.py
--- a/vid2vid_b200/model_g.py
+++ b/vid2vid_b200/model_g.py
@@ -7,6 +7,7 @@
 
 from .base_model import HostScheduleMixin
 from . import networks, ops
+from .plan import simt_selected
 
 
 def _adam(params, **kw):
@@ -139,10 +140,34 @@
         return ops.fg_mask(real_As, ts, list(self.opt.fg_labels))
 
     def inference(self, input_A, input_B, inst_A):
+        return self._infer(input_A, input_B, inst_A, True)
+
+    def _label_ids(self):
+        return self.opt.label_nc != 0 and not simt_selected()
+
+    def _label_input(self, label_ids, inst_ids):
+        inst = inst_ids.to(self.device_, torch.float32).contiguous() if self.opt.use_instance else None
+        return networks.LabelInput(label_ids.to(self.device_, torch.float32).contiguous(), inst, self.opt.label_nc,
+                                   self.opt.fg_labels)
+
+    def _infer(self, input_A, input_B, inst_A, want_label_frame):
         with torch.no_grad():
-            real_A, real_B, pool_map = self.encode_input(input_A, input_B, inst_A)
+            if not self._label_ids():
+                real_A, real_B, pool_map = self.encode_input(input_A, input_B, inst_A)
+                with self._per_clip_statistics(self.bs > 1):
+                    return self._inference(real_A, real_B, pool_map)
+            labels = self._label_input(input_A, inst_A)
+            self.bs, self.height, self.width = labels.N, labels.H0, labels.W0
+            real_A = real_B = pool_map = None
+            if self.fake_B_prev is None:
+                real_A, real_B, pool_map = self.encode_input(input_A, input_B, inst_A)
             with self._per_clip_statistics(self.bs > 1):
-                return self._inference(real_A, real_B, pool_map)
+                fake_B, _ = self._inference(real_A, real_B, pool_map, labels)
+            if not want_label_frame:
+                return fake_B, None
+            last = lambda t: t[:, -1:].contiguous() if t is not None else None
+            frame = ops.onehot_edges(last(labels.labels), last(labels.inst), self.opt.label_nc, self.opt.use_instance)
+            return fake_B, (frame[0, 0] if self.bs == 1 else frame[:, 0])
 
     @contextlib.contextmanager
     def _per_clip_statistics(self, on):
@@ -156,15 +181,19 @@
             for net, p in zip(nets, prev):
                 net.sample_stats = p
 
-    def _inference(self, real_A, real_B, pool_map):
+    def _inference(self, real_A, real_B, pool_map, labels=None):
         self.is_first_frame = self.fake_B_prev is None
         if self.is_first_frame:
             self.fake_B_prev = self.generate_first_frame(real_A, real_B, pool_map)
         elif self.bs != self._clips():
             raise ValueError('this sequence was started with %d clip(s) and is fed %d: clips of one sequence start and advance '
                              'together (reset_stream() starts a new one)' % (self._clips(), self.bs))
+        self.fake_B_feat = self.flow_feat = self.fake_B_fg_feat = None
+        if labels is not None:
+            for s in range(self.n_scales):
+                fake_B = self.generate_frame_infer(None, s, labels.at(self.n_scales - 1 - s))
+            return fake_B, None
         real_A = self.build_pyr(real_A)
-        self.fake_B_feat = self.flow_feat = self.fake_B_fg_feat = None
         for s in range(self.n_scales):
             fake_B = self.generate_frame_infer(real_A[self.n_scales - 1 - s], s)
         return fake_B, (real_A[0][0, -1] if self.bs == 1 else real_A[0][:, -1])
@@ -214,7 +243,7 @@
         self._win_n += 1
         if self._win_n < tG:
             return None
-        fake_B, _ = self.inference(self._win_A, None, self._win_I)
+        fake_B, _ = self._infer(self._win_A, None, self._win_I, False)
         if out_u8 is None:
             return fake_B
         shape = (H, W, fake_B.shape[1]) if label_frame.dim() == 2 else (B, H, W, fake_B.shape[1])
@@ -232,21 +261,24 @@
     def stream_slots(self, B):
         return SlotStream(self, B)
 
-    def generate_frame_infer(self, real_A, s):
+    def generate_frame_infer(self, real_A, s, labels=None):
         tG = self.opt.n_frames_G
-        b, _, _, h, w = real_A.size()
         si = self.n_scales - 1 - s
         netG_s = getattr(self, 'netG' + str(s))
-        real_As_reshaped = real_A[:, :tG].reshape(b, -1, h, w)
+        real_As_reshaped = mask_F = None
+        if labels is not None:
+            b, h, w = labels.N, labels.H, labels.W
+        else:
+            b, _, _, h, w = real_A.size()
+            real_As_reshaped = real_A[:, :tG].reshape(b, -1, h, w)
+            if self.opt.fg:
+                mask_F = self.compute_mask(real_A, tG - 1)
+                mask_F = mask_F[0] if b == 1 else mask_F
         fake_B_prevs_reshaped = self.fake_B_prev[si].reshape(b, -1, h, w)
-        mask_F = None
-        if self.opt.fg:
-            mask_F = self.compute_mask(real_A, tG - 1)
-            mask_F = mask_F[0] if b == 1 else mask_F
         use_raw_only = self.opt.no_first_img and self.is_first_frame
         fake_B, flow, weight, fake_B_raw, self.fake_B_feat, self.flow_feat, self.fake_B_fg_feat = netG_s.forward(
             real_As_reshaped, fake_B_prevs_reshaped, mask_F, self.fake_B_feat, self.flow_feat, self.fake_B_fg_feat,
-            use_raw_only)
+            use_raw_only, labels=labels)
         if b == 1:
             self.fake_B_prev[si] = torch.cat([self.fake_B_prev[si][1:, ...], fake_B])
         else:
@@ -464,21 +496,29 @@
             L.LAUNCHES[0] += 1
         self._flags.copy_(torch.tensor(st.flags(), dtype=torch.int32).pin_memory(), non_blocking=True)
         with torch.no_grad():
-            real_A, _, _ = m.encode_input(self._win_A, None, self._win_I)
+            labels = m._label_input(self._win_A, self._win_I) if m._label_ids() else None
+            real_A = None
+            if labels is None or (any(st.join) and not opt.no_first_img):
+                real_A, _, _ = m.encode_input(self._win_A, None, self._win_I)
             for k in range(B):
                 if st.join[k]:
                     self._seed_first_frames(real_A, k)
-            real_A = m.build_pyr(real_A)
+            real_A = m.build_pyr(real_A) if labels is None else None
             feats = (None, None, None)
             with m._per_clip_statistics(True):
                 for s in range(m.n_scales):
                     si = m.n_scales - 1 - s
-                    ra = real_A[si]
-                    h, w = ra.shape[-2:]
-                    mask = m.compute_mask(ra, tG - 1) if opt.fg else None
+                    inp = mask = lab = None
+                    if labels is not None:
+                        lab = labels.at(si)
+                        h, w = lab.H, lab.W
+                    else:
+                        ra = real_A[si]
+                        h, w = ra.shape[-2:]
+                        inp = ra[:, :tG].reshape(B, -1, h, w)
+                        mask = m.compute_mask(ra, tG - 1) if opt.fg else None
                     fake_B, _, _, _, *feats = getattr(m, 'netG' + str(s)).forward(
-                        ra[:, :tG].reshape(B, -1, h, w), self.fake_B_prev[si].reshape(B, -1, h, w), mask, *feats, False,
-                        image_flags=self._flags)
+                        inp, self.fake_B_prev[si].reshape(B, -1, h, w), mask, *feats, False, image_flags=self._flags, labels=lab)
                     self.fake_B_prev[si] = torch.cat([self.fake_B_prev[si][:, 1:], fake_B.unsqueeze(1)], dim=1)
         if out_u8 is None:
             return fake_B, st.ready
diff --git a/vid2vid_b200/networks.py b/vid2vid_b200/networks.py
--- a/vid2vid_b200/networks.py
+++ b/vid2vid_b200/networks.py
@@ -336,7 +336,29 @@
         return plan.conv_macs
 
 
-S_IN, S_PREV, S_MASK, S_FINAL, S_FLOW, S_W, S_RAW, S_IMGF, S_FLOWF, S_FGF, S_FG, S_CI, S_CF, S_CG, S_RAWC, S_FLAGS = range(16)
+S_IN, S_PREV, S_MASK, S_FINAL, S_FLOW, S_W, S_RAW, S_IMGF, S_FLOWF, S_FGF, S_FG, S_CI, S_CF, S_CG, S_RAWC, S_FLAGS, S_LABELS, S_INST = \
+    range(18)
+
+
+class LabelInput:
+
+    def __init__(self, labels, inst, label_nc, fg_labels, level=0):
+        if labels.dim() != 5 or labels.shape[2] != 1 or (inst is not None and inst.shape != labels.shape):
+            raise ValueError('label / instance id windows must be (N, T, 1, H, W), got %s / %s' % (
+                tuple(labels.shape), None if inst is None else tuple(inst.shape)))
+        self.labels, self.inst, self.label_nc, self.fg_labels, self.level = labels, inst, label_nc, tuple(fg_labels), level
+        self.N, self.T = labels.shape[:2]
+        self.H0, self.W0 = labels.shape[-2:]
+        h, w = self.H0, self.W0
+        for _ in range(level):
+            h, w = (h - 1) // 2 + 1, (w - 1) // 2 + 1
+        self.H, self.W = h, w
+
+    def at(self, level):
+        return LabelInput(self.labels, self.inst, self.label_nc, self.fg_labels, level)
+
+    def key(self):
+        return ('ids', self.T, self.level, self.H0, self.W0, self.label_nc, self.inst is not None, self.fg_labels)
 
 
 class CompositeGenerator(_Planned):
@@ -391,8 +413,18 @@
     fuse_stems = True
     input_exact_bf16 = False
 
-    def _describe(self, plan, N, H, W, use_raw_only=False):
-        v_in = plan.input(S_IN, N, self.input_nc, 0, self.input_nc, H, W, exact_bf16=self.input_exact_bf16)
+    def _stem_input(self, plan, N, H, W, ids):
+        if ids is None:
+            return plan.input(S_IN, N, self.input_nc, 0, self.input_nc, H, W, exact_bf16=self.input_exact_bf16)
+        cf = ids.label_nc + (ids.inst is not None)
+        if self.input_nc % cf:
+            raise ValueError('label input: %d input channels are not whole frames of %d channels' % (self.input_nc, cf))
+        return plan.label_input(S_LABELS, S_INST if ids.inst is not None else -1, N, ids.T, self.input_nc // cf, ids.label_nc,
+                                ids.level, ids.H0, ids.W0, S_MASK if self.use_fg_model else -1,
+                                ids.fg_labels if self.use_fg_model else (), exact_bf16=self.input_exact_bf16)
+
+    def _describe(self, plan, N, H, W, use_raw_only=False, ids=None):
+        v_in = self._stem_input(plan, N, H, W, ids)
         v_prev = plan.input(S_PREV, N, self.prev_output_nc, 0, self.prev_output_nc, H, W)
         fg0 = None
         if self.use_fg_model and self.fuse_stems and _can_pair(self.model_down_seg, self.indv_down):
@@ -422,19 +454,32 @@
                        S_FG if self.use_fg_model else -1, S_MASK if self.use_fg_model else -1, S_FINAL, N, H, W, warp,
                        self.align_corners, s_raw_out=S_RAWC if (plan.train and self.use_fg_model) else -1)
 
-    def _run(self, key, coarse, input, img_prev, mask, use_raw_only, image_flags=None):
-        self._require_cuda(input, img_prev, mask, *coarse)
-        input, img_prev = input.contiguous(), img_prev.contiguous()
-        N, _, H, W = input.shape
-        if input.shape[1] != self.input_nc or img_prev.shape[1] != self.prev_output_nc or tuple(img_prev.shape[2:]) != (H, W):
-            raise ValueError('netG input / img_prev shapes %s / %s do not match the module (%d / %d channels)' % (
-                tuple(input.shape), tuple(img_prev.shape), self.input_nc, self.prev_output_nc))
-        if self.use_fg_model and (mask is None or mask.numel() != N * H * W):
-            raise ValueError('fg model needs a (N,1,H,W) mask')
+    def _run(self, key, coarse, input, img_prev, mask, use_raw_only, image_flags=None, labels=None):
+        if labels is not None:
+            if input is not None or mask is not None:
+                raise ValueError('netG takes either an input tensor (and mask) or label ids, not both')
+            self._require_cuda(labels.labels, labels.inst, img_prev, *coarse)
+            img_prev = img_prev.contiguous()
+            N, H, W = labels.N, labels.H, labels.W
+            if img_prev.shape[1] != self.prev_output_nc or tuple(img_prev.shape[2:]) != (H, W):
+                raise ValueError('netG img_prev shape %s does not match the module (%d channels) at %dx%d' % (
+                    tuple(img_prev.shape), self.prev_output_nc, H, W))
+            if self._wants_grad(img_prev, *coarse):
+                raise RuntimeError('label-id inputs are for inference: a training forward takes the one-hot input tensor')
+            key = key + labels.key()
+        else:
+            self._require_cuda(input, img_prev, mask, *coarse)
+            input, img_prev = input.contiguous(), img_prev.contiguous()
+            N, _, H, W = input.shape
+            if input.shape[1] != self.input_nc or img_prev.shape[1] != self.prev_output_nc or tuple(img_prev.shape[2:]) != (H, W):
+                raise ValueError('netG input / img_prev shapes %s / %s do not match the module (%d / %d channels)' % (
+                    tuple(input.shape), tuple(img_prev.shape), self.input_nc, self.prev_output_nc))
+            if self.use_fg_model and (mask is None or mask.numel() != N * H * W):
+                raise ValueError('fg model needs a (N,1,H,W) mask')
         if self.output_nc != 3:
             raise NotImplementedError('the fused composite kernel handles 3 output channels')
         train = self._wants_grad(input, img_prev, *coarse)
-        build = lambda p: self._describe(p, N, H, W, use_raw_only)
+        build = lambda p: self._describe(p, N, H, W, use_raw_only, labels)
         if image_flags is not None:
             if train:
                 raise RuntimeError('per-image flags are for inference plans: a slot plan has no gradient')
@@ -443,13 +488,17 @@
             if not image_flags.is_cuda or image_flags.dtype != torch.int32 or image_flags.numel() != N:
                 raise ValueError('image_flags must be an int32 CUDA tensor of %d elements' % N)
             key = key + ('image_flags',)
-            build = lambda p: (p.set_image_flags(S_FLAGS), self._describe(p, N, H, W, use_raw_only))
-        plan = self._get_plan(key + (N, H, W, bool(use_raw_only), bool(self.align_corners), bool(self.input_exact_bf16)), input.device,
+            build = lambda p: (p.set_image_flags(S_FLAGS), self._describe(p, N, H, W, use_raw_only, labels))
+        plan = self._get_plan(key + (N, H, W, bool(use_raw_only), bool(self.align_corners), bool(self.input_exact_bf16)), img_prev.device,
                               build, train=train)
-        new = lambda c: torch.empty((N, c, H, W), device=input.device, dtype=torch.float32)
-        io = [None] * 16
+        new = lambda c: torch.empty((N, c, H, W), device=img_prev.device, dtype=torch.float32)
+        io = [None] * 18
         io[S_FLAGS] = image_flags
         io[S_IN], io[S_PREV] = input, img_prev
+        if labels is not None:
+            io[S_LABELS], io[S_INST] = labels.labels, labels.inst
+            if self.use_fg_model:
+                mask = new(1)
         io[S_FINAL], io[S_RAW], io[S_IMGF] = new(self.output_nc), new(self.output_nc), new(self._feat_c())
         if not self.no_flow:
             io[S_FLOW], io[S_W], io[S_FLOWF] = new(2), new(1), new(self._feat_c())
@@ -481,8 +530,9 @@
     def _fg_feat_c(self):
         return self.indv_final[1].in_channels
 
-    def forward(self, input, img_prev, mask, img_feat_coarse, flow_feat_coarse, img_fg_feat_coarse, use_raw_only, image_flags=None):
-        return self._run(('G',), (), input, img_prev, mask, use_raw_only, image_flags)
+    def forward(self, input, img_prev, mask, img_feat_coarse, flow_feat_coarse, img_fg_feat_coarse, use_raw_only, image_flags=None,
+                labels=None):
+        return self._run(('G',), (), input, img_prev, mask, use_raw_only, image_flags, labels)
 
 
 class CompositeLocalGenerator(CompositeGenerator):
@@ -510,10 +560,10 @@
             self.model_final_flow = nn.Sequential(*_head(ngf, 2))
             self.model_final_w = nn.Sequential(*_head(ngf, 1, nn.Sigmoid()))
 
-    def _describe(self, plan, N, H, W, use_raw_only=False):
+    def _describe(self, plan, N, H, W, use_raw_only=False, ids=None):
         h2, w2 = H // 2, W // 2
         c2 = self.model_down_seg[4].out_channels
-        v_in = plan.input(S_IN, N, self.input_nc, 0, self.input_nc, H, W, exact_bf16=self.input_exact_bf16)
+        v_in = self._stem_input(plan, N, H, W, ids)
         v_prev = plan.input(S_PREV, N, self.prev_output_nc, 0, self.prev_output_nc, H, W)
         ci = plan.input(S_CI, N, c2, 0, c2, h2, w2)
         fg0 = None
@@ -544,9 +594,10 @@
             emit_head(plan, self.indv_final, fg_feat, (S_FG, self.output_nc, 1.0))
         self._emit_composite(plan, N, H, W, use_raw_only)
 
-    def forward(self, input, img_prev, mask, img_feat_coarse, flow_feat_coarse, img_fg_feat_coarse, use_raw_only, image_flags=None):
+    def forward(self, input, img_prev, mask, img_feat_coarse, flow_feat_coarse, img_fg_feat_coarse, use_raw_only, image_flags=None,
+                labels=None):
         return self._run(('GL',), (img_feat_coarse, flow_feat_coarse, img_fg_feat_coarse), input, img_prev, mask,
-                         use_raw_only, image_flags)
+                         use_raw_only, image_flags, labels)
 
 
 class GlobalGenerator(_Planned):
diff --git a/vid2vid_b200/plan.py b/vid2vid_b200/plan.py
--- a/vid2vid_b200/plan.py
+++ b/vid2vid_b200/plan.py
@@ -52,10 +52,14 @@
     return d
 
 
+def simt_selected():
+    return os.environ.get('V2V_CONV_IMPL') == 'simt'
+
+
 class Plan:
     def __init__(self, device=0, impl=None, precision='fast', train=False, sample_stats=False):
         if impl is None:
-            impl = L.IMPL_SIMT if os.environ.get('V2V_CONV_IMPL') == 'simt' else L.IMPL_UMMA
+            impl = L.IMPL_SIMT if simt_selected() else L.IMPL_UMMA
         self._h = C.c_void_p()
         self.device = device
         self.precision = precision
@@ -91,6 +95,14 @@
         self.n_slots = max(self.n_slots, slot + 1)
         return v.value
 
+    def label_input(self, s_labels, s_inst, N, T, tG, label_nc, level, H0, W0, s_mask=-1, fg_labels=(), exact_bf16=False):
+        v = C.c_int()
+        arr = (C.c_int * max(1, len(fg_labels)))(*fg_labels)
+        L.check(L.lib().v2v_g_label_input(self._h, s_labels, s_inst, N, T, tG, label_nc, level, H0, W0, s_mask, arr, len(fg_labels),
+                                          1 if exact_bf16 else 0, C.byref(v)))
+        self.n_slots = max(self.n_slots, s_labels + 1, s_inst + 1, s_mask + 1)
+        return v.value
+
     def conv(self, vin, desc):
         r = C.c_int()
         self._keep.append(desc)
```

Result: faster. 21.70 (median of 6 runs) (+1.8%).
